# medhini/audio-video-textures

Hardware: AMD Instinct MI355X
Metric: clip-windows/sec encoded + N×N transition build, N=4096; HBM GB/s achieved (higher is better)
Workload: dtype f16x3

## Files before the change

audio-video-textures_amd/_lib.py:

```python
import ctypes as C
import os

_HERE = os.path.dirname(os.path.abspath(__file__))
LIB_PATH = os.environ.get("AVT_HIP_LIB") or os.path.join(_HERE, "libavt_hip.so")
HEADER_PATH = os.path.join(os.path.dirname(_HERE), "include", "avt.h")

_i32p, _i64p, _f32p, _vp = (C.POINTER(C.c_int32), C.POINTER(C.c_int64), C.POINTER(C.c_float), C.c_void_p)

SIGNATURES = {
    "avt_abi_version": [],
    "avt_device_check": [C.c_char_p, C.c_size_t],
    "avt_clip_sample_table": [C.c_int, _vp, _vp],
    "avt_clip_pack_plan": [_vp, C.c_int, C.c_int, C.c_int, _vp, _vp],
    "avt_clip_pack_u8": [_vp, C.c_int, C.c_int, C.c_int, _vp, _vp, C.c_int, C.c_int, C.c_float, C.c_float,
                         C.c_int, _vp, _vp, C.c_int, _vp],
    "avt_l2norm_rows": [_vp, C.c_int, _vp, C.c_int, C.c_int64, C.c_float, _vp, _vp, _vp, _vp],
    "avt_sim_gemm_nt": [_vp, _vp, _vp, _vp, C.c_int64, C.c_int64, C.c_int, C.c_float, C.c_int, _vp, C.c_int64, _vp],
    "avt_gemm_nt_x3_f32out": [_vp, _vp, C.c_int, _vp, _vp, _vp, C.c_int64, C.c_int, C.c_int, C.c_int, C.c_float, _vp, C.c_int, _vp],
    "avt_row_transition": [_vp, C.c_int64, C.c_int64, C.c_int64, _vp, C.c_int64, _vp, C.c_int64, C.c_float,
                           C.c_float, C.c_int, _vp, _vp, _vp, _vp, _vp, _vp],
    "avt_row_topk": [_vp, C.c_int64, C.c_int64, C.c_int64, _vp, C.c_int, _vp, _vp, _vp],
    "avt_softmax_ce_fwd": [_vp, C.c_int64, C.c_int64, _vp, _vp, _vp, _vp],
    "avt_softmax_ce_bwd": [_vp, _vp, C.c_int64, C.c_int64, C.c_float, _vp, _vp],
    "avt_clip_pack_u8_ndhwc4": [_vp, C.c_int, C.c_int, C.c_int, _vp, _vp, C.c_int, C.c_int, C.c_float, C.c_float,
                                C.c_int, _vp, _vp, _vp],
    "avt_maxpool_hw3s2_ndhwc_bf16": [_vp, _vp] + [C.c_int] * 7 + [_vp],
    "avt_mean_positions_bf16": [_vp] + [C.c_int] * 4 + [_vp, C.c_int, _vp],
    "avt_maxpool_hw2s2_ndhwc_bf16": [_vp, _vp] + [C.c_int] * 6 + [_vp],
    "avt_stem_conv_supported": [C.c_int] * 3,
    "avt_stem_conv_bf16": [_vp, _vp, _vp, _vp] + [C.c_int] * 9 + [_vp],
    "avt_stem_conv_pool_bf16": [_vp, _vp, _vp, _vp] + [C.c_int] * 10 + [_vp],
    "avt_bottleneck_fused_supported": [C.c_int] * 2,
    "avt_bottleneck_fused_bf16": [_vp] * 8 + [C.c_int] * 6 + [_vp],
    "avt_bottleneck_first_supported": [C.c_int] * 3,
    "avt_bottleneck_first_bf16": [_vp] * 9 + [C.c_int] * 7 + [_vp],
    "avt_pairwise_l2_f32": [_vp, C.c_int, C.c_int64, _vp, _vp],
    "avt_diag_filter_f32": [_vp, C.c_int, _vp, C.c_int, _vp, _vp],
    "avt_q_learning_supported": [C.c_int],
    "avt_q_learning_f32": [_vp, C.c_int, C.c_float, C.c_float, C.c_int, _vp, _vp, _vp],
    "avt_conv33_c64_supported": [C.c_int] * 3,
    "avt_conv33_c64_bf16": [_vp] * 4 + [C.c_int] * 6 + [_vp],
    "avt_pw_chain_supported": [C.c_int] * 5,
    "avt_pw_chain_bf16": [_vp, C.c_int, C.c_int, _vp, _vp, _vp, C.c_int, _vp, C.c_int, C.c_int, _vp, C.c_int, C.c_int,
                          _vp, _vp, _vp, C.c_int, C.c_int, C.c_int64, _vp],
    "avt_logmel_f64": [_vp, C.c_int, C.c_int64, _vp, C.c_int, C.c_int, C.c_int, _vp, C.c_int, C.c_double, _vp, _vp],
    "avt_logmel_examples_f32": [_vp, C.c_int64, C.c_int, C.c_int, C.c_int, _vp, _vp],
    "avt_infonce_fwd": [_vp, _vp, C.c_int64, C.c_int, C.c_int, C.c_float, C.c_float, _vp, _vp, _vp, _vp],
    "avt_infonce_bwd": [_vp] * 6 + [C.c_int64, C.c_int, C.c_int, C.c_float, _vp, _vp, _vp],
    "avt_conv3d_ktab": [C.c_int] * 7 + [_vp, C.c_int],
    "avt_conv3d_igemm_bf16": [_vp] * 6 + [C.c_int] * 22 + [_vp],
    "avt_conv3d_igemm_rows_bf16": [_vp] * 6 + [C.c_int] * 25 + [_vp],
    "avt_bn_train_fwd": [_vp, _vp, _vp, C.c_int64, C.c_int, _vp, _vp, C.c_float, C.c_float, C.c_int, C.c_int, _vp, C.c_int64, _vp, _vp, _vp,
                         _vp, _vp, _vp, C.c_int64, _vp],
    "avt_bn_train_bwd": [_vp, _vp, _vp, C.c_int64, C.c_int, _vp, _vp, _vp, _vp, C.c_int, C.c_int, _vp, _vp, C.c_int64, _vp, _vp, _vp, _vp,
                         C.c_int64, _vp],
    "avt_bn_train_ws_bytes": [C.c_int64, C.c_int, C.c_int],
    "avt_bn_train_ws_bytes_pre": [C.c_int, C.c_int, C.c_int],
    "avt_bn_train_fwd_pre": [_vp, _vp, _vp, C.c_int64, C.c_int, _vp, _vp, C.c_float, C.c_float, C.c_int, C.c_int, _vp, C.c_int64, _vp, _vp,
                             _vp, _vp, _vp, _vp, C.c_int64, C.c_int, _vp],
    "avt_conv3d_igemm_x3_f32_stat_rows": [C.c_int, C.c_int, C.c_int64, C.c_int],
    "avt_conv3d_igemm_x3_f32_bwdstats_rows": [C.c_int, C.c_int, C.c_int64, C.c_int],
    "avt_conv3d_igemm_x3_f32_bwdstats": [_vp] * 7 + [C.c_int] * 16 + [_vp] * 6 + [C.c_int, _vp, C.c_int, C.c_int, _vp],
    "avt_bn_train_bwd_pre": [_vp, _vp, C.c_int64, C.c_int, _vp, _vp, _vp, C.c_int, _vp, C.c_int64, C.c_int, _vp, _vp, _vp, _vp],
    "avt_pw_x3_f32_stat_rows": [C.c_int, C.c_int, C.c_int64, C.c_int],
    "avt_pw_x3_f32_bwdstats_rows": [C.c_int, C.c_int, C.c_int64, C.c_int],
    "avt_pw_x3_f32_bwdstats": [_vp, C.c_int, C.c_int, _vp, _vp, _vp, C.c_int, _vp, C.c_int, C.c_int, C.c_int64, C.c_int] + [_vp] * 6 +
                              [C.c_int, _vp, C.c_int, _vp],
    "avt_pw_x3_f32_stats": [_vp, C.c_int, C.c_int, _vp, _vp, _vp, _vp, C.c_int, C.c_int, C.c_int64, C.c_int, _vp, C.c_int, _vp],
    "avt_conv3d_igemm_x3_f32_stats": [_vp, _vp, _vp, _vp, _vp, _vp] + [C.c_int] * 18 + [_vp, C.c_int, C.c_int, _vp],
    "avt_conv3d_igemm_x3_f32": [_vp, _vp, _vp, _vp, _vp, _vp, _vp] + [C.c_int] * 19 + [_vp],
    "avt_conv3d_igemm_x3_f32_ex": [_vp] * 6 + [C.c_int] * 21 + [_vp],
    "avt_conv3d_wgrad_x3_f32": [_vp, _vp, _vp] + [C.c_int] * 17 + [_vp],
    "avt_wgrad_x3_set_xl": [C.c_int],
    "avt_conv_x3_set_small_tile": [C.c_int],
    "avt_conv3d_wgrad_x3_sub_f32": [_vp, _vp, _vp] + [C.c_int] * 22 + [_vp],
    "avt_interp_pack_pair_u8": [_vp, _vp, C.c_int, C.c_int, _f32p, _vp, _vp, _vp, C.c_int, _vp],
    "avt_avgpool2_x3": [_vp, _vp, C.c_int, C.c_int, C.c_int, C.c_int, C.c_int, _vp, _vp, C.c_int, C.c_int, _vp],
    "avt_upsample2_bilinear_x3": [_vp, _vp, C.c_int, C.c_int, C.c_int, C.c_int, C.c_int, _vp, _vp, C.c_int, C.c_int, _vp],
    "avt_interp_mid_input": [_vp, _vp, _vp, C.c_int, C.c_int, C.c_int, _vp, _vp, _vp, C.c_int, _vp],
    "avt_interp_final_u8": [_vp, _vp, _vp, _vp, C.c_int, C.c_int, C.c_int, _f32p, _vp, C.c_int, _vp],
    "avt_negative_sample_mt19937": [_vp, _vp, C.c_int, C.c_int, C.c_int, _vp, _vp],
    "avt_clip_pack_gather_u8": [_vp, C.c_int, C.c_int, C.c_int, _vp, C.c_int, C.c_int, C.c_int, C.c_float, C.c_float,
                                C.c_int, _vp, _vp, C.c_int, _vp],
    "avt_frames_resize_aa_norm_u8": [_vp, C.c_int, C.c_int, C.c_int, C.c_int, _f32p, _f32p, _vp, _vp],
    "avt_clip_gather_frames_f32": [_vp, C.c_int, C.c_int, _vp, C.c_int, C.c_int, _vp, _vp],
    "avt_stem_conv_x3": [_vp] * 8 + [C.c_int] * 11 + [_vp, C.c_int, _vp],
    "avt_lateral_x3_supported": [C.c_int] * 3,
    "avt_lateral_x3": [_vp, _vp, C.c_int, C.c_int, _vp, _vp, _vp, _vp, _vp, _vp] + [C.c_int] * 10 + [_vp],
    "avt_stem_conv_x3_merged": [_vp] * 8 + [C.c_int] * 10 + [_vp, _vp, C.c_int, C.c_int, _vp],
    "avt_clip_planes_f32": [_vp] + [C.c_int] * 4 + [C.c_int64] * 5 + [_vp, _vp, C.c_int, _vp],
    "avt_stem_conv_x3_f32": [_vp] * 6 + [C.c_int] * 11 + [_vp],
    "avt_weight_planes_f32": [_vp, C.c_int, C.c_int, _vp, _vp, _vp, C.c_int, _vp],
    "avt_weight_planes_t_f32": [_vp, C.c_int, C.c_int, C.c_int, _i32p, C.c_int, _vp, _vp, _vp],
    "avt_weight_planes_gather_f32": [_vp, _vp, C.c_int, C.c_int, _vp, _vp, _vp, C.c_int, _vp],
    "avt_weight_planes_job_bytes": [],
    "avt_weight_planes_multi": [_vp, _vp, C.c_int, _vp],
    "avt_sgd_job_bytes": [],
    "avt_sgd_multi": [_vp, _vp, C.c_int, _vp, _vp],
    "avt_sgd_upload": [_vp, _vp, C.c_int64, _vp],
    "avt_pack_job_bytes": [],
    "avt_grad_pack_multi": [_vp, _vp, C.c_int, _vp, _vp],
    "avt_maxpool_train_fwd": [_vp, _vp, _vp] + [C.c_int] * 4 + [C.c_int64, _vp],
    "avt_maxpool_train_bwd": [_vp, _vp, _vp] + [C.c_int] * 4 + [C.c_int64, _vp],
    "avt_maxpool3d_train_fwd": [_vp, _vp, _vp] + [C.c_int] * 5 + [C.c_int64, _vp],
    "avt_maxpool3d_train_bwd": [_vp, _vp, _vp] + [C.c_int] * 5 + [C.c_int64, _vp],
    "avt_stem_wgrad_x3_supported": [C.c_int] * 4,
    "avt_stem_wgrad_x3": [_vp] * 4 + [C.c_int] * 7 + [_vp],
    "avt_pw_x3_supported": [C.c_int] * 2,
    "avt_pw_x3": [_vp, _vp, C.c_int, C.c_int, _vp, _vp, _vp, _vp, _vp, _vp, C.c_int, _vp, _vp, C.c_int, C.c_int, C.c_int64,
                  C.c_int, C.c_int, _vp],
    "avt_pw_x3_f32_supported": [C.c_int] * 2,
    "avt_pw_x3_f32": [_vp, C.c_int, C.c_int, _vp, _vp, _vp, _vp, C.c_int, _vp, C.c_int, C.c_int, C.c_int64, C.c_int, _vp],
    "avt_pw_chain_x3_supported": [C.c_int] * 3,
    "avt_pw_chain_x3": [_vp, _vp, C.c_int, C.c_int, _vp, _vp, _vp, _vp, _vp, _vp, C.c_int, _vp, _vp, C.c_int, C.c_int, C.c_int,
                        _vp, _vp, _vp, _vp, _vp, _vp, C.c_int, C.c_int, C.c_int64, C.c_int, _vp],
    "avt_conv3d_igemm_x3": [_vp] * 10 + [C.c_int] * 26 + [_vp, _vp],
    "avt_conv3d_igemm_x3_wblk": [_vp] * 10 + [C.c_int] * 26 + [_vp, _vp],
    "avt_clip_pack_u8_ndhwc4_x3": [_vp, C.c_int, C.c_int, C.c_int, _vp, _vp, C.c_int, C.c_int, C.c_float, C.c_float,
                                   C.c_int, _vp, _vp, _vp, _vp, C.c_int, _vp],
    "avt_maxpool_hw3s2_ndhwc_x3": [_vp] * 4 + [C.c_int] * 8 + [_vp, _vp],
    "avt_maxpool_hw2s2_ndhwc_x3": [_vp] * 4 + [C.c_int] * 7 + [_vp],
    "avt_maxpool3d_k3s2_ndhwc_x3": [_vp] * 4 + [C.c_int] * 8 + [_vp],
    "avt_mean_positions_x3": [_vp, _vp] + [C.c_int] * 4 + [_vp, C.c_int, C.c_int, _vp],
    "avt_conv3d_igemm_x3_xl_picked": [C.c_int] * 3,
    "avt_conv33_x3_supported": [C.c_int] * 2,
    "avt_conv33_x3": [_vp] * 6 + [C.c_int] * 8 + [_vp],
    "avt_bneck_x3_supported": [C.c_int] * 3,
    "avt_bneck_x3": [_vp] * 6 + [C.c_int] * 8 + [_vp],
    "avt_res2_x3_supported": [C.c_int] * 3,
    "avt_res2_x3_wfrag_bytes": [],
    "avt_res2_x3": [_vp] * 6 + [C.c_int] * 7 + [_vp],
    "avt_conv3d_igemm_wfrag_supported": [C.c_int] * 5,
    "avt_conv3d_igemm_wfrag_bf16": [_vp] * 6 + [C.c_int] * 25 + [_vp, C.c_int, _vp],
}


class AvtError(RuntimeError):
    pass


_lib = None


def lib():
    global _lib
    if _lib is None:
        if not os.path.exists(LIB_PATH):
            raise AvtError(
                "HIP extension not built: %s is missing. Run `make -C %s` (needs hipcc); "
                "there is no CPU fallback for the hot path." % (LIB_PATH, os.path.join(_HERE, "csrc")))
        handle = C.CDLL(LIB_PATH)
        for name, argtypes in SIGNATURES.items():
            fn = getattr(handle, name)
            fn.argtypes = argtypes
            fn.restype = C.c_int64 if name in _RETURNS_I64 else C.c_int
        handle.avt_last_error.argtypes = []
        handle.avt_last_error.restype = C.c_char_p
        if handle.avt_abi_version() != ABI_VERSION:
            raise AvtError("libavt_hip.so ABI version %d, expected %d: rebuild with `make -C %s`"
                           % (handle.avt_abi_version(), ABI_VERSION, os.path.join(_HERE, "csrc")))
        if os.environ.get("AVT_SMALL_TILE", "") == "0":
            handle.avt_conv_x3_set_small_tile(0)
        if os.environ.get("AVT_WGRAD_ROUNDS", "") == "0":
            handle.avt_wgrad_x3_set_xl(7)
        _lib = handle
    return _lib


ABI_VERSION = 8
_RETURNS_I64 = {"avt_bn_train_ws_bytes", "avt_bn_train_ws_bytes_pre"}


def check(status, what):
    if status != 0:
        msg = lib().avt_last_error()
        raise AvtError("%s failed (%d): %s" % (what, status, msg.decode() if msg else "?"))
```

audio-video-textures_amd/csrc/conv_x3.hip:

```cpp
#include <stdlib.h>

#include <type_traits>

#include "avt_common.h"
#include "conv_args.h"
#include "launch.h"
#include "mfma.h"
#include "split_planes.h"

#ifdef AVT_CONV_STAMP
#define AVT_STAMP_FN avt_debug_stamps_x3
namespace {
#include "../../tools/diag/conv_stamp.h"
}
#ifndef AVT_DBG_CONST
#define AVT_DBG_CONST 0
#endif
#define DBG_SKIP(bit) (((AVT_DBG_CONST) & (bit)) != 0)
#ifdef AVT_STAMP_EPI
#define KSTAMP(i) STAMP(0)
#define EPI_STAMP(i) STAMP(i)
#else
#define KSTAMP(i) STAMP(i)
#define EPI_STAMP(i)
// ... 94 lines not shown
    }
    const int koff = ks * 32 + lh * 16;
#pragma unroll
    for (int j = 0; j < MT; ++j) {
      const int o = (wm * WTM + j * 32 + lr) * LSTR + koff;
      f.ah[j] = *reinterpret_cast<const i32x4*>(lds + o);
      f.al[j] = *reinterpret_cast<const i32x4*>(lds + A_LO + o);
    }
#pragma unroll
    for (int i = 0; i < NT; ++i) {
      const int o = (wn * WN + i * 32 + lr) * LSTR + koff;
      f.wh[i] = *reinterpret_cast<const i32x4*>(lds + B_HI + o);
      f.wl[i] = *reinterpret_cast<const i32x4*>(lds + B_LO + o);
    }
  };
  constexpr int NPIECE = 2 * (AU + BU), NGROUP = 4 * NT * MT, PPG = 2 * ((NPIECE + NGROUP - 1) / NGROUP);
  auto fmul = [&](const Frags& f, int g0, auto more_, auto&& piece) {
    constexpr bool more = decltype(more_)::value;
#pragma unroll
    for (int i = 0; i < NT; ++i)
#pragma unroll
      for (int j = 0; j < MT; ++j) {
        if (!DBG_SKIP(2)) {
          acc[i][j] = mfma32<F16>(f.wl[i], f.ah[j], acc[i][j]);
          acc[i][j] = mfma32<F16>(f.wh[i], f.al[j], acc[i][j]);
          acc[i][j] = mfma32<F16>(f.wh[i], f.ah[j], acc[i][j]);
        }
        if (more && !DBG_SKIP(4)) {
#pragma unroll
          for (int e = 0; e < PPG; ++e) {
            const int pc = (g0 + i * MT + j) * PPG + e;
            if (pc < NPIECE) piece(pc);
          }
        }
        __builtin_amdgcn_sched_barrier(0);
      }
  };
  auto compute = [&](auto more, auto&& prep, auto&& piece) {
    Frags f0, f1;
    fload(f0, 0);
    fload(f1, 1);
    if constexpr (decltype(more)::value) prep();
    __builtin_amdgcn_sched_barrier(0);
    fmul(f0, 0, more, piece);
    fload(f0, 2);
    __builtin_amdgcn_sched_barrier(0);
    fmul(f1, NT * MT, more, piece);
    fload(f1, 3);
    __builtin_amdgcn_sched_barrier(0);
    fmul(f0, 2 * NT * MT, more, piece);
    fmul(f1, 3 * NT * MT, more, piece);
  };

  const __amdgpu_buffer_rsrc_t rih = avt::buffer_rsrc(a.in, a.in_bytes);
  const __amdgpu_buffer_rsrc_t ril = avt::buffer_rsrc(a.in_lo, a.in_bytes);
  const __amdgpu_buffer_rsrc_t rwh = avt::buffer_rsrc(a.wt, a.wt_bytes);
  const __amdgpu_buffer_rsrc_t rwl = avt::buffer_rsrc(a.wt_lo, a.wt_bytes);
  int2* ltab = reinterpret_cast<int2*>(lds + STAGE);
  const bool tab_lds = a.nk <= kMaxTabSteps;
  if (tab_lds)
    for (int i = tid; i < a.nk * 8; i += 256) ltab[i] = a.ktab[i];
  i32x4 rah[AU], ral[AU], rbh[BU], rbl[BU];
  unsigned aoffs[AU], boffs[BU];
  auto gprep = [&](auto tl_, int kt) {
    int2 e;
    if constexpr (decltype(tl_)::value) e = ltab[kt * 8 + c16];
    else e = a.ktab[kt * 8 + c16];
    const unsigned ebits = (unsigned)e.y;
#pragma unroll
    for (int u = 0; u < AU; ++u) {
      const unsigned sel = ((rowmask[u] & ebits) == ebits) ? 0xFFFFFFFFu : 0u;
      aoffs[u] = (((unsigned)(rowoff[u] + e.x) * (IO32 ? 4u : 2u)) & sel) | (kOob & ~sel);
    }
    const unsigned ksel = ~(unsigned)(e.y >> 31);
    const unsigned kc2 = (unsigned)((kt * 8 + c16) * 16);
#pragma unroll
    for (int u = 0; u < BU; ++u) {
      const unsigned sel = ksel & wsel[u];
      boffs[u] = (((unsigned)wrow[u] * 2u + kc2) & sel) | (kOob & ~sel);
    }
  };
  auto gpiece = [&](int p) {
    if (p < 2 * AU) {
      const int u = p >> 1;
      if constexpr (IO32) {
        const unsigned o2 = aoffs[u] == kOob ? kOob : aoffs[u] + 16u;
        if (p & 1) ral[u] = __builtin_amdgcn_raw_buffer_load_b128(rih, (int)o2, 0, 0);
        else rah[u] = __builtin_amdgcn_raw_buffer_load_b128(rih, (int)aoffs[u], 0, 0);
      } else {
        if (p & 1) ral[u] = __builtin_amdgcn_raw_buffer_load_b128(ril, (int)aoffs[u], 0, 0);
        else rah[u] = __builtin_amdgcn_raw_buffer_load_b128(rih, (int)aoffs[u], 0, 0);
      }
    } else {
      const int u = (p - 2 * AU) >> 1;
      if (p & 1) rbl[u] = __builtin_amdgcn_raw_buffer_load_b128(rwl, (int)boffs[u], 0, 0);
      else rbh[u] = __builtin_amdgcn_raw_buffer_load_b128(rwh, (int)boffs[u], 0, 0);
    }
  };
  auto gload = [&](int kt) {
    gprep(std::false_type{}, kt);
#pragma unroll
    for (int p = 0; p < NPIECE; ++p) gpiece(p);
  };
  auto lstore = [&]() {
#pragma unroll
    for (int u = 0; u < AU; ++u) {
      const int o = (r0 + 32 * u) * LSTR + c16 * 16;
      if constexpr (IO32) {
        const float* fa = reinterpret_cast<const float*>(&rah[u]);
        const float* fb = reinterpret_cast<const float*>(&ral[u]);
        uint4 h, l;
        const float f8[8] = {fa[0], fa[1], fa[2], fa[3], fb[0], fb[1], fb[2], fb[3]};
        avt::split8<F16>(f8, h, l);
        *reinterpret_cast<uint4*>(lds + o) = h;
        *reinterpret_cast<uint4*>(lds + A_LO + o) = l;
      } else {
        *reinterpret_cast<i32x4*>(lds + o) = rah[u];
        *reinterpret_cast<i32x4*>(lds + A_LO + o) = ral[u];
      }
    }
#pragma unroll
    for (int u = 0; u < BU; ++u) {
      const int o = (r0 + 32 * u) * LSTR + c16 * 16;
      *reinterpret_cast<i32x4*>(lds + B_HI + o) = rbh[u];
      *reinterpret_cast<i32x4*>(lds + B_LO + o) = rbl[u];
    }
  };
  float* cfl = reinterpret_cast<float*>(lds + a.cf_ofs);
  for (int i = tid; i < 2 * BN; i += 256) {
    const int n = n0 + (i < BN ? i : i - BN);
    float v = i < BN ? 0.0f : 1.0f;
    if (n < a.Cout) {
      if (i < BN) { if (a.bias) v = a.bias[n]; } else if (a.wscale) v = a.wscale[n];
    }
    cfl[i] = v;
  }
  __syncthreads();
  STAMP_BEGIN();
  gload(0);
  lstore();
  __syncthreads();
  STAMP(0);
  auto kloop = [&](auto tl) {
    for (int kt = 0; kt + 1 < a.nk; ++kt) {
      STAMP(1);
      compute(std::true_type{}, [&]() { gprep(tl, kt + 1); }, gpiece);
      STAMP(2);
      __syncthreads();
      STAMP(3);
      if (!DBG_SKIP(1)) lstore();
      STAMP(4);
      __syncthreads();
      STAMP(5);
    }
  };
  if (tab_lds) kloop(std::true_type{});
  else kloop(std::false_type{});
  STAMP(1);
  compute(std::false_type{}, []() {}, gpiece);
  STAMP(2);
  __syncthreads();
  STAMP(3);

  const bool has_res = !IO32 && a.res != nullptr;
  uint4 rrh[EU], rrl[EU];
  if (has_res) {
#pragma unroll
    for (int u = 0; u < EU; ++u) {
      const int c = tid + 256 * u;
      const int m = m0 + c / CPR, n = n0 + (c % CPR) * 8;
      const bool ok = m < m_end && n < a.Cout;
      rrh[u] = ok ? *reinterpret_cast<const uint4*>(a.res + (int64_t)m * a.ldr + n) : make_uint4(0u, 0u, 0u, 0u);
      rrl[u] = ok ? *reinterpret_cast<const uint4*>(a.res_lo + (int64_t)m * a.ldr + n) : make_uint4(0u, 0u, 0u, 0u);
    }
  }
  if constexpr (IO32) {
    if (a.res) {
#pragma unroll
      for (int u = 0; u < EU; ++u) {
        const int c = tid + 256 * u;
        const int m = m0 + c / CPR, n = n0 + (c % CPR) * 8;
        const bool ok = m < m_end && n < a.Cout;
        const float* rf = reinterpret_cast<const float*>(a.res) + (int64_t)m * a.ldr + n;
        rrh[u] = ok ? *reinterpret_cast<const uint4*>(rf) : make_uint4(0u, 0u, 0u, 0u);
        rrl[u] = ok ? *reinterpret_cast<const uint4*>(rf + 4) : make_uint4(0u, 0u, 0u, 0u);
      }
    }
  }
  float4 bxa[BST ? EU : 1], bxb[BST ? EU : 1];
  unsigned bbits[BST ? EU : 1];
  BstCoef bk;
  if constexpr (BST) {
    {
      const int n = n0 + (tid % CPR) * 8;
      bst_load(a, tm / a.stat_tpg, n < a.Cout ? n : 0, bk);
#pragma unroll
      for (int u = 0; u < EU; ++u) {
        const int c = tid + 256 * u;
        const int m = m0 + c / CPR;
        const bool ok = m < m_end && n < a.Cout;
        const int64_t o = ok ? (int64_t)m * a.ldo + n : 0;
        bxa[u] = *reinterpret_cast<const float4*>(a.bst_x + o);
        bxb[u] = *reinterpret_cast<const float4*>(a.bst_x + o + 4);
        bbits[u] = a.bst_mask ? *reinterpret_cast<const uint16_t*>(a.bst_mask + (o >> 2)) : 0u;
        bbits[u] = (bbits[u] & 0xFu) | ((bbits[u] >> 4) & 0xF0u);
      }
    }
  }
#pragma unroll
  for (int i = 0; i < NT; ++i)
#pragma unroll
    for (int g = 0; g < 4; ++g) {
      const int nl = wn * WN + i * 32 + 8 * g + 4 * lh;
      const float4 bv = *reinterpret_cast<const float4*>(cfl + nl);
      const float4 sv = *reinterpret_cast<const float4*>(cfl + BN + nl);
#pragma unroll
      for (int j = 0; j < MT; ++j) {
        float4 v;
        v.x = acc[i][j][4 * g + 0] * sv.x + bv.x;
        v.y = acc[i][j][4 * g + 1] * sv.y + bv.y;
        v.z = acc[i][j][4 * g + 2] * sv.z + bv.z;
        v.w = acc[i][j][4 * g + 3] * sv.w + bv.w;
        const int ml = wm * WTM + j * 32 + lr;
        *reinterpret_cast<float4*>(lds + ml * ESTR + nl * 4) = v;
      }
    }
  __syncthreads();
  float st_s[IO32 ? 8 : 1], st_q[IO32 ? 8 : 1];
  if constexpr (IO32) {
#pragma unroll
    for (int e = 0; e < 8; ++e) st_s[e] = st_q[e] = 0.0f;
  }
#pragma unroll
  for (int u = 0; u < EU; ++u) {
    const int c = tid + 256 * u;
    const int row = c / CPR, cc = c % CPR;
    const int m = m0 + row, n = n0 + cc * 8;
    if (m < m_end && n < a.Cout) {
      const float4 v0 = *reinterpret_cast<const float4*>(lds + row * ESTR + cc * 32);
      const float4 v1 = *reinterpret_cast<const float4*>(lds + row * ESTR + cc * 32 + 16);
      float x[8] = {v0.x, v0.y, v0.z, v0.w, v1.x, v1.y, v1.z, v1.w};
      if (has_res) {
        const uint32_t* ph = reinterpret_cast<const uint32_t*>(&rrh[u]);
        const uint32_t* pl = reinterpret_cast<const uint32_t*>(&rrl[u]);
#pragma unroll
        for (int e = 0; e < 4; ++e) {
          const avt::f32x2 r = avt::join2<F16>(ph[e], pl[e]);
          x[2 * e] += r.x;
          x[2 * e + 1] += r.y;
        }
      }
      if (a.relu == 1) {
#pragma unroll
        for (int e = 0; e < 8; ++e) x[e] = avt::relu_keep_nan(x[e]);
      } else if (a.relu == 2) {
#pragma unroll
        for (int e = 0; e < 8; ++e) x[e] = fmaxf(x[e], 0.1f * x[e]);
      }
      const int64_t o = (int64_t)out_row(a, m) * a.ldo + n;
      if constexpr (IO32) {
        if (a.res) {
          const float4 r0_ = __builtin_bit_cast(float4, rrh[u]), r1_ = __builtin_bit_cast(float4, rrl[u]);
          x[0] += r0_.x; x[1] += r0_.y; x[2] += r0_.z; x[3] += r0_.w;
          x[4] += r1_.x; x[5] += r1_.y; x[6] += r1_.z; x[7] += r1_.w;
        }
        if constexpr (BST) {
          const float xv[8] = {bxa[u].x, bxa[u].y, bxa[u].z, bxa[u].w, bxb[u].x, bxb[u].y, bxb[u].z, bxb[u].w};
          bst_apply(a, bk, xv, bbits[u], x, st_s, st_q);
        } else if (a.stat_part) {
#pragma unroll
          for (int e = 0; e < 8; ++e) {
            st_s[e] += x[e];
            st_q[e] += x[e] * x[e];
          }
        }
        float* of = reinterpret_cast<float*>(a.out) + o;
        avt::stg4(of, avt::f32x4{x[0], x[1], x[2], x[3]});
        avt::stg4(of + 4, avt::f32x4{x[4], x[5], x[6], x[7]});
      } else {
        uint4 oh, ol;
        avt::split8<F16>(x, oh, ol);
        *reinterpret_cast<uint4*>(a.out + o) = oh;
        *reinterpret_cast<uint4*>(a.out_lo + o) = ol;
      }
    }
  }
  if constexpr (IO32) {
    if (a.stat_part) {
      __syncthreads();
      float* red = reinterpret_cast<float*>(lds);
      const int tr = tid / CPR, cc = tid % CPR;
#pragma unroll
      for (int e = 0; e < 8; ++e) {
        red[(tr * 2 + 0) * BN + cc * 8 + e] = st_s[e];
        red[(tr * 2 + 1) * BN + cc * 8 + e] = st_q[e];
      }
      __syncthreads();
      stat_fold_store<BN, 256>(a, red, 256 / CPR, tm, n0, tid);
    }
  }
  STAMP_END();
}

template <bool F16, bool IO32 = false, bool OUT32 = IO32>
__global__ __launch_bounds__(512, 2) void conv_x3_xl_kernel(ConvArgs a) {
  constexpr int BM = 256, BN = 256, NTHR = 512, KB = 32;
  constexpr int MT = 4, NT = 2;
  constexpr int AU = BM / 128, BU = BN / 128;
  constexpr int PL = BM * 64;
  constexpr int STG = 4 * PL;
  constexpr int ESTR = BN * 4 + 16;
  extern __shared__ __attribute__((aligned(16))) char lds[];

  const int swz = avt::xcd_contiguous(blockIdx.x, a.nblk);
  const int tm = swz / a.tiles_n, tn = swz % a.tiles_n;
  const int n0 = tn * BN;
  int m0, m_end;
  if constexpr (IO32) tile_rows(a, tm, BM, m0, m_end);
  else { m0 = tm * BM; m_end = a.M; }
  const int tid = threadIdx.x;
  const int lane = tid & 63, wid = tid >> 6;
  const int wm = wid >> 2, wn = wid & 3;
  const int lr = lane & 31, lh = lane >> 5;
  const int r0 = tid >> 2, c4 = (tid & 3) ^ ((r0 >> 2) & 3);

  int rowoff[AU];
  unsigned rowmask[AU];
#pragma unroll
  for (int u = 0; u < AU; ++u) {
    const int m = m0 + r0 + 128 * u;
    rowoff[u] = 0;
    rowmask[u] = 0u;
    if (m < m_end && a.pointwise) {
      rowoff[u] = m * a.ldi;
      rowmask[u] = 0x010101u;
    } else if (m < m_end) {
      const int t1 = (int)fastdiv((uint32_t)m, a.dWo), wo = m - t1 * a.Wo;
      const int t2 = (int)fastdiv((uint32_t)t1, a.dHo), ho = t1 - t2 * a.Ho;
      const int b = (int)fastdiv((uint32_t)t2, a.dTo), to = t2 - b * a.To;
      const int ti0 = to * a.st - a.pt, hi0 = ho * a.sh - a.ph, wi0 = wo * a.sw - a.pw;
      rowoff[u] = (((b * a.T + ti0) * a.H + hi0) * a.W + wi0) * a.ldi;
      unsigned mask = 0u;
      for (int dt = 0; dt < a.KT; ++dt) mask |= ((unsigned)(ti0 + dt) < (unsigned)a.T ? 1u : 0u) << dt;
      for (int dh = 0; dh < a.KH; ++dh) mask |= ((unsigned)(hi0 + dh) < (unsigned)a.H ? 1u : 0u) << (8 + dh);
      for (int dw = 0; dw < a.KW; ++dw) mask |= ((unsigned)(wi0 + dw) < (unsigned)a.W ? 1u : 0u) << (16 + dw);
      rowmask[u] = mask;
    }
  }
  int wrow[BU];
  unsigned wsel[BU];
#pragma unroll
  for (int u = 0; u < BU; ++u) {
    const int n = n0 + r0 + 128 * u;
    wrow[u] = n < a.Cout ? n * a.K : 0;
    wsel[u] = n < a.Cout ? 0xFFFFFFFFu : 0u;
  }

  f32x16 acc[NT][MT];
#pragma unroll
  for (int i = 0; i < NT; ++i)
#pragma unroll
    for (int j = 0; j < MT; ++j)
#pragma unroll
      for (int r = 0; r < 16; ++r) acc[i][j][r] = 0.0f;
  const __amdgpu_buffer_rsrc_t rih = avt::buffer_rsrc(a.in, a.in_bytes);
  const __amdgpu_buffer_rsrc_t ril = avt::buffer_rsrc(a.in_lo, a.in_bytes);
  const __amdgpu_buffer_rsrc_t rwh = avt::buffer_rsrc(a.wt, a.wt_bytes);
  const __amdgpu_buffer_rsrc_t rwl = avt::buffer_rsrc(a.wt_lo, a.wt_bytes);
  int2* ltab = reinterpret_cast<int2*>(lds + 2 * STG);
  for (int i = tid; i < a.nk * 8; i += NTHR) ltab[i] = a.ktab[i];
  const int nk32 = (a.K + KB - 1) / KB;

  unsigned aoffs[AU], boffs[BU];
  auto gtab = [&](int kt) -> int2 { return ltab[kt * 4 + c4]; };
  auto gcalc = [&](int kt, int2 e) {
    const unsigned ebits = (unsigned)e.y;
#pragma unroll
    for (int u = 0; u < AU; ++u) {
      const unsigned sel = ((rowmask[u] & ebits) == ebits) ? 0xFFFFFFFFu : 0u;
      aoffs[u] = (((unsigned)(rowoff[u] + e.x) * (IO32 ? 4u : 2u)) & sel) | (kOob & ~sel);
    }
    const unsigned ksel = ~(unsigned)(e.y >> 31);
    const unsigned kc2 = (unsigned)((kt * 4 + c4) * 16);
#pragma unroll
    for (int u = 0; u < BU; ++u) {
      const unsigned sel = ksel & wsel[u];
      boffs[u] = (((unsigned)wrow[u] * 2u + kc2) & sel) | (kOob & ~sel);
      if (a.wblk) boffs[u] = (((unsigned)(kt * a.Cout + n0 + r0 + 128 * u) * 64u + (unsigned)c4 * 16u) & sel) | (kOob & ~sel);
    }
  };
  auto gprep = [&](int kt) { gcalc(kt, gtab(kt)); };
  constexpr int NPIECE = 2 * (AU + BU);
  typedef __attribute__((address_space(3))) void* lds_ptr;
  const int wrow0 = wid * 16 * 64;
  auto gpiece = [&](int p, char* st) {
    if (p < 2 * AU) {
      const int u = p >> 1;
      __builtin_amdgcn_raw_ptr_buffer_load_lds((p & 1) ? ril : rih, (lds_ptr)(st + (p & 1) * PL + wrow0 + u * 128 * 64), 16,
                                               (int)aoffs[u], 0, 0, 0);
    } else {
      const int u = (p - 2 * AU) >> 1;
      __builtin_amdgcn_raw_ptr_buffer_load_lds((p & 1) ? rwl : rwh, (lds_ptr)(st + (2 + (p & 1)) * PL + wrow0 + u * 128 * 64), 16,
                                               (int)boffs[u], 0, 0, 0);
    }
  };
  i32x4 ra[IO32 ? AU : 1][2];
  auto aload = [&]() {
    if constexpr (IO32) {
#pragma unroll
      for (int u = 0; u < AU; ++u) {
        const unsigned o2 = aoffs[u] == kOob ? kOob : aoffs[u] + 16u;
        ra[u][0] = __builtin_amdgcn_raw_buffer_load_b128(rih, (int)aoffs[u], 0, 0);
        ra[u][1] = __builtin_amdgcn_raw_buffer_load_b128(rih, (int)o2, 0, 0);
      }
    }
  };
  auto astore = [&](char* st) {
    if constexpr (IO32) {
#pragma unroll
      for (int u = 0; u < AU; ++u) {
        const float* fa = reinterpret_cast<const float*>(&ra[u][0]);
        const float* fb = reinterpret_cast<const float*>(&ra[u][1]);
        uint4 h, l;
        const float f8[8] = {fa[0], fa[1], fa[2], fa[3], fb[0], fb[1], fb[2], fb[3]};
        avt::split8<F16>(f8, h, l);
        const int o = (r0 + 128 * u) * 64 + (tid & 3) * 16;
        *reinterpret_cast<uint4*>(st + o) = h;
        *reinterpret_cast<uint4*>(st + PL + o) = l;
      }
    }
  };
  const int fsw = (lr >> 2) & 3;
  struct Frags {
    i32x4 ah[MT], al[MT], wh[NT], wl[NT];
  };
  auto fload = [&](Frags& f, const char* st, int ks) {
    const int slot = ((ks * 2 + lh) ^ fsw) * 16;
    auto rd_w = [&](int i) {
      const int o = (wn * 64 + i * 32 + lr) * 64 + slot;
      f.wh[i] = *reinterpret_cast<const i32x4*>(st + 2 * PL + o);
      f.wl[i] = *reinterpret_cast<const i32x4*>(st + 3 * PL + o);
    };
    rd_w(0);
#pragma unroll
    for (int j = 0; j < MT; ++j) {
      const int o = (wm * 128 + j * 32 + lr) * 64 + slot;
      f.ah[j] = *reinterpret_cast<const i32x4*>(st + o);
      f.al[j] = *reinterpret_cast<const i32x4*>(st + PL + o);
    }
#pragma unroll
    for (int i = 1; i < NT; ++i) rd_w(i);
  };
  auto fmul = [&](const Frags& f, int g0, bool more, char* nst) {
#pragma unroll
    for (int i = 0; i < NT; ++i)
#pragma unroll
      for (int j = 0; j < MT; ++j) {
        acc[i][j] = mfma32<F16>(f.wl[i], f.ah[j], acc[i][j]);
        acc[i][j] = mfma32<F16>(f.wh[i], f.al[j], acc[i][j]);
        acc[i][j] = mfma32<F16>(f.wh[i], f.ah[j], acc[i][j]);
        const int pc = g0 + i * MT + j + (IO32 ? 2 * AU : 0);
        if (more && pc < NPIECE) gpiece(pc, nst);
        __builtin_amdgcn_sched_barrier(0);
      }
  };

  float* cfl = reinterpret_cast<float*>(lds + a.cf_ofs);
  {
    const int n = n0 + (tid & 255);
    float v = tid < 256 ? 0.0f : 1.0f;
    if (n < a.Cout) {
      if (tid < 256) { if (a.bias) v = a.bias[n]; } else if (a.wscale) v = a.wscale[n];
    }
    cfl[tid] = v;
  }
  __syncthreads();
  STAMP_BEGIN();
  gprep(0);
  if constexpr (IO32) {
    aload();
#pragma unroll
    for (int p = 2 * AU; p < NPIECE; ++p) gpiece(p, lds);
    asm volatile("s_waitcnt vmcnt(0)" ::: "memory");
    astore(lds);
  } else {
#pragma unroll
    for (int p = 0; p < NPIECE; ++p) gpiece(p, lds);
    asm volatile("s_waitcnt vmcnt(0)" ::: "memory");
  }
  __syncthreads();
  STAMP(0);
  if constexpr (IO32) {
    for (int kt = 0; kt < nk32; ++kt) {
      const bool more = kt + 1 < nk32;
      char* cur = lds + (kt & 1) * STG;
      char* nst = lds + ((kt + 1) & 1) * STG;
      int2 e = make_int2(0, 0);
      if (more) e = gtab(kt + 1);
      Frags f;
      fload(f, cur, 0);
      if (more) {
        gcalc(kt + 1, e);
        aload();
      }
      __builtin_amdgcn_sched_barrier(0);
      fmul(f, 0, more, nst);
      fload(f, cur, 1);
      __builtin_amdgcn_sched_barrier(0);
      fmul(f, NPIECE, false, nst);
      asm volatile("s_waitcnt vmcnt(0)" ::: "memory");
      if (more) astore(nst);
      __syncthreads();
    }
  } else {
    Frags f0, f1;
    fload(f0, lds, 0);
    if (nk32 > 1) gprep(1);
    fload(f1, lds, 1);
    __builtin_amdgcn_sched_barrier(0);
    fmul(f0, 0, nk32 > 1, lds + STG);
    asm volatile("s_waitcnt vmcnt(0) lgkmcnt(0)" ::: "memory");
    __syncthreads();
    for (int kt = 1; kt < nk32; ++kt) {
      const bool more = kt + 1 < nk32;
      char* cur = lds + (kt & 1) * STG;
      char* nst = lds + ((kt + 1) & 1) * STG;
      int2 e = make_int2(0, 0);
      if (more) e = gtab(kt + 1);
      fload(f0, cur, 0);
      if (more) gcalc(kt + 1, e);
      __builtin_amdgcn_sched_barrier(0);
      fmul(f1, 0, more, nst);
      KSTAMP(1);
      fload(f1, cur, 1);
      __builtin_amdgcn_sched_barrier(0);
      fmul(f0, NPIECE, false, nst);
      KSTAMP(2);
      asm volatile("s_waitcnt vmcnt(0) lgkmcnt(0)" ::: "memory");
      KSTAMP(3);
      __syncthreads();
      KSTAMP(4);
    }
    fmul(f1, NPIECE, false, lds);
  }

  constexpr int SR = 64;
  constexpr int CPR = BN / 8;
  constexpr int EU = (SR * CPR) / NTHR;
  constexpr int EBUF = SR * ESTR;
  static_assert(2 * EBUF <= 2 * STG + kMaxTabSteps * 64, "two staging buffers fit the operand stages + the table area");
  const bool has_res = !OUT32 && a.res != nullptr;
  auto stage_slab = [&](auto half, int pass) {
    constexpr int H = decltype(half)::value;
    char* eb = lds + (pass & 1) * EBUF;
#pragma unroll
    for (int i = 0; i < NT; ++i)
#pragma unroll
      for (int g = 0; g < 4; ++g) {
        const int nl = wn * 64 + i * 32 + 8 * g + 4 * lh;
        const float4 bv = *reinterpret_cast<const float4*>(cfl + nl);
        const float4 sv = *reinterpret_cast<const float4*>(cfl + 256 + nl);
#pragma unroll
        for (int jj = 0; jj < 2; ++jj) {
          const int j = 2 * H + jj;
          float4 v;
          v.x = acc[i][j][4 * g + 0] * sv.x + bv.x;
          v.y = acc[i][j][4 * g + 1] * sv.y + bv.y;
          v.z = acc[i][j][4 * g + 2] * sv.z + bv.z;
          v.w = acc[i][j][4 * g + 3] * sv.w + bv.w;
          const int rl = jj * 32 + lr;
          *reinterpret_cast<float4*>(eb + rl * ESTR + nl * 4) = v;
        }
      }
  };
  KSTAMP(5);
  if (wm == 0) stage_slab(std::integral_constant<int, 0>{}, 0);
  __syncthreads();
  EPI_STAMP(1);
  float st_s[IO32 ? 8 : 1], st_q[IO32 ? 8 : 1];
  if constexpr (IO32) {
#pragma unroll
    for (int e = 0; e < 8; ++e) st_s[e] = st_q[e] = 0.0f;
  }
#pragma unroll 1
  for (int pass = 0; pass < 4; ++pass) {
    const char* eb = lds + (pass & 1) * EBUF;
    uint4 rrh[EU], rrl[EU];
    if (has_res) {
#pragma unroll
      for (int u = 0; u < EU; ++u) {
        const int c = tid + NTHR * u;
        const int m = m0 + pass * SR + c / CPR, n = n0 + (c % CPR) * 8;
        const bool ok = m < m_end && n < a.Cout;
        rrh[u] = ok ? *reinterpret_cast<const uint4*>(a.res + (int64_t)m * a.ldr + n) : make_uint4(0u, 0u, 0u, 0u);
        rrl[u] = ok ? *reinterpret_cast<const uint4*>(a.res_lo + (int64_t)m * a.ldr + n) : make_uint4(0u, 0u, 0u, 0u);
      }
    }
    if constexpr (IO32) {
      if (a.res) {
#pragma unroll
        for (int u = 0; u < EU; ++u) {
          const int c = tid + NTHR * u;
          const int m = m0 + pass * SR + c / CPR, n = n0 + (c % CPR) * 8;
          const bool ok = m < m_end && n < a.Cout;
          const float* rf = reinterpret_cast<const float*>(a.res) + (int64_t)m * a.ldr + n;
          rrh[u] = ok ? *reinterpret_cast<const uint4*>(rf) : make_uint4(0u, 0u, 0u, 0u);
          rrl[u] = ok ? *reinterpret_cast<const uint4*>(rf + 4) : make_uint4(0u, 0u, 0u, 0u);
        }
      }
    }
    if (pass + 1 < 4 && wm == ((pass + 1) >> 1)) {
      if ((pass + 1) & 1) stage_slab(std::integral_constant<int, 1>{}, pass + 1);
      else stage_slab(std::integral_constant<int, 0>{}, pass + 1);
    }
    EPI_STAMP(2);
#pragma unroll
    for (int u = 0; u < EU; ++u) {
      const int c = tid + NTHR * u;
      const int row = c / CPR, cc = c % CPR;
      const int m = m0 + pass * SR + row, n = n0 + cc * 8;
      if (m < m_end && n < a.Cout) {
        const float4 v0 = *reinterpret_cast<const float4*>(eb + row * ESTR + cc * 32);
        const float4 v1 = *reinterpret_cast<const float4*>(eb + row * ESTR + cc * 32 + 16);
        float x[8] = {v0.x, v0.y, v0.z, v0.w, v1.x, v1.y, v1.z, v1.w};
        if (has_res) {
          const uint32_t* ph = reinterpret_cast<const uint32_t*>(&rrh[u]);
          const uint32_t* pl = reinterpret_cast<const uint32_t*>(&rrl[u]);
#pragma unroll
          for (int e = 0; e < 4; ++e) {
            const avt::f32x2 r = avt::join2<F16>(ph[e], pl[e]);
            x[2 * e] += r.x;
            x[2 * e + 1] += r.y;
          }
        }
        if (a.relu == 1) {
#pragma unroll
          for (int e = 0; e < 8; ++e) x[e] = avt::relu_keep_nan(x[e]);
        } else if (a.relu == 2) {
#pragma unroll
          for (int e = 0; e < 8; ++e) x[e] = fmaxf(x[e], 0.1f * x[e]);
        }
        const int64_t o = (int64_t)out_row(a, m) * a.ldo + n;
        if constexpr (OUT32) {
          if (a.odiv != 0.0f) {
#pragma unroll
            for (int e = 0; e < 8; ++e) x[e] = __fdiv_rn(x[e], a.odiv);
          }
          if (IO32 && a.res) {
            const float4 q0 = __builtin_bit_cast(float4, rrh[u]), q1 = __builtin_bit_cast(float4, rrl[u]);
            x[0] += q0.x; x[1] += q0.y; x[2] += q0.z; x[3] += q0.w;
            x[4] += q1.x; x[5] += q1.y; x[6] += q1.z; x[7] += q1.w;
          }
          if constexpr (IO32) {
            if (a.stat_part) {
#pragma unroll
              for (int e = 0; e < 8; ++e) {
                st_s[e] += x[e];
                st_q[e] += x[e] * x[e];
              }
            }
          }
          float* of = reinterpret_cast<float*>(a.out) + o;
          avt::stg4(of, avt::f32x4{x[0], x[1], x[2], x[3]});
          avt::stg4(of + 4, avt::f32x4{x[4], x[5], x[6], x[7]});
        } else {
          uint4 oh, ol;
          avt::split8<F16>(x, oh, ol);
          *reinterpret_cast<uint4*>(a.out + o) = oh;
          *reinterpret_cast<uint4*>(a.out_lo + o) = ol;
        }
      }
    }
    EPI_STAMP(3);
    __syncthreads();
    EPI_STAMP(4);
  }
  if constexpr (IO32) {
    if (a.stat_part) {
      float* red = reinterpret_cast<float*>(lds);
      const int tr = tid / CPR, cc = tid % CPR;
#pragma unroll
      for (int e = 0; e < 8; ++e) {
        red[(tr * 2 + 0) * BN + cc * 8 + e] = st_s[e];
        red[(tr * 2 + 1) * BN + cc * 8 + e] = st_q[e];
      }
      __syncthreads();
      stat_fold_store<BN, NTHR>(a, red, NTHR / CPR, tm, n0, tid);
    }
  }
  STAMP_END();
}

template <bool F16, bool IO32 = false, bool OUT32 = IO32>
int launch_x3_xl(ConvArgs& a, hipStream_t st) {
  if (a.stat_part) a.stat_tpg = (a.stat_mg + 255) / 256;
  const int tiles_m = a.stat_part ? a.stat_groups * a.stat_tpg : (a.M + 255) / 256;
  a.tiles_n = (a.Cout + 255) / 256;
  a.nblk = tiles_m * a.tiles_n;
  constexpr int lds_bytes = 2 * 4 * 256 * 64 + kMaxTabSteps * 64 + 2 * 256 * 4;
  a.cf_ofs = lds_bytes - 2 * 256 * 4;
  return avt::launch<conv_x3_xl_kernel<F16, IO32, OUT32>>("avt_conv3d_igemm_x3", dim3((unsigned)a.nblk), dim3(512), lds_bytes, lds_bytes,
                                                          st, a);
}

template <int BM, int BN, int WTM, bool F16, bool IO32 = false, bool BST = false>
int launch_x3(ConvArgs& a, hipStream_t st) {
  if (a.stat_part) a.stat_tpg = (a.stat_mg + BM - 1) / BM;
  const int tiles_m = a.stat_part ? a.stat_groups * a.stat_tpg : (a.M + BM - 1) / BM;
  a.tiles_n = (a.Cout + BN - 1) / BN;
  a.nblk = tiles_m * a.tiles_n;
  constexpr int epi_bytes = BM * (BN * 4 + 16);
  constexpr int opnd_max = 2 * (BM + BN) * LSTR + kMaxTabSteps * 64;
  constexpr int lds_max = (opnd_max > epi_bytes ? opnd_max : epi_bytes) + 2 * BN * 4;
  const int tab_bytes = (a.nk <= kMaxTabSteps ? a.nk : 0) * 64;
  int lds_bytes = 2 * (BM + BN) * LSTR + tab_bytes;
  if (lds_bytes < epi_bytes) lds_bytes = epi_bytes;
  a.cf_ofs = lds_bytes;
  lds_bytes += 2 * BN * 4;
  return avt::launch<conv_x3_kernel<BM, BN, WTM, F16, IO32, BST>>("avt_conv3d_igemm_x3", dim3((unsigned)a.nblk), dim3(256), lds_max,
                                                                  lds_bytes, st, a);
}

template <bool F16, bool IO32 = false, bool BST = false>
int launch_x3_by_cout(ConvArgs& a, hipStream_t st, bool small = false) {
  if (a.Cout <= 32) return launch_x3<128, 32, 32, F16, IO32, BST>(a, st);
  if (a.Cout <= 64) return launch_x3<128, 64, 64, F16, IO32, BST>(a, st);
  if constexpr (IO32) {
    if (small) return launch_x3<64, 128, 32, F16, IO32, BST>(a, st);
  }
  return launch_x3<128, 128, 64, F16, IO32, BST>(a, st);
}

struct X3Planes {
  const void *in_hi, *in_lo, *wt_hi, *wt_lo;
  const float* bias;
  const void *res_hi, *res_lo;
  void *out_hi, *out_lo;
};

}

extern "C" int avt_conv3d_igemm_x3_xl_picked(int cout, int k, int m) {
  return (cout % 256 == 0 && k >= 256 && k <= kMaxTabSteps * 64 && m >= 256 * 64) ? 1 : 0;
}

static int igemm_x3_one(const X3Planes& p, const int32_t* ktab, const ConvGeom& g, int plane_dtype, const float* wscale, void* stream,
                        int wblk, int xl) {
  AVT_REQUIRE(plane_dtype == AVT_X3_BF16 || plane_dtype == AVT_X3_F16, "avt_conv3d_igemm_x3: plane_dtype must be 0 (bf16) or 1 (fp16)");
  AVT_REQUIRE(!wscale || avt::aligned16(wscale), "avt_conv3d_igemm_x3: wscale must be 16-byte aligned");
  AVT_REQUIRE(p.in_lo && p.wt_lo && p.out_lo && (!p.res_hi == !p.res_lo), "avt_conv3d_igemm_x3: every tensor needs both planes");
  AVT_REQUIRE(avt::aligned16(p.in_lo) && avt::aligned16(p.wt_lo) && avt::aligned16(p.out_lo) && (!p.res_lo || avt::aligned16(p.res_lo)),
              "avt_conv3d_igemm_x3: pointers must be 16-byte aligned");
  ConvArgs a;
  const int rc = conv_args_fill(a, "avt_conv3d_igemm_x3", p.in_hi, p.wt_hi, p.bias, p.res_hi, p.out_hi, ktab, g);
  if (rc != AVT_OK) return rc;
  a.in_lo = static_cast<const uint16_t*>(p.in_lo);
  a.wt_lo = static_cast<const uint16_t*>(p.wt_lo);
  a.res_lo = static_cast<const uint16_t*>(p.res_lo);
  a.out_lo = static_cast<uint16_t*>(p.out_lo);
  a.wscale = wscale;
  a.wfrag = nullptr;
  a.nup = 0;
  a.wblk = wblk;
  hipStream_t s = static_cast<hipStream_t>(stream);
  AVT_REQUIRE(!wblk || (xl && a.K % 32 == 0),
              "avt_conv3d_igemm_x3_wblk: K-blocked weights are the 256 x 256 tile's (avt_conv3d_igemm_x3_xl_picked, K %% 32 == 0)");
  if (xl) return plane_dtype == AVT_X3_F16 ? launch_x3_xl<true>(a, s) : launch_x3_xl<false>(a, s);
  return plane_dtype == AVT_X3_F16 ? launch_x3_by_cout<true>(a, s) : launch_x3_by_cout<false>(a, s);
}

static int igemm_x3_impl(const X3Planes& p, const int32_t* ktab, const ConvGeom& g, int plane_dtype, const float* wscale, void* stream,
                         int wblk) {
  constexpr int64_t kMaxPlane = (1ll << 31) - 64;
  const bool sane = g.batch > 0 && g.t > 0 && g.h > 0 && g.w > 0 && g.ldi > 0 && g.ldo > 0 && g.cin > 0 && g.cout > 0 && g.kt >= 1 &&
                    g.kh >= 1 && g.kw >= 1 && g.st >= 1 && g.sh >= 1 && g.sw >= 1 && g.ph >= 0 && g.pw >= 0 && g.ho >= 0 && g.wo >= 0 &&
                    g.out_row_stride >= 1 && g.out_h >= 0 && g.out_w >= 0;
  const int64_t frame = sane ? (int64_t)g.h * g.w * g.ldi : 0, frames = sane ? (int64_t)g.batch * g.t : 0;
  if (!sane || frame * frames < kMaxPlane || g.kt != 1 || g.st != 1 || g.pt != 0 || (g.to != 0 && g.to != g.t)) {
    const int64_t k_all = (int64_t)g.kt * g.kh * g.kw * g.cin;
    int xl = 0;
    if (sane && k_all < (1ll << 31)) {
      const int64_t fho = g.ho > 0 ? g.ho : (g.h + 2 * g.ph - g.kh) / g.sh + 1, fwo = g.wo > 0 ? g.wo : (g.w + 2 * g.pw - g.kw) / g.sw + 1;
      const int64_t fto = g.to > 0 ? g.to : (g.t + 2 * g.pt - g.kt) / g.st + 1;
      const int64_t m = (int64_t)g.batch * fto * fho * fwo;
      xl = (m > 0 && m < (1ll << 31)) ? avt_conv3d_igemm_x3_xl_picked(g.cout, (int)k_all, (int)m) : 0;
    }
    return igemm_x3_one(p, ktab, g, plane_dtype, wscale, stream, wblk, xl);
  }
  AVT_REQUIRE(frame < kMaxPlane, "avt_conv3d_igemm_x3: one frame's input plane (%d x %d x %d elements) is too large for 32-bit offsets", g.h,
              g.w, g.ldi);
  AVT_REQUIRE(p.in_hi && p.in_lo && p.out_hi && p.out_lo && (!p.res_hi == !p.res_lo), "avt_conv3d_igemm_x3: every tensor needs both planes");
  const int fho = g.ho > 0 ? g.ho : (g.h + 2 * g.ph - g.kh) / g.sh + 1, fwo = g.wo > 0 ? g.wo : (g.w + 2 * g.pw - g.kw) / g.sw + 1;
  AVT_REQUIRE(fho > 0 && fwo > 0, "avt_conv3d_igemm_x3: bad output extent");
  const bool remap = g.out_row_stride > 1 || (g.out_h > 0 && g.out_w > 0);
  const int64_t m_all = frames * fho * fwo;
  const int64_t orows = remap ? (int64_t)g.out_h * g.out_w : (int64_t)fho * fwo;
  AVT_REQUIRE(m_all < (1ll << 31) && frames * orows < (1ll << 31) && (int64_t)g.kh * g.kw * g.cin < (1ll << 31),
              "avt_conv3d_igemm_x3: tensor too large for 32-bit rows");
  const int xl = avt_conv3d_igemm_x3_xl_picked(g.cout, g.kh * g.kw * g.cin, (int)m_all);
  const int64_t fmax = kMaxPlane / frame;
  const int64_t nrange = (frames + fmax - 1) / fmax;
  const int64_t per = (frames + nrange - 1) / nrange;
  for (int64_t f0 = 0; f0 < frames; f0 += per) {
    ConvGeom gr = g;
    gr.batch = (int)((frames - f0 < per) ? frames - f0 : per);
    gr.t = 1;
    gr.to = g.to ? 1 : 0;
    const int64_t io = f0 * frame, oo = f0 * orows * g.ldo, ro = f0 * fho * fwo * g.ldr;
    auto adv = [](const void* q, int64_t e) { return q ? static_cast<const void*>(static_cast<const uint16_t*>(q) + e) : nullptr; };
    X3Planes pr = p;
    pr.in_hi = adv(p.in_hi, io), pr.in_lo = adv(p.in_lo, io);
    pr.res_hi = adv(p.res_hi, ro), pr.res_lo = adv(p.res_lo, ro);
    pr.out_hi = const_cast<void*>(adv(p.out_hi, oo)), pr.out_lo = const_cast<void*>(adv(p.out_lo, oo));
    const int rc = igemm_x3_one(pr, ktab, gr, plane_dtype, wscale, stream, wblk, xl);
    if (rc != AVT_OK) return rc;
  }
  return AVT_OK;
}

extern "C" int avt_conv3d_igemm_x3(const void* in_hi, const void* in_lo, const void* wt_hi, const void* wt_lo,
                                   const float* bias, const void* res_hi, const void* res_lo, void* out_hi, void* out_lo,
                                   const int32_t* ktab, int batch, int t, int h, int w, int cin, int cout, int kt, int kh,
                                   int kw, int st, int sh, int sw, int pt, int ph, int pw, int to, int ho, int wo, int ldi,
                                   int ldo, int ldr, int relu, int out_row_stride, int out_h, int out_w, int plane_dtype,
                                   const float* wscale, void* stream) {
  const ConvGeom g = {.batch = batch, .t = t, .h = h, .w = w, .cin = cin, .cout = cout, .kt = kt, .kh = kh, .kw = kw,
                      .st = st, .sh = sh, .sw = sw, .pt = pt, .ph = ph, .pw = pw, .to = to, .ho = ho, .wo = wo,
                      .ldi = ldi, .ldo = ldo, .ldr = ldr, .relu = relu, .out_row_stride = out_row_stride, .out_h = out_h, .out_w = out_w};
  const X3Planes p = {.in_hi = in_hi, .in_lo = in_lo, .wt_hi = wt_hi, .wt_lo = wt_lo, .bias = bias,
                      .res_hi = res_hi, .res_lo = res_lo, .out_hi = out_hi, .out_lo = out_lo};
  return igemm_x3_impl(p, ktab, g, plane_dtype, wscale, stream, 0);
}

extern "C" int avt_conv3d_igemm_x3_wblk(const void* in_hi, const void* in_lo, const void* wt_hi, const void* wt_lo,
                                        const float* bias, const void* res_hi, const void* res_lo, void* out_hi, void* out_lo,
                                        const int32_t* ktab, int batch, int t, int h, int w, int cin, int cout, int kt, int kh,
                                        int kw, int st, int sh, int sw, int pt, int ph, int pw, int to, int ho, int wo, int ldi,
                                        int ldo, int ldr, int relu, int out_row_stride, int out_h, int out_w, int plane_dtype,
                                        const float* wscale, void* stream) {
  const ConvGeom g = {.batch = batch, .t = t, .h = h, .w = w, .cin = cin, .cout = cout, .kt = kt, .kh = kh, .kw = kw,
                      .st = st, .sh = sh, .sw = sw, .pt = pt, .ph = ph, .pw = pw, .to = to, .ho = ho, .wo = wo,
                      .ldi = ldi, .ldo = ldo, .ldr = ldr, .relu = relu, .out_row_stride = out_row_stride, .out_h = out_h, .out_w = out_w};
  const X3Planes p = {.in_hi = in_hi, .in_lo = in_lo, .wt_hi = wt_hi, .wt_lo = wt_lo, .bias = bias,
                      .res_hi = res_hi, .res_lo = res_lo, .out_hi = out_hi, .out_lo = out_lo};
  return igemm_x3_impl(p, ktab, g, plane_dtype, wscale, stream, 1);
}

extern "C" int avt_gemm_nt_x3_f32out(const void* a_hi, const void* a_lo, int lda, const void* b_hi, const void* b_lo, float* out, int64_t ldo,
                                     int m, int n, int k, float divisor, const int32_t* ktab, int plane_dtype, void* stream) {
  AVT_REQUIRE(plane_dtype == AVT_X3_BF16 || plane_dtype == AVT_X3_F16, "avt_gemm_nt_x3_f32out: plane_dtype must be 0 (bf16) or 1 (fp16)");
  AVT_REQUIRE(a_lo && b_lo && avt::aligned16(a_lo) && avt::aligned16(b_lo) && divisor != 0.0f, "avt_gemm_nt_x3_f32out: both planes, divisor != 0");
  AVT_REQUIRE(m > 0 && n % 256 == 0 && k % 32 == 0 && k >= 256 && k <= kMaxTabSteps * 64 && ldo >= n && ldo % 4 == 0 && ldo < (1ll << 31),
              "avt_gemm_nt_x3_f32out: n %% 256 == 0, 256 <= k <= %d in multiples of 32 (got m %d n %d k %d)", kMaxTabSteps * 64, m, n, k);
  const ConvGeom g = {.batch = 1, .t = 1, .h = 1, .w = m, .cin = k, .cout = n, .kt = 1, .kh = 1, .kw = 1, .st = 1, .sh = 1, .sw = 1,
                      .pt = 0, .ph = 0, .pw = 0, .to = 0, .ho = 0, .wo = 0, .ldi = lda, .ldo = 8 * (int)((ldo + 7) / 8), .ldr = 0,
                      .relu = 0, .out_row_stride = 1, .out_h = 0, .out_w = 0};
  ConvArgs a;
  const int rc = conv_args_fill(a, "avt_gemm_nt_x3_f32out", a_hi, b_hi, nullptr, nullptr, out, ktab, g);
  if (rc != AVT_OK) return rc;
  a.ldo = (int)ldo;
  a.in_lo = static_cast<const uint16_t*>(a_lo);
  a.wt_lo = static_cast<const uint16_t*>(b_lo);
  a.res_lo = nullptr;
  a.out_lo = nullptr;
  a.wscale = nullptr;
  a.wfrag = nullptr;
  a.nup = 0;
  a.wblk = 0;
  a.odiv = divisor;
  hipStream_t s = static_cast<hipStream_t>(stream);
  return plane_dtype == AVT_X3_F16 ? launch_x3_xl<true, false, true>(a, s) : launch_x3_xl<false, false, true>(a, s);
}

static int g_io32_small = 1;
static int io32_tile_rows(int cout, int k, int64_t m) {
  if (k % 32 == 0 && m < (1ll << 31) && avt_conv3d_igemm_x3_xl_picked(cout, k, (int)m) && m >= 256 * 256) return 256;
  if (g_io32_small && cout > 64 && ((m + 127) / 128) * ((cout + 127) / 128) < 512) return 64;
  return 128;
}

extern "C" int avt_conv_x3_set_small_tile(int on) {
  const int was = g_io32_small;
  g_io32_small = on ? 1 : 0;
  return was;
}

static int igemm_x3_f32_impl(const float* in, const void* wt_hi, const void* wt_lo, const float* wscale, const float* add, float* out,
                             const int32_t* ktab, const ConvGeom& g, int plane_dtype, void* stream, double* stat_part = nullptr,
                             int stat_groups = 0, int stat_c = 0, const ConvArgs* bst = nullptr) {
  const int cout = g.cout;
  AVT_REQUIRE(plane_dtype == AVT_X3_BF16 || plane_dtype == AVT_X3_F16, "avt_conv3d_igemm_x3_f32: plane_dtype must be 0 (bf16) or 1 (fp16)");
  AVT_REQUIRE(wt_lo && avt::aligned16(wt_lo) && (!wscale || avt::aligned16(wscale)), "avt_conv3d_igemm_x3_f32: weight planes / wscale NULL or unaligned");
  AVT_REQUIRE((int64_t)g.batch * g.t * g.h * g.w * g.ldi < (1ll << 30) - 64, "avt_conv3d_igemm_x3_f32: input too large for 32-bit byte offsets");
  ConvArgs a;
  const int rc = conv_args_fill(a, "avt_conv3d_igemm_x3_f32", in, wt_hi, nullptr, add, out, ktab, g);
  if (rc != AVT_OK) return rc;
  a.in_bytes *= 2u;
  a.in_lo = nullptr;
  a.wt_lo = static_cast<const uint16_t*>(wt_lo);
  a.res_lo = nullptr;
  a.out_lo = nullptr;
  a.wscale = wscale;
  a.wfrag = nullptr;
  a.nup = 0;
  a.wblk = 0;
  if (stat_part) {
    AVT_REQUIRE(stat_groups >= 1 && a.M % stat_groups == 0 && stat_c >= 8 && cout % stat_c == 0 && a.oH == 0 && (!add || bst) &&
                    avt::aligned16(stat_part),
                "avt_conv3d_igemm_x3_f32_stats: %d rows in %d groups, %d channels of %d columns, no row remap, no add operand", a.M,
                stat_groups, stat_c, cout);
    {
      const int bn_launch = (!bst && a.oH == 0 && io32_tile_rows(cout, a.K, a.M) == 256) ? 256 : (cout <= 32 ? 32 : (cout <= 64 ? 64 : 128));
      AVT_REQUIRE(stat_c == cout || cout <= bn_launch,
                  "avt_conv3d_igemm_x3_f32_stats: %d pixel copies of %d channels span more than one %d-column tile", cout / stat_c, stat_c,
                  bn_launch);
    }
    if (bst) {
      AVT_REQUIRE(bst->bst_x && bst->bst_mean && bst->bst_invstd && bst->bst_gamma && g.ldo == cout && avt::aligned16(bst->bst_x) &&
                      (!bst->bst_relu || bst->bst_mask || bst->bst_beta),
                  "avt_conv3d_igemm_x3_f32_bwdstats: BatchNorm input / statistics / scale missing, or the output rows are not contiguous");
      a.bst_x = bst->bst_x; a.bst_mean = bst->bst_mean; a.bst_invstd = bst->bst_invstd; a.bst_gamma = bst->bst_gamma;
      a.bst_beta = bst->bst_beta; a.bst_mask = bst->bst_mask; a.bst_relu = bst->bst_relu;
    }
    a.stat_part = stat_part;
    a.stat_groups = stat_groups;
    a.stat_mg = a.M / stat_groups;
    a.stat_c = stat_c;
    AVT_REQUIRE((int64_t)stat_groups * ((a.stat_mg + 127) / 128) < (1ll << 24), "avt_conv3d_igemm_x3_f32_stats: too many tiles");
  }
  hipStream_t s = static_cast<hipStream_t>(stream);
  if (bst) {
    AVT_REQUIRE(plane_dtype == AVT_X3_BF16 && io32_tile_rows(cout, a.K, a.M) != 256,
                "avt_conv3d_igemm_x3_f32_bwdstats: bf16 planes, layers of the 128- / 64-row tiles (avt_conv3d_igemm_x3_f32_bwdstats_rows)");
    return launch_x3_by_cout<false, true, true>(a, s, io32_tile_rows(cout, a.K, a.M) == 64);
  }
  const bool small = io32_tile_rows(cout, a.K, a.M) == 64;
  if (a.oH == 0 && io32_tile_rows(cout, a.K, a.M) == 256)
    return plane_dtype == AVT_X3_F16 ? launch_x3_xl<true, true>(a, s) : launch_x3_xl<false, true>(a, s);
  return plane_dtype == AVT_X3_F16 ? launch_x3_by_cout<true, true>(a, s, small) : launch_x3_by_cout<false, true>(a, s, small);
}

extern "C" int avt_conv3d_igemm_x3_f32(const float* in, const void* wt_hi, const void* wt_lo, const float* wscale, const float* add,
                                       float* out, const int32_t* ktab, int batch, int t, int h, int w, int cin, int cout, int kt, int kh,
                                       int kw, int st, int sh, int sw, int pt, int ph, int pw, int ldi, int ldo, int lda, int plane_dtype,
                                       void* stream) {
  const ConvGeom g = {.batch = batch, .t = t, .h = h, .w = w, .cin = cin, .cout = cout, .kt = kt, .kh = kh, .kw = kw,
                      .st = st, .sh = sh, .sw = sw, .pt = pt, .ph = ph, .pw = pw, .ldi = ldi, .ldo = ldo, .ldr = add ? lda : 0,
                      .out_row_stride = 1};
  return igemm_x3_f32_impl(in, wt_hi, wt_lo, wscale, add, out, ktab, g, plane_dtype, stream);
}

extern "C" int avt_conv3d_igemm_x3_f32_stat_rows(int cout, int k, int64_t m, int groups) {
  if (groups < 1 || m <= 0 || m % groups) return -1;
  const int bm = io32_tile_rows(cout, k, m);
  return (int)((m / groups + bm - 1) / bm);
}

extern "C" int avt_conv3d_igemm_x3_f32_stats(const float* in, const void* wt_hi, const void* wt_lo, const float* wscale, float* out,
                                             const int32_t* ktab, int batch, int t, int h, int w, int cin, int cout, int kt, int kh, int kw,
                                             int st, int sh, int sw, int pt, int ph, int pw, int ldi, int ldo, int plane_dtype,
                                             void* stat_part, int groups, int stat_c, void* stream) {
  AVT_REQUIRE(stat_part, "avt_conv3d_igemm_x3_f32_stats: NULL stat_part");
  const ConvGeom g = {.batch = batch, .t = t, .h = h, .w = w, .cin = cin, .cout = cout, .kt = kt, .kh = kh, .kw = kw,
                      .st = st, .sh = sh, .sw = sw, .pt = pt, .ph = ph, .pw = pw, .ldi = ldi, .ldo = ldo, .ldr = 0,
                      .out_row_stride = 1};
  return igemm_x3_f32_impl(in, wt_hi, wt_lo, wscale, nullptr, out, ktab, g, plane_dtype, stream, static_cast<double*>(stat_part), groups,
                           stat_c);
}

extern "C" int avt_conv3d_igemm_x3_f32_bwdstats_rows(int cout, int k, int64_t m, int groups) {
  if (groups < 1 || m <= 0 || m % groups) return -1;
  const int bm = io32_tile_rows(cout, k, m);
  if (bm == 256) return -1;
  return (int)((m / groups + bm - 1) / bm);
}

extern "C" int avt_conv3d_igemm_x3_f32_bwdstats(const float* in, const void* wt_hi, const void* wt_lo, const float* wscale, const float* add,
                                                float* out, const int32_t* ktab, int batch, int t, int h, int w, int cin, int cout, int kt,
                                                int kh, int kw, int pt, int ph, int pw, int ldi, int ldo, int lda, int plane_dtype,
                                                const float* bn_x, const float* bn_mean, const float* bn_invstd, const float* bn_gamma,
                                                const float* bn_beta, const void* bn_mask, int relu, void* stat_part, int groups, int stat_c,
                                                void* stream) {
  AVT_REQUIRE(stat_part, "avt_conv3d_igemm_x3_f32_bwdstats: NULL stat_part");
  ConvArgs b = {};
  b.bst_x = bn_x; b.bst_mean = bn_mean; b.bst_invstd = bn_invstd; b.bst_gamma = bn_gamma; b.bst_beta = bn_beta;
  b.bst_mask = static_cast<const uint8_t*>(bn_mask); b.bst_relu = relu;
  const ConvGeom g = {.batch = batch, .t = t, .h = h, .w = w, .cin = cin, .cout = cout, .kt = kt, .kh = kh, .kw = kw,
                      .st = 1, .sh = 1, .sw = 1, .pt = pt, .ph = ph, .pw = pw, .ldi = ldi, .ldo = ldo, .ldr = add ? lda : 0,
                      .out_row_stride = 1};
  return igemm_x3_f32_impl(in, wt_hi, wt_lo, wscale, add, out, ktab, g, plane_dtype, stream, static_cast<double*>(stat_part), groups,
                           stat_c, &b);
}

extern "C" int avt_conv3d_igemm_x3_f32_ex(const float* in, const void* wt_hi, const void* wt_lo, const float* wscale, float* out,
                                          const int32_t* ktab, int batch, int t, int h, int w, int cin, int cout, int kt, int kh, int kw,
                                          int pt, int ph, int pw, int to, int ho, int wo, int ldi, int ldo, int out_row_stride, int out_h,
                                          int out_w, int plane_dtype, void* stream) {
  const ConvGeom g = {.batch = batch, .t = t, .h = h, .w = w, .cin = cin, .cout = cout, .kt = kt, .kh = kh, .kw = kw,
                      .st = 1, .sh = 1, .sw = 1, .pt = pt, .ph = ph, .pw = pw, .to = to, .ho = ho, .wo = wo, .ldi = ldi, .ldo = ldo, .ldr = 0,
                      .out_row_stride = out_row_stride, .out_h = out_h, .out_w = out_w};
  return igemm_x3_f32_impl(in, wt_hi, wt_lo, wscale, nullptr, out, ktab, g, plane_dtype, stream);
}
```

audio-video-textures_amd/fused_slowfast.py:

```python
import torch
import torch.nn as nn

from . import ops
from ._lib import AvtError


_FUSE_BLOCK = 1
_C33 = 1
_CHAIN = 1
_CHAIN_MAXN = 512
_FUSE_KCAT = 1
_XB = 1
_FUSE_SCAT = 1
_FUSE_TCHUNK = 0
_FUSE_SCAT_X3 = 1
_SCAT_X3_SKIP = set()
_FUSE_BLOCK_X3 = 1
_FUSE_TCHUNK_X3 = 0
_CHAIN_X3 = 1
_WBLK_X3 = 1
_STEM_FM_X3 = 1
_C33_X3 = 1
_RES2_X3 = 1
_PW_X3 = 1
_STEM_LDS = 1
_STEM_POOL = 1
_PW_X3_SKIP = {(512, 128), (320, 128)}
_LATERAL_X3 = {(32, 64)}
_STEM_MERGE = 1
_KW1_CAP = 32

PROFILER = None


def _observed(name, launch, flops, nbytes):
    if PROFILER is None:
        launch()
    else:
        PROFILER(name() if callable(name) else name, launch, flops, nbytes)


def _rows(dims):
    return dims[0] * dims[1] * dims[2] * dims[3]


class Act:

    __slots__ = ("buf", "dims", "c0", "C", "lo")

    def __init__(self, buf, dims, c0=0, C=None, lo=None):
        self.buf, self.dims, self.c0, self.lo = buf, dims, c0, lo
        self.C = buf.shape[1] - c0 if C is None else C

    @property
    def ptr(self):
        return self.buf.data_ptr() + 2 * self.c0

    @property
    def ptrs(self):
        return (self.buf.data_ptr() + 2 * self.c0, self.lo.data_ptr() + 2 * self.c0)

    @property
    def ld(self):
        return self.buf.shape[1]

    @property
    def rows(self):
        return _rows(self.dims)

    def float(self, plane_dtype=None):
        if self.lo is None:
            return self.buf[:, self.c0 : self.c0 + self.C].float()
        dt = torch.float16 if plane_dtype == ops.X3_F16 else torch.bfloat16
        sl = slice(self.c0, self.c0 + self.C)
        return self.buf.view(dt)[:, sl].float() + self.lo.view(dt)[:, sl].float()


def new_act(m, c, dims, device, x3=False):
    buf = torch.empty((m, c), dtype=torch.bfloat16, device=device)
    return Act(buf, dims, lo=torch.empty_like(buf) if x3 else None)


def split_planes(w, plane_dtype):
    w = w.detach().float()
    dt = torch.float16 if plane_dtype == ops.X3_F16 else torch.bfloat16
    hi = w.to(dt)
    lo = (w - hi.float()).to(dt)
    return hi.view(torch.bfloat16).contiguous(), lo.view(torch.bfloat16).contiguous()


def fold_bn(conv, bn):
    w = conv.weight.detach().float()
    if bn is not None:
        scale = bn.weight.detach().float() / torch.sqrt(bn.running_var.detach().float() + bn.eps)
        bias = bn.bias.detach().float() - bn.running_mean.detach().float() * scale
        w = w * scale.view(-1, 1, 1, 1, 1)
    else:
        bias = conv.bias.detach().float() if conv.bias is not None else torch.zeros(w.shape[0])
    return w, bias


def group_weights_w(w, g):
    cout, cin, kt, kh, kw = w.shape
    r = kw // 2
    rg = -(-r // g)
    kwg = 1 + 2 * rg
    wg = torch.zeros((g, cout, g, cin, kt, kh, kwg))
    for po in range(g):
        for dg in range(kwg):
            for pi in range(g):
                dw = g * (dg - rg) + pi - po + r
                if 0 <= dw < kw:
                    wg[po, :, pi, :, :, :, dg] = w[:, :, :, :, dw]
    return wg.reshape(g * cout, g * cin, kt, kh, kwg), rg


def pack_wfrag(wt, cin, taps):
    wt = wt.detach().float().cpu()
    cout, k = wt.shape
    nu = -(-k // 32)
    nup = -(-nu // 4) * 4 + 4
    tiles = -(-cout // 256) * 8
    wp = torch.zeros((tiles * 32, k + 1))
    wp[:cout, :k] = wt
    i = torch.arange(nup).view(-1, 1, 1, 1)
    cc, tap = (i // taps, i % taps) if taps > 1 else (i, torch.zeros_like(i))
    ks = torch.arange(2).view(1, -1, 1, 1)
    lane = torch.arange(64).view(1, 1, -1, 1)
    e = torch.arange(8).view(1, 1, 1, -1)
    cch = cc * 32 + ks * 16 + (lane >> 5) * 8 + e
    kidx = torch.where((cch < cin) & (i < nu), tap * cin + cch, torch.full_like(cch, k)).expand(nup, 2, 64, 8)
    rows = (torch.arange(tiles).view(-1, 1, 1, 1, 1) * 32 + (lane & 31).view(1, 1, 1, 64, 1)).expand(tiles, nup, 2, 64, 8)
    return wp[rows, kidx.unsqueeze(0).expand(tiles, nup, 2, 64, 8)].to(torch.bfloat16).contiguous()


class FusedConv:
    def __init__(self, conv, bn, relu, device, packed=None, folded=None, x3=None):
        self.crop = (0, 0, 0)
        self.x3 = x3
        self._folded = None
        self._grouped = {}
        if packed is None:
            if folded is None:
                w, bias = fold_bn(conv, bn)
                self.stride, self.pad = tuple(conv.stride), tuple(conv.padding)
            else:
                w, bias, self.stride, self.pad = folded
            self.kernel = tuple(w.shape[2:])
            self.cin, cout = w.shape[1], w.shape[0]
            wt = w.permute(0, 2, 3, 4, 1).reshape(cout, -1)
            self._folded = (w, bias)
        else:
            wt, bias, self.cin, self.kernel, self.stride, self.pad, self.crop = packed
            cout = wt.shape[0]
        self.cout, self.relu = cout, relu
        if relu == 2 and x3 is None:
            raise AvtError("FusedConv: LeakyReLU (relu=2) exists in the split-plane kernel only")
        if self.cin % 8:
            raise AvtError("FusedConv: input channels must be a multiple of 8 (got %d)" % self.cin)
        if cout % 8:
            raise AvtError("FusedConv: output channels must be a multiple of 8 (got %d)" % cout)
        self.wfrag = self.wt_lo = self.wscale = self.wblk = self.pw = self.lat = None
        taps = self.kernel[0] * self.kernel[1] * self.kernel[2]
        if x3 is not None:
            wf = wt.detach().float()
            if x3 == ops.X3_F16:
                mx = wf.abs().amax(dim=1).clamp_min(1e-30)
                e = torch.floor(torch.log2(mx))
                sc = torch.pow(2.0, 9.0 - e)
                wf = wf * sc.view(-1, 1)
                self.wscale = (1.0 / sc).float().contiguous().to(device)
            hi, lo = split_planes(wf, x3)
            self.wt, self.wt_lo = hi.to(device), lo.to(device)
            k_all = hi.shape[1]
            if _WBLK_X3 and cout % 256 == 0 and k_all % 32 == 0 and ops.conv3d_igemm_x3_xl_picked(cout, k_all, 1 << 20):
                blk = lambda p: p.view(cout, k_all // 32, 32).permute(1, 0, 2).contiguous().to(device)
                self.wblk = (blk(hi), blk(lo))
            if (_PW_X3 and relu != 2 and self.kernel == (1, 1, 1) and self.stride == (1, 1, 1) and self.pad == (0, 0, 0) and
                    not any(self.crop) and cout % 32 == 0 and ops.pw_x3_supported(self.cin, cout) and
                    (self.cin, cout) not in _PW_X3_SKIP):
                self.pw = (pack_pw_planes(hi).to(device), pack_pw_planes(lo).to(device))
            if ((_LATERAL_X3 == "all" or (self.cin, cout) in _LATERAL_X3) and relu != 2 and self.kernel[0] > 1 and self.kernel[1:] == (1, 1) and self.stride[1:] == (1, 1) and
                    self.pad[1:] == (0, 0) and not any(self.crop) and ops.lateral_x3_supported(self.cin, cout, self.kernel[0])):
                n_pad = -(-cout // 32) * 32
                padr = lambda p: torch.cat([p.cpu(), torch.zeros((n_pad - cout, p.shape[1]), dtype=p.dtype)], 0) if n_pad > cout else p
                padv = lambda v, fill: None if v is None else torch.cat([v.cpu().float(), torch.full((n_pad - cout,), fill)]).contiguous().to(device)
                self.lat = (pack_pw_planes(padr(hi)).to(device), pack_pw_planes(padr(lo)).to(device), padv(bias, 0.0), padv(self.wscale, 1.0))
        else:
            self.wt = wt.to(torch.bfloat16).contiguous().to(device)
            if _XB and ops.conv3d_wfrag_supported(self.cin, cout, self.kernel):
                self.wfrag = pack_wfrag(self.wt.float().cpu(), self.cin, taps).to(device)
        self.bias = bias.float().contiguous().to(device)
        self.dev = device
        self._tabs = {}
        self.alg_flops_per_row = 2.0 * self.wt.shape[1] * cout

    def out_dims(self, dims):
        b, t, h, w = dims
        o = [(n + 2 * p - k) // s + 1 - c for n, p, k, s, c in zip((t, h, w), self.pad, self.kernel, self.stride, self.crop)]
        return (b, o[0], o[1], o[2])

    def kernel_symbol(self, m_out):
        if self.x3 is not None:
            if self.pw is not None or self.lat is not None:
                return "pw_x3_kernel<%s>" % ("f16" if self.x3 == ops.X3_F16 else "bf16")
            if ops.conv3d_igemm_x3_xl_picked(self.cout, self.wt.shape[1], m_out):
                return "conv_x3_xl_kernel<%s>" % ("f16" if self.x3 == ops.X3_F16 else "bf16")
            tile = "128,32,32" if self.cout <= 32 else ("128,64,64" if self.cout <= 64 else "128,128,64")
            return "conv_x3_kernel<%s,%s>" % (tile, "f16" if self.x3 == ops.X3_F16 else "bf16")
        if self.wfrag is not None:
            return "conv_xb_kernel"
        taps = self.kernel[0] * self.kernel[1] * self.kernel[2]
        nk = -(-self.wt.shape[1] // 64)
        if self.cout >= 256 and nk >= 16 and (self.cin % 32 == 0 or taps == 1):
            return "conv_xl_kernel<256,256,2>"
        return "conv_igemm_kernel<%s>" % ("256,32,64" if self.cout <= 32 else ("256,64,64" if self.cout <= 64 else "128,128,64"))

    def group_factor(self, x, out, res):
        if self._folded is None or self.stride[2] != 1 or self.pad[2] != self.kernel[2] // 2:
            return 1
        if self.lat is not None and res is None:
            return 1
        if x.ld != x.C or x.c0 or (out is not None and (out.ld != out.C or out.c0)) or \
                (res is not None and (res.ld != res.C or res.c0)):
            return 1
        small = min(self.cin, self.cout)
        g = 4 if small <= 16 else (2 if small <= 32 else 1)
        if self.kernel[2] == 1 and self.kernel[0] > 1 and _KW1_CAP:
            while g > 1 and g * self.cout > _KW1_CAP:
                g //= 2
        while g > 1 and x.dims[3] % g:
            g //= 2
        return g

    def __call__(self, x, out=None, res=None, relu=None, out_rows=None):
        if x.C != self.cin:
            raise AvtError("FusedConv: input has %d channels, conv expects %d" % (x.C, self.cin))
        g = 1 if out_rows is not None else self.group_factor(x, out, res)
        if g > 1:
            sub = self._grouped.get(g)
            if sub is None:
                w, bias = self._folded
                wg, rg = group_weights_w(w, g)
                sub = FusedConv(None, None, self.relu, self.dev,
                                folded=(wg, bias.repeat(g), self.stride, (self.pad[0], self.pad[1], rg)), x3=self.x3)
                sub._folded = None
                sub.alg_flops_per_row = g * self.alg_flops_per_row
                self._grouped[g] = sub
            b, t, h, w_ = x.dims
            od = self.out_dims(x.dims)
            if out is None:
                out = new_act(_rows(od), self.cout, od, self.dev, self.x3 is not None)
            view = lambda a, d, c: Act(a.buf.view(-1, g * c), (d[0], d[1], d[2], d[3] // g),
                                       lo=a.lo.view(-1, g * c) if a.lo is not None else None)
            sub(view(x, x.dims, self.cin), out=view(out, od, self.cout),
                res=view(res, od, self.cout) if res is not None else None, relu=relu)
            return out
        key = (x.dims[2], x.dims[3], x.ld)
        tab = self._tabs.get(key)
        if tab is None:
            tab = torch.from_numpy(ops.conv3d_ktab(self.cin, self.kernel, x.dims[2], x.dims[3], x.ld)).to(self.dev)
            self._tabs[key] = tab
        od = self.out_dims(x.dims)
        m_out = _rows(od)
        if out is None:
            out = new_act(m_out, self.cout, od, self.dev, self.x3 is not None)

        def launch_x3():
            blocked = self.wblk is not None and ops.conv3d_igemm_x3_xl_picked(self.cout, self.wt.shape[1], m_out)
            wh, wl = self.wblk if blocked else (self.wt, self.wt_lo)
            ops.conv3d_igemm_x3(x.ptrs, wh, wl, self.bias, res.ptrs if res is not None else None, out.ptrs, tab,
                                x.dims, self.cin, self.cout, self.kernel, self.stride, self.pad, x.ld, out.ld,
                                res.ld if res is not None else 0, self.relu if relu is None else relu, self.x3,
                                wscale=self.wscale, out_dims=od[1:] if any(self.crop) else (0, 0, 0), out_rows=out_rows,
                                wblk=blocked)

        def launch_pw():
            ops.pw_x3(x.ptrs, x.ld, self.cin, self.pw[0], self.pw[1], self.bias, self.wscale,
                      res.ptrs if res is not None else None, res.ld if res is not None else 0, out.ptrs, out.ld, self.cout,
                      x.rows, self.relu if relu is None else relu, self.x3)

        def launch_lat():
            b_, t_, h_, w_ = x.dims
            ops.lateral_x3(x.ptrs, x.ld, self.cin, self.lat[0], self.lat[1], self.lat[2], self.lat[3], out.ptrs, out.ld, self.cout, b_, t_,
                           h_ * w_, self.kernel[0], self.stride[0], self.pad[0], self.relu if relu is None else relu, self.x3)

        def launch():
            if self.x3 is not None:
                if self.lat is not None and out_rows is None and res is None:
                    return launch_lat()
                return launch_pw() if (self.pw is not None and out_rows is None) else launch_x3()
            ops.conv3d_igemm(x.ptr, self.wt, self.bias, res.ptr if res is not None else 0, out.ptr, tab, x.dims,
                             self.cin, self.cout, self.kernel, self.stride, self.pad, x.ld, out.ld,
                             res.ld if res is not None else 0, self.relu if relu is None else relu,
                             out_dims=od[1:] if any(self.crop) else (0, 0, 0), out_rows=out_rows, wfrag=self.wfrag)

        nb = 2.0 * (x.rows * self.cin + m_out * self.cout * (2 if res is not None else 1)) + self.wt.numel() * 2
        _observed(lambda: self.kernel_symbol(m_out), launch, m_out * self.alg_flops_per_row, nb * (2 if self.x3 is not None else 1))
        return out


def stem_lds_image(wt, kt, frame_major=False):
    cout = wt.shape[0]
    if frame_major:
        w = wt.reshape(cout // 32, 2, 4, 4, kt, 7, 4, 8)
        return w.permute(0, 4, 5, 1, 6, 2, 3, 7).contiguous().reshape(cout // 32, -1)
    w = wt.reshape(cout // 32, 4, 2, 4, kt, 7, 4, 8)
    return w.permute(0, 4, 5, 2, 6, 1, 3, 7).contiguous().reshape(cout // 32, -1)


def merged_stem_taps(conv, win_len, device):
    hit = conv._merged.get(win_len)
    if hit is not None or win_len in conv._merged:
        return hit
    wg, bias = conv.wg
    g, c, kt_g = wg.shape[0], wg.shape[1], wg.shape[2]
    fast_off, _ = ops.clip_sample_table(win_len)
    n_slots, pt = len(fast_off), conv.pad[0]
    n_grp = (n_slots + 2 * pt - kt_g) // g + 1
    groups = []
    for to in range(n_grp):
        by_src = {}
        for dt in range(kt_g):
            k = g * to - pt + dt
            if 0 <= k < n_slots:
                by_src.setdefault(int(fast_off[k]), []).append(dt)
        groups.append(sorted(by_src.items()))
    ktm = max(len(x) for x in groups)
    if ktm >= kt_g:
        conv._merged[win_len] = None
        return None
    kt0 = kt_g - g + 1
    wflat = wg.reshape(g * c, kt_g, -1)
    wm = torch.zeros((g * c, n_grp * ktm, wflat.shape[2]))
    src = torch.full((n_grp, ktm), -1, dtype=torch.int32)
    tiles = torch.zeros((n_grp * ktm,), dtype=torch.int32)
    for to, items in enumerate(groups):
        for j, (off, dts) in enumerate(items):
            wm[:, to * ktm + j] = sum(wflat[:, dt] for dt in dts)
            src[to, j] = off
            tiles[to * ktm + j] = sum(1 << n for n in range(2) if any(2 * n <= dt <= 2 * n + kt0 for dt in dts))
    m = FusedConv(None, None, True, device,
                  packed=(wm.reshape(g * c, -1), bias.repeat(g), 8, (n_grp * ktm, conv.kernel[1], 4), conv.stride, conv.pad, (0, 0, 1)),
                  x3=conv.x3)
    out = {"wt_hi": stem_lds_image(m.wt, n_grp * ktm, True), "wt_lo": stem_lds_image(m.wt_lo, n_grp * ktm, True), "bias": m.bias,
           "wscale": m.wscale, "src": src.to(device), "tiles": tiles.to(device), "ktm": ktm, "groups": n_grp}
    conv._merged[win_len] = out
    return out


def stem_conv(stem, device, tgroup=1, x3=None):
    w, bias = fold_bn(stem.conv, stem.bn)
    c, _, kt, kh, kw = w.shape
    if (kh, kw) != (7, 7) or tuple(stem.conv.stride) != (1, 2, 2) or tuple(stem.conv.padding) != (kt // 2, 3, 3):
        raise AvtError("stem_conv: expected a [kt,7,7] stride-[1,2,2] stem")
    wp = torch.zeros((c, kt, kh, 4, 2, 4))
    for dwp in range(4):
        for p in range(2):
            k = 2 * dwp + p - 1
            if 0 <= k < kw:
                wp[:, :, :, dwp, p, :3] = w[:, :, :, :, k].permute(0, 2, 3, 1)
    if tgroup > 1:
        g = tgroup
        wg = torch.zeros((g, c, kt + g - 1) + tuple(wp.shape[2:]))
        for j in range(g):
            wg[j, :, j : j + kt] = wp
        conv = FusedConv(None, None, True, device,
                         packed=(wg.reshape(g * c, -1), bias.repeat(g), 8, (kt + g - 1, kh, 4), (g, 2, 1),
                                 (kt // 2, 3, 2), (0, 0, 1)), x3=x3)
        conv.tgroup, conv.frame_channels = g, c
        conv.alg_flops_per_row = g * 2.0 * (kt * kh * kw * 3) * c
        conv.frames_per_tile = 2 if (_STEM_FM_X3 and x3 is not None and g == 4 and c == 8) else 0
        fm = conv.frames_per_tile > 0
        conv.wt_lds = stem_lds_image(conv.wt, kt + g - 1, fm) if conv.cout % 32 == 0 else None
        conv.wt_lds_lo = stem_lds_image(conv.wt_lo, kt + g - 1, fm) if conv.cout % 32 == 0 and x3 is not None else None
        conv.wg, conv._merged = (wg, bias) if fm else None, {}
        return conv
    conv = FusedConv(None, None, True, device,
                     packed=(wp.reshape(c, -1), bias, 8, (kt, kh, 4), (1, 2, 1), (kt // 2, 3, 2), (0, 0, 1)), x3=x3)
    conv.tgroup, conv.frame_channels, conv.frames_per_tile = 1, c, 0
    conv.wg, conv._merged = None, {}
    conv.alg_flops_per_row = 2.0 * (kt * kh * kw * 3) * c
    conv.wt_lds = stem_lds_image(conv.wt, kt) if conv.cout % 32 == 0 else None
    conv.wt_lds_lo = stem_lds_image(conv.wt_lo, kt) if conv.cout % 32 == 0 and x3 is not None else None
    return conv


def pack_pw_planes(plane):
    raw = plane.detach().cpu().view(torch.int16)
    n_out, k = raw.shape
    ks = -(-k // 32)
    wp = torch.zeros((n_out, ks * 32), dtype=torch.int16)
    wp[:, :k] = raw
    lane = torch.arange(64)
    n, q = lane & 15, lane >> 4
    e = torch.arange(8)
    shape = (n_out // 16, ks, 64, 8)
    nt = torch.arange(n_out // 16).view(-1, 1, 1, 1)
    row = (32 * (nt // 2) + 8 * (n >> 2).view(1, 1, -1, 1) + 4 * (nt % 2) + (n & 3).view(1, 1, -1, 1)).expand(shape)
    col = (torch.arange(ks).view(1, -1, 1, 1) * 32 + q.view(1, 1, -1, 1) * 8 + e.view(1, 1, 1, -1)).expand(shape)
    return wp[row, col].contiguous().view(torch.bfloat16)


def _bottleneck_fragments(wa, wb, wc, wsc=None, sc_kgroup=0):
    cm, c, cin = wa.shape[0], wc.shape[0], wa.shape[1]
    cmp_ = 16 if cm <= 16 else 32
    first = cin == 8
    nta = cmp_ // 16
    lane = torch.arange(64)
    n, q = lane & 15, lane >> 4
    e = torch.arange(8)
    L, E = n.numel(), e.numel()
    if first:
        wa_p = torch.zeros((cmp_, 8, 4))
        wa_p[:cm, :, :3] = wa[:, :, :, 0, 0]
        wa_f = wa_p[n.view(-1, 1).expand(L, E), e.view(1, -1).expand(L, E), q.view(-1, 1).expand(L, E)].view(1, 1, 1, L, E)
    else:
        wa_p = torch.zeros((cmp_, cin, 3))
        wa_p[:cm] = wa[:, :, :, 0, 0]
        ka = cin // 32
        k_idx = (torch.arange(ka).view(-1, 1, 1, 1) * 32 + q.view(1, 1, -1, 1) * 8 + e.view(1, 1, 1, -1)).expand(ka, nta, L, E)
        r_idx = (torch.arange(nta).view(1, -1, 1, 1) * 16 + n.view(1, 1, -1, 1)).expand(ka, nta, L, E)
        wa_f = torch.stack([wa_p[r_idx, k_idx, dt] for dt in range(3)])
    wb_p = torch.zeros((cmp_, cmp_, 10))
    wb_p[:cm, :cm, :9] = wb[:, :, 0].reshape(cm, cm, 9)
    nb = 5 if cmp_ == 16 else 9
    j = torch.arange(nb).view(-1, 1, 1, 1)
    if cmp_ == 16:
        tap = (2 * j + (q >> 1).view(1, 1, -1, 1)).expand(nb, nta, L, E)
        ch = (8 * (q & 1).view(1, 1, -1, 1) + e.view(1, 1, 1, -1)).expand(nb, nta, L, E)
    else:
        tap = j.expand(nb, nta, L, E)
        ch = (8 * q.view(1, 1, -1, 1) + e.view(1, 1, 1, -1)).expand(nb, nta, L, E)
    rb = (torch.arange(nta).view(1, -1, 1, 1) * 16 + n.view(1, 1, -1, 1)).expand(nb, nta, L, E)
    wb_f = wb_p[rb, ch, tap]
    wc_p = torch.zeros((c, 32))
    wc_p[:, :cm] = wc[:, :, 0, 0, 0]
    nt = torch.arange(c // 16).view(-1, 1, 1)
    chan = (32 * (nt // 2) + 8 * (n >> 2).view(1, -1, 1) + 4 * (nt % 2) + (n & 3).view(1, -1, 1)).expand(c // 16, L, E)
    kk = (q.view(1, -1, 1) * 8 + e.view(1, 1, -1)).expand(c // 16, L, E)
    wc_f = wc_p[chan, kk]
    if wsc is None:
        return wa_f, wb_f, wc_f, None
    ks = max(cin // 32, 1)
    ws_p = torch.zeros((c, ks * 32))
    ws_p[:, 8 * sc_kgroup : 8 * sc_kgroup + cin] = wsc[:, :, 0, 0, 0]
    chan4 = chan.view(c // 16, 1, L, E).expand(c // 16, ks, L, E)
    kk4 = (torch.arange(ks).view(1, -1, 1, 1) * 32 + kk.view(c // 16, 1, L, E)).expand(c // 16, ks, L, E)
    return wa_f, wb_f, wc_f, ws_p[chan4, kk4]


def pack_bottleneck(wa, ba, wb, bb, wc, bc, device, shortcut=None):
    wa, ba, wb, bb, wc, bc = [v.detach().float().cpu() for v in (wa, ba, wb, bb, wc, bc)]
    cmp_ = 16 if wa.shape[0] <= 16 else 32
    wsc = bsc = None
    if shortcut is not None:
        wsc, bsc = [v.detach().float().cpu() for v in shortcut]
    wa_f, wb_f, wc_f, ws_f = _bottleneck_fragments(wa, wb, wc, wsc)
    padw = lambda v: torch.cat([v.float(), torch.zeros(cmp_ - v.numel())])
    dev = lambda v, dt: v.to(dt).contiguous().to(device)
    out = (dev(wa_f, torch.bfloat16), dev(padw(ba), torch.float32), dev(wb_f, torch.bfloat16), dev(padw(bb), torch.float32),
           dev(wc_f, torch.bfloat16))
    if shortcut is None:
        return out + (dev(bc.float(), torch.float32),)
    return out + (dev((bc + bsc).float(), torch.float32), dev(ws_f, torch.bfloat16))


def pack_bottleneck_x3(wa, ba, wb, bb, wc, bc, x3, device, shortcut=None):
    wa, ba, wb, bb, wc, bc = [v.detach().float().cpu() for v in (wa, ba, wb, bb, wc, bc)]
    cm, c = wa.shape[0], wc.shape[0]
    cmp_ = 16 if cm <= 16 else 32
    wsc = bsc = None
    if shortcut is not None:
        wsc, bsc = [v.detach().float().cpu() for v in shortcut]

    def scale_of(*ws):
        if x3 != ops.X3_F16:
            return torch.ones(ws[0].shape[0])
        mx = torch.stack([w.reshape(w.shape[0], -1).abs().amax(dim=1) for w in ws]).amax(dim=0).clamp_min(1e-30)
        return torch.pow(2.0, 9.0 - torch.floor(torch.log2(mx)))

    sa, sb = scale_of(wa), scale_of(wb)
    sc = scale_of(wc, wsc) if wsc is not None else scale_of(wc)
    v5 = lambda s_: s_.view(-1, 1, 1, 1, 1)
    wa_f, wb_f, wc_f, ws_f = _bottleneck_fragments(wa * v5(sa), wb * v5(sb), wc * v5(sc),
                                                    None if wsc is None else wsc * v5(sc),
                                                    sc_kgroup=1 if wa.shape[1] == 8 else 0)
    frags = [wa_f.reshape(-1, 64, 8), wb_f.reshape(-1, 64, 8), wc_f.reshape(-1, 64, 8)]
    if ws_f is not None:
        frags.append(ws_f.reshape(-1, 64, 8))
    allf = torch.cat(frags, 0)
    hi, lo = split_planes(allf, x3)
    wfrag = torch.stack([hi, lo], 1).contiguous().to(device)
    padw = lambda v, fill: torch.cat([v.float(), torch.full((cmp_ - v.numel(),), fill)])
    coef = torch.cat([padw(1.0 / sa, 1.0), padw(ba, 0.0), padw(1.0 / sb, 1.0), padw(bb, 0.0), 1.0 / sc,
                      bc if bsc is None else bc + bsc]).float().contiguous().to(device)
    return wfrag, coef


def pack_c33(wb, device):
    wb = wb.detach().float().cpu()
    cm = wb.shape[0]
    lane = torch.arange(64)
    n, q = lane & 15, lane >> 4
    e = torch.arange(8)
    wb9 = wb[:, :, 0].reshape(cm, cm, 9)
    shape = (9, 2, cm // 16, 64, 8)
    tap = torch.arange(9).view(-1, 1, 1, 1, 1).expand(shape)
    kh = torch.arange(2).view(1, -1, 1, 1, 1)
    nt = torch.arange(cm // 16).view(1, 1, -1, 1, 1)
    row = (32 * (nt // 2) + 8 * (n >> 2).view(1, 1, 1, -1, 1) + 4 * (nt % 2) + (n & 3).view(1, 1, 1, -1, 1)).expand(shape)
    ch = (kh * 32 + q.view(1, 1, 1, -1, 1) * 8 + e.view(1, 1, 1, 1, -1)).expand(shape)
    return wb9[row, ch, tap].to(torch.bfloat16).contiguous().to(device)


def pack_c33_x3(wb, bias, x3, device):
    wb = wb.detach().float().cpu()
    co, ci = wb.shape[0], wb.shape[1]
    w9 = wb[:, :, 0].reshape(co, ci, 9)
    if x3 == ops.X3_F16:
        mx = w9.reshape(co, -1).abs().amax(dim=1).clamp_min(1e-30)
        sc = torch.pow(2.0, 9.0 - torch.floor(torch.log2(mx)))
    else:
        sc = torch.ones(co)
    w9 = w9 * sc.view(-1, 1, 1)
    lane = torch.arange(64)
    rho, kh = lane & 31, lane >> 5
    h = (rho >> 2) & 1
    r = (rho & 3) + 4 * (rho >> 3)
    shape = (9, 4, 2, 64, 8)
    n = torch.arange(2).view(1, 1, -1, 1, 1)
    ch = (32 * n + ((2 * (r >> 3) + h) * 8 + (r & 7)).view(1, 1, 1, -1, 1)).expand(shape)
    kk = (torch.arange(4).view(1, -1, 1, 1, 1) * 16 + (kh * 8).view(1, 1, 1, -1, 1) + torch.arange(8).view(1, 1, 1, 1, -1)).expand(shape)
    tap = torch.arange(9).view(-1, 1, 1, 1, 1).expand(shape)
    frags = w9[ch, kk, tap]
    hi, lo = split_planes(frags, x3)
    wfrag = torch.stack([hi, lo], 3).contiguous().to(device)
    coef = torch.cat([1.0 / sc, bias.detach().float().cpu()]).float().contiguous().to(device)
    return wfrag, coef


def pack_res2_x3(wa, ba, wb, bb, wc, bc, x3, device):
    wa, ba, wb, bb, wc, bc = [v.detach().float().cpu() for v in (wa, ba, wb, bb, wc, bc)]
    cm, c = wa.shape[0], wc.shape[0]
    assert (cm, c) == (64, 256) and wa.shape[1] == c and tuple(wb.shape) == (cm, cm, 1, 3, 3) and wc.shape[1] == cm

    def scale_of(w):
        if x3 != ops.X3_F16:
            return torch.ones(w.shape[0])
        mx = w.reshape(w.shape[0], -1).abs().amax(dim=1).clamp_min(1e-30)
        return torch.pow(2.0, 9.0 - torch.floor(torch.log2(mx)))

    sa, sb, sc = scale_of(wa), scale_of(wb), scale_of(wc)
    a2 = wa.reshape(cm, c) * sa.view(-1, 1)
    b9 = wb[:, :, 0].reshape(cm, cm, 9) * sb.view(-1, 1, 1)
    c2 = wc.reshape(c, cm) * sc.view(-1, 1)

    def frags(mat):
        hi, lo = split_planes(mat, x3)
        return pack_pw_planes(hi), pack_pw_planes(lo)

    pairs = []
    ah, al = frags(a2)
    for jc in range(4):
        for kk in range(2):
            for nt in range(4):
                pairs.append((ah[nt, 2 * jc + kk], al[nt, 2 * jc + kk]))
    for t in range(9):
        bh, bl = frags(b9[:, :, t].contiguous())
        for kk in range(2):
            for nt in range(4):
                pairs.append((bh[nt, kk], bl[nt, kk]))
    ch, cl = frags(c2)
    for jc in range(4):
        for nn in range(4):
            for kk in range(2):
                pairs.append((ch[4 * jc + nn, kk], cl[4 * jc + nn, kk]))
    wfrag = torch.stack([torch.stack([h, l]) for h, l in pairs]).contiguous().to(device)
# ... 490 lines not shown
```

audio-video-textures_amd/ops.py:

```python
import ctypes as C

import numpy as np
import torch

from . import _lib

SIM_BF16, SIM_BF16X3, SIM_F32 = 0, 1, 2
_PREC = {"bf16": SIM_BF16, "bf16x3": SIM_BF16X3, "f32": SIM_F32}
FAST_T, SLOW_T, SLOTS = 32, 8, 40


def _dev(t, name, dtype=None, contiguous=True):
    if not isinstance(t, torch.Tensor) or not t.is_cuda:
        raise _lib.AvtError("%s must be a device (HIP) tensor; the hot path has no CPU fallback" % name)
    if dtype is not None and t.dtype != dtype:
        raise _lib.AvtError("%s must be %s, got %s" % (name, dtype, t.dtype))
    if contiguous and not t.is_contiguous():
        raise _lib.AvtError("%s must be contiguous" % name)
    return t


def _p(t):
    return None if t is None else C.c_void_p(t.data_ptr())

# ... 80 lines not shown

    def chunk(self, parts):
        starts = self.start.chunk(parts) if self.start is not None else [None] * parts
        return [FrameClip(self.hi, self.lo, i.contiguous(), self.plane_dtype, s, self.win_len) for i, s in zip(self.idx.chunk(parts), starts)]

    def record_stream(self, st):
        for t_ in (self.hi, self.lo, self.idx, self.start):
            if t_ is not None:
                t_.record_stream(st)

    def dense(self):
        flat = self.idx.reshape(-1).long()
        shp = self.shape
        return SplitClip(self.hi.index_select(0, flat).view(shp), self.lo.index_select(0, flat).view(shp), self.plane_dtype)

    def float(self):
        return self.dense().float()


X3_BF16, X3_F16 = 0, 1
_X3 = {"bf16x3": X3_BF16, "f16x3": X3_F16}


def clip_pack(frames_u8, win_start, win_len, out_hw=224, mean=0.45, std=0.225, bgr=True,
              dtype=torch.bfloat16, plan=None, layout="ncthw", planes=None):
    _dev(frames_u8, "frames_u8", torch.uint8)
    assert frames_u8.dim() == 4 and frames_u8.shape[3] == 3
    n_frames, h, w, _ = frames_u8.shape
    win_start = np.ascontiguousarray(win_start, np.int32)
    n_win = win_start.shape[0]
    if plan is None:
        off, slot = clip_pack_plan(win_start, win_len, n_frames)
        plan = (torch.from_numpy(off).to(frames_u8.device), torch.from_numpy(slot).to(frames_u8.device))
    d_off, d_slot = plan
    if layout == "ndhwc4":
        if dtype != torch.bfloat16:
            raise _lib.AvtError("clip_pack: layout ndhwc4 is bf16 only")
        mk = lambda t_: torch.empty((n_win, t_, out_hw, out_hw, 4), dtype=dtype, device=frames_u8.device)
        if planes is not None:
            pd = _X3[planes]
            slow, fast = SplitClip(mk(SLOW_T), mk(SLOW_T), pd), SplitClip(mk(FAST_T), mk(FAST_T), pd)
            _lib.check(_lib.lib().avt_clip_pack_u8_ndhwc4_x3(_p(frames_u8), n_frames, h, w, _p(d_off), _p(d_slot), n_win,
                                                             int(out_hw), float(mean), float(std), 1 if bgr else 0,
                                                             _p(slow.hi), _p(slow.lo), _p(fast.hi), _p(fast.lo), pd,
                                                             _stream()), "avt_clip_pack_u8_ndhwc4_x3")
            return slow, fast
        slow, fast = mk(SLOW_T), mk(FAST_T)
        _lib.check(_lib.lib().avt_clip_pack_u8_ndhwc4(_p(frames_u8), n_frames, h, w, _p(d_off), _p(d_slot), n_win,
                                                      int(out_hw), float(mean), float(std), 1 if bgr else 0, _p(slow),
                                                      _p(fast), _stream()), "avt_clip_pack_u8_ndhwc4")
        return slow, fast
    if dtype not in (torch.bfloat16, torch.float32):
        raise _lib.AvtError("clip_pack: dtype must be bfloat16 or float32")
    slow = torch.empty((n_win, 3, SLOW_T, out_hw, out_hw), dtype=dtype, device=frames_u8.device)
    fast = torch.empty((n_win, 3, FAST_T, out_hw, out_hw), dtype=dtype, device=frames_u8.device)
    _lib.check(_lib.lib().avt_clip_pack_u8(_p(frames_u8), n_frames, h, w, _p(d_off), _p(d_slot), n_win, int(out_hw),
                                           float(mean), float(std), 1 if bgr else 0, _p(slow), _p(fast),
                                           1 if dtype == torch.bfloat16 else 0, _stream()), "avt_clip_pack_u8")
    return slow, fast


def clip_pack_frames(frames_u8, win_start, win_len, out_hw=224, mean=0.45, std=0.225, bgr=True, planes="f16x3"):
    _dev(frames_u8, "frames_u8", torch.uint8)
    assert frames_u8.dim() == 4 and frames_u8.shape[3] == 3
    n_frames, h, w, _ = frames_u8.shape
    win_start = np.ascontiguousarray(win_start, np.int64)
    if win_start.size and (win_start.min() < 0 or win_start.max() + win_len > n_frames):
        raise _lib.AvtError("clip_pack_frames: a window leaves the %d frames" % n_frames)
    pd = _X3[planes]
    dev = frames_u8.device
    f = np.arange(n_frames, dtype=np.int32)
    off = np.arange(n_frames + 1, dtype=np.int32)
    slot = (f // SLOW_T) * SLOTS + f % SLOW_T
    n_grp = -(-n_frames // SLOW_T)
    hi = torch.empty((n_grp * SLOW_T, out_hw, out_hw, 4), dtype=torch.bfloat16, device=dev)
    lo = torch.empty_like(hi)
    d_off, d_slot = torch.from_numpy(off).to(dev, non_blocking=True), torch.from_numpy(slot.astype(np.int32)).to(dev, non_blocking=True)
    _lib.check(_lib.lib().avt_clip_pack_u8_ndhwc4_x3(_p(frames_u8), n_frames, h, w, _p(d_off), _p(d_slot), n_grp, int(out_hw),
                                                     float(mean), float(std), 1 if bgr else 0, _p(hi), _p(lo), _p(hi), _p(lo), pd,
                                                     _stream()), "avt_clip_pack_u8_ndhwc4_x3")
    fast_off, slow_off = clip_sample_table(win_len)
    idx_f = torch.from_numpy((win_start[:, None] + fast_off[None, :]).astype(np.int32)).to(dev, non_blocking=True)
    idx_s = torch.from_numpy((win_start[:, None] + slow_off[None, :]).astype(np.int32)).to(dev, non_blocking=True)
    start = torch.from_numpy(win_start.astype(np.int32)).to(dev, non_blocking=True)
    hi, lo = hi[:n_frames], lo[:n_frames]
    return FrameClip(hi, lo, idx_s, pd, start, int(win_len)), FrameClip(hi, lo, idx_f, pd, start, int(win_len))


def clip_pack_gather(frames_u8, win_start_dev, win_len, out_hw=224, mean=0.45, std=0.225, bgr=True, dtype=torch.float32):
    _dev(frames_u8, "frames_u8", torch.uint8)
    _dev(win_start_dev, "win_start", torch.int32)
    n_frames, h, w, _ = frames_u8.shape
    n_win = int(win_start_dev.numel())
    if dtype not in (torch.bfloat16, torch.float32):
        raise _lib.AvtError("clip_pack_gather: dtype must be bfloat16 or float32")
    slow = torch.empty((n_win, 3, SLOW_T, out_hw, out_hw), dtype=dtype, device=frames_u8.device)
    fast = torch.empty((n_win, 3, FAST_T, out_hw, out_hw), dtype=dtype, device=frames_u8.device)
    _lib.check(_lib.lib().avt_clip_pack_gather_u8(_p(frames_u8), n_frames, h, w, _p(win_start_dev), n_win, int(win_len),
                                                  int(out_hw), float(mean), float(std), 1 if bgr else 0, _p(slow), _p(fast),
                                                  1 if dtype == torch.bfloat16 else 0, _stream()), "avt_clip_pack_gather_u8")
    return slow, fast


RESNET_MEAN, RESNET_STD = (0.4345, 0.4051, 0.3775), (0.2768, 0.2713, 0.2737)


def frames_resize_aa_norm(frames_u8, out_hw, mean=RESNET_MEAN, std=RESNET_STD):
    _dev(frames_u8, "frames_u8", torch.uint8)
    if frames_u8.dim() != 4 or frames_u8.shape[3] != 3:
        raise _lib.AvtError("frames_resize_aa_norm: frames_u8 must be [F, H, W, 3]")
    n_frames, h, w, _ = frames_u8.shape
    out = torch.empty((n_frames, 3, int(out_hw), int(out_hw)), dtype=torch.float32, device=frames_u8.device)
    m, s = (C.c_float * 3)(*[float(v) for v in mean]), (C.c_float * 3)(*[float(v) for v in std])
    _lib.check(_lib.lib().avt_frames_resize_aa_norm_u8(_p(frames_u8), n_frames, h, w, int(out_hw), m, s, _p(out), _stream()),
               "avt_frames_resize_aa_norm_u8")
    return out


def clip_gather_frames(table, win_start_dev, win_len):
    _dev(table, "table", torch.float32)
    _dev(win_start_dev, "win_start", torch.int32)
    if table.dim() != 4 or table.shape[1] != 3 or table.shape[2] != table.shape[3]:
        raise _lib.AvtError("clip_gather_frames: table must be [F, 3, hw, hw]")
    n_frames, hw, n_win = int(table.shape[0]), int(table.shape[2]), int(win_start_dev.numel())
    out = torch.empty((n_win, int(win_len), 3, hw, hw), dtype=torch.float32, device=table.device)
    _lib.check(_lib.lib().avt_clip_gather_frames_f32(_p(table), n_frames, hw, _p(win_start_dev), n_win, int(win_len), _p(out),
                                                     _stream()), "avt_clip_gather_frames_f32")
    return out


def negative_sample(mt_state, idx, n_len, n_negs):
    _dev(mt_state, "mt_state", torch.int32)
    _dev(idx, "idx", torch.int64)
    out = torch.empty((idx.numel(), int(n_negs)), dtype=torch.int32, device=idx.device)
    _lib.check(_lib.lib().avt_negative_sample_mt19937(_p(mt_state), _p(idx), int(idx.numel()), int(n_len), int(n_negs),
                                                      _p(out), _stream()), "avt_negative_sample_mt19937")
    return out


def l2norm_rows(x0, x1=None, eps=1e-12, want_f32=True, want_split=False):
    _dev(x0, "x0", torch.float32)
    n, d0 = x0.shape
    d1 = 0
    if x1 is not None:
        _dev(x1, "x1", torch.float32)
        assert x1.shape[0] == n
        d1 = x1.shape[1]
    d = d0 + d1
    y = torch.empty((n, d), dtype=torch.float32, device=x0.device) if want_f32 else None
    hi = torch.empty((n, d), dtype=torch.bfloat16, device=x0.device) if want_split else None
    lo = torch.empty((n, d), dtype=torch.bfloat16, device=x0.device) if want_split else None
    _lib.check(_lib.lib().avt_l2norm_rows(_p(x0), d0, _p(x1), d1, n, float(eps), _p(y), _p(hi), _p(lo), _stream()),
               "avt_l2norm_rows")
    return y, hi, lo


SIM_XL = True
_GEMM_TABS = {}


def _gemm_ktab(k, lda, device):
    key = (int(k), int(lda), str(device))
    tab = _GEMM_TABS.get(key)
    if tab is None:
        tab = torch.from_numpy(conv3d_ktab(int(k), (1, 1, 1), 1, 1, int(lda))).to(device)
        _GEMM_TABS[key] = tab
    return tab


def sim_gemm_nt(q, t, temp, precision="f32", q_lo=None, t_lo=None, out=None, nq_total=None):
    prec = _PREC[precision]
    nq_all = max(int(q.shape[0]), int(t.shape[0])) if nq_total is None else int(nq_total)
    if (SIM_XL and prec == SIM_BF16X3 and q_lo is not None and t_lo is not None and q.dim() == 2 and t.shape[0] % 256 == 0 and
            q.shape[1] % 32 == 0 and 256 <= q.shape[1] <= 8192 and (SIM_XL == "always" or -(-nq_all // 256) * (t.shape[0] // 256) >= 192) and
            (out is None or out.stride(0) % 4 == 0)):
        for name, v in (("q", q), ("q_lo", q_lo), ("t", t), ("t_lo", t_lo)):
            _dev(v, name, torch.bfloat16)
        nq, d = q.shape
        nt = t.shape[0]
        if out is None:
            out = torch.empty((nq, nt), dtype=torch.float32, device=q.device)
        else:
            _dev(out, "out", torch.float32, contiguous=False)
        _lib.check(_lib.lib().avt_gemm_nt_x3_f32out(_p(q), _p(q_lo), d, _p(t), _p(t_lo), _p(out), out.stride(0), nq, nt, d, float(temp),
                                                    _p(_gemm_ktab(d, d, q.device)), X3_BF16, _stream()), "avt_gemm_nt_x3_f32out")
        return out
    want = torch.float32 if prec == SIM_F32 else torch.bfloat16
    _dev(q, "q", want)
    _dev(t, "t", want)
    nq, d = q.shape
    nt = t.shape[0]
    assert t.shape[1] == d
    if prec == SIM_BF16X3:
        _dev(q_lo, "q_lo", torch.bfloat16)
        _dev(t_lo, "t_lo", torch.bfloat16)
    if out is None:
        out = torch.empty((nq, nt), dtype=torch.float32, device=q.device)
    else:
        _dev(out, "out", torch.float32)
    _lib.check(_lib.lib().avt_sim_gemm_nt(_p(q), _p(q_lo), _p(t), _p(t_lo), nq, nt, d, float(temp), prec, _p(out),
                                          out.stride(0), _stream()), "avt_sim_gemm_nt")
    return out


def row_transition(sim, q_ids=None, sim_a=None, alpha=0.5, threshold=0.0, cap=64):
    _dev(sim, "sim", torch.float32)
    nq, nt = sim.shape
    n_seg = 0
    if q_ids is not None:
        _dev(q_ids, "q_ids", torch.int64)
        n_seg = nt
    if sim_a is not None:
        _dev(sim_a, "sim_a", torch.float32)
        assert sim_a.shape == sim.shape
    dev = sim.device
    idx = torch.full((nq, cap), -1, dtype=torch.int32, device=dev)
    seg = torch.full((nq, cap), -1, dtype=torch.int32, device=dev)
    p = torch.zeros((nq, cap), dtype=torch.float32, device=dev)
    cnt = torch.zeros((nq,), dtype=torch.int32, device=dev)
    stats = torch.zeros((nq, 4), dtype=torch.float32, device=dev)
    _lib.check(_lib.lib().avt_row_transition(_p(sim), nq, nt, sim.stride(0), _p(q_ids), n_seg, _p(sim_a),
                                             sim_a.stride(0) if sim_a is not None else 0, float(alpha),
                                             float(threshold), int(cap), _p(idx), _p(seg), _p(p), _p(cnt), _p(stats),
                                             _stream()), "avt_row_transition")
    return dict(idx=idx, seg=seg, p=p, cnt=cnt, stats=stats)


def row_topk(sim, k, self_col=None):
    _dev(sim, "sim", torch.float32)
    nq, nt = sim.shape
    if self_col is not None:
        _dev(self_col, "self_col", torch.int64)
    idx = torch.empty((nq, k), dtype=torch.int32, device=sim.device)
    val = torch.empty((nq, k), dtype=torch.float32, device=sim.device)
    _lib.check(_lib.lib().avt_row_topk(_p(sim), nq, nt, sim.stride(0), _p(self_col), int(k), _p(idx), _p(val),
                                       _stream()), "avt_row_topk")
    return idx, val


def softmax_ce_fwd(logits, label=None):
    _dev(logits, "logits", torch.float32)
    b, c = logits.shape
    if label is not None:
        _dev(label, "label", torch.int64)
    loss = torch.empty((b,), dtype=torch.float32, device=logits.device)
    prob = torch.empty((b, c), dtype=torch.float32, device=logits.device)
    _lib.check(_lib.lib().avt_softmax_ce_fwd(_p(logits), b, c, _p(label), _p(loss), _p(prob), _stream()),
               "avt_softmax_ce_fwd")
    return loss, prob


def softmax_ce_bwd(prob, label=None, scale=1.0):
    _dev(prob, "prob", torch.float32)
    b, c = prob.shape
    d = torch.empty_like(prob)
    _lib.check(_lib.lib().avt_softmax_ce_bwd(_p(prob), _p(label), b, c, float(scale), _p(d), _stream()),
               "avt_softmax_ce_bwd")
    return d


def conv3d_ktab(cin, kernel, h, w, ldi):
    kt, kh, kw = kernel
    n_entries = 8 * ((kt * kh * kw * cin + 63) // 64) + 2
    tab = np.empty((n_entries, 2), np.int32)
    _lib.check(_lib.lib().avt_conv3d_ktab(int(cin), kt, kh, kw, int(h), int(w), int(ldi), tab.ctypes.data, n_entries),
               "avt_conv3d_ktab")
    return tab


def conv3d_wfrag_supported(cin, cout, kernel):
    return bool(_lib.lib().avt_conv3d_igemm_wfrag_supported(int(cin), int(cout), *[int(k) for k in kernel]))


def conv3d_igemm(x_ptr, wt, bias, res_ptr, out_ptr, ktab, dims, cin, cout, kernel, stride, pad, ldi, ldo, ldr, relu,
                 out_dims=(0, 0, 0), out_rows=None, wfrag=None):
    b, t, h, w = dims
    if wfrag is not None:
        _dev(wfrag, "wfrag", torch.bfloat16)
        orr = out_rows if out_rows is not None else (1, 0, 0)
        _lib.check(_lib.lib().avt_conv3d_igemm_wfrag_bf16(C.c_void_p(x_ptr), _p(wt), _p(bias),
                                                          C.c_void_p(res_ptr) if res_ptr else None, C.c_void_p(out_ptr),
                                                          _p(ktab), b, t, h, w, int(cin), int(cout), *kernel, *stride, *pad,
                                                          *out_dims, int(ldi), int(ldo), int(ldr), 1 if relu else 0,
                                                          int(orr[0]), int(orr[1]), int(orr[2]), _p(wfrag),
                                                          int(wfrag.shape[1]), _stream()),
                   "avt_conv3d_igemm_wfrag_bf16")
        return
    if out_rows is not None:
        _lib.check(_lib.lib().avt_conv3d_igemm_rows_bf16(C.c_void_p(x_ptr), _p(wt), _p(bias),
                                                         C.c_void_p(res_ptr) if res_ptr else None, C.c_void_p(out_ptr),
                                                         _p(ktab), b, t, h, w, int(cin), int(cout), *kernel, *stride, *pad,
                                                         *out_dims, int(ldi), int(ldo), int(ldr), 1 if relu else 0,
                                                         int(out_rows[0]), int(out_rows[1]), int(out_rows[2]), _stream()),
                   "avt_conv3d_igemm_rows_bf16")
        return
    _lib.check(_lib.lib().avt_conv3d_igemm_bf16(C.c_void_p(x_ptr), _p(wt), _p(bias),
                                                C.c_void_p(res_ptr) if res_ptr else None, C.c_void_p(out_ptr), _p(ktab),
                                                b, t, h, w, int(cin), int(cout), *kernel, *stride, *pad, *out_dims,
                                                int(ldi), int(ldo), int(ldr), 1 if relu else 0, _stream()),
               "avt_conv3d_igemm_bf16")


def conv3d_igemm_x3(x_ptrs, wt_hi, wt_lo, bias, res_ptrs, out_ptrs, ktab, dims, cin, cout, kernel, stride, pad, ldi, ldo,
                    ldr, relu, plane_dtype, wscale=None, out_dims=(0, 0, 0), out_rows=None, wblk=False):
    b, t, h, w = dims
    _dev(wt_hi, "wt_hi", torch.bfloat16)
    _dev(wt_lo, "wt_lo", torch.bfloat16)
    orr = out_rows if out_rows is not None else (1, 0, 0)
    rh, rl = res_ptrs if res_ptrs is not None else (0, 0)
    fn = _lib.lib().avt_conv3d_igemm_x3_wblk if wblk else _lib.lib().avt_conv3d_igemm_x3
    _lib.check(fn(C.c_void_p(x_ptrs[0]), C.c_void_p(x_ptrs[1]), _p(wt_hi), _p(wt_lo), _p(bias),
                                              C.c_void_p(rh) if rh else None, C.c_void_p(rl) if rl else None,
                                              C.c_void_p(out_ptrs[0]), C.c_void_p(out_ptrs[1]), _p(ktab), b, t, h, w,
                                              int(cin), int(cout), *kernel, *stride, *pad, *out_dims, int(ldi), int(ldo),
                                              int(ldr), int(relu), int(orr[0]), int(orr[1]), int(orr[2]),
                                              int(plane_dtype), _p(wscale), _stream()), "avt_conv3d_igemm_x3_wblk" if wblk else "avt_conv3d_igemm_x3")


def conv3d_igemm_x3_f32(x, wt_hi, wt_lo, wscale, out, ktab, dims, cin, cout, kernel, stride, pad, ldi, ldo, plane_dtype, add=None):
    b, t, h, w = dims
    _dev(x, "x", torch.float32)
    _dev(out, "out", torch.float32)
    _dev(wt_hi, "wt_hi", torch.bfloat16)
    _dev(wt_lo, "wt_lo", torch.bfloat16)
    if add is not None:
        _dev(add, "add", torch.float32)
    _lib.check(_lib.lib().avt_conv3d_igemm_x3_f32(_p(x), _p(wt_hi), _p(wt_lo), _p(wscale), _p(add), _p(out), _p(ktab), int(b), int(t),
                                                  int(h), int(w), int(cin), int(cout), *[int(k) for k in kernel],
                                                  *[int(v) for v in stride], *[int(v) for v in pad], int(ldi), int(ldo),
                                                  int(cout), int(plane_dtype), _stream()), "avt_conv3d_igemm_x3_f32")


def conv3d_igemm_x3_f32_stats(x, wt_hi, wt_lo, wscale, out, ktab, dims, cin, cout, kernel, stride, pad, ldi, ldo, plane_dtype, groups, stat_c):
    b, t, h, w = dims
    _dev(x, "x", torch.float32)
    _dev(out, "out", torch.float32)
    _dev(wt_hi, "wt_hi", torch.bfloat16)
    _dev(wt_lo, "wt_lo", torch.bfloat16)
    k = int(kernel[0]) * int(kernel[1]) * int(kernel[2]) * int(cin)
    m = out.numel() // int(cout)
    rows = _lib.lib().avt_conv3d_igemm_x3_f32_stat_rows(int(cout), k, int(m), int(groups))
    if rows <= 0:
        raise _lib.AvtError("conv3d_igemm_x3_f32_stats: %d rows do not split into %d groups" % (m, groups))
    pre_rows = rows * max(1, int(stat_c) // 1024)
    ws = torch.empty(_lib.lib().avt_bn_train_ws_bytes_pre(int(stat_c), int(groups), pre_rows), dtype=torch.uint8, device=x.device)
    _lib.check(_lib.lib().avt_conv3d_igemm_x3_f32_stats(_p(x), _p(wt_hi), _p(wt_lo), _p(wscale), _p(out), _p(ktab), int(b), int(t), int(h),
                                                        int(w), int(cin), int(cout), *[int(v) for v in kernel], *[int(v) for v in stride],
                                                        *[int(v) for v in pad], int(ldi), int(ldo), int(plane_dtype), _p(ws), int(groups),
                                                        int(stat_c), _stream()), "avt_conv3d_igemm_x3_f32_stats")
    return ws, pre_rows


def pw_x3_f32_supported(k, n):
    return bool(_lib.lib().avt_pw_x3_f32_supported(int(k), int(n)))


def pw_x3_f32(x, k, wt_hi, wt_lo, wscale, out, n, plane_dtype, add=None):
    _dev(x, "x", torch.float32)
    _dev(out, "out", torch.float32)
    _dev(wt_hi, "wt_hi", torch.bfloat16)
    _dev(wt_lo, "wt_lo", torch.bfloat16)
    if add is not None:
        _dev(add, "add", torch.float32)
    m = x.numel() // k
    _lib.check(_lib.lib().avt_pw_x3_f32(_p(x), int(k), int(k), _p(wt_hi), _p(wt_lo), _p(wscale), _p(add), int(n), _p(out), int(n), int(n),
                                        int(m), int(plane_dtype), _stream()), "avt_pw_x3_f32")


def conv3d_igemm_x3_f32_bwdstats(dy, wt_hi, wt_lo, out, ktab, dims, cin, cout, kernel, pad, plane_dtype, bn, groups, stat_c, add=None):
    b, t, h, w = dims
    _dev(dy, "dy", torch.float32)
    _dev(out, "out", torch.float32)
    k = int(kernel[0]) * int(kernel[1]) * int(kernel[2]) * int(cin)
    m = out.numel() // int(cout)
    rows = _lib.lib().avt_conv3d_igemm_x3_f32_bwdstats_rows(int(cout), k, int(m), int(groups))
    if rows <= 0:
        return None
    bx, mean, invstd, gamma, beta, mask, relu = bn
    pre_rows = rows * max(1, int(stat_c) // 1024)
    ws = torch.empty(_lib.lib().avt_bn_train_ws_bytes_pre(int(stat_c), int(groups), pre_rows), dtype=torch.uint8, device=dy.device)
    _lib.check(_lib.lib().avt_conv3d_igemm_x3_f32_bwdstats(
        _p(dy), _p(wt_hi), _p(wt_lo), None, _p(add), _p(out), _p(ktab), int(b), int(t), int(h), int(w), int(cin), int(cout),
        *[int(v) for v in kernel], *[int(v) for v in pad], int(cin), int(cout), int(cout), int(plane_dtype), _p(bx), _p(mean), _p(invstd),
        _p(gamma), _p(beta), _p(mask), int(relu), _p(ws), int(groups), int(stat_c), _stream()), "avt_conv3d_igemm_x3_f32_bwdstats")
    return ws, pre_rows


def pw_x3_f32_bwdstats(dy, k, wt_hi, wt_lo, out, n, plane_dtype, bn, groups, add=None):
    _dev(dy, "dy", torch.float32)
    _dev(out, "out", torch.float32)
    m = dy.numel() // k
    rows = _lib.lib().avt_pw_x3_f32_bwdstats_rows(int(k), int(n), int(m), int(groups))
    if rows <= 0 or plane_dtype != X3_BF16:
        return None
    bx, mean, invstd, gamma, beta, mask, relu = bn
    pre_rows = rows * max(1, int(n) // 1024)
    ws = torch.empty(_lib.lib().avt_bn_train_ws_bytes_pre(int(n), int(groups), pre_rows), dtype=torch.uint8, device=dy.device)
    _lib.check(_lib.lib().avt_pw_x3_f32_bwdstats(_p(dy), int(k), int(k), _p(wt_hi), _p(wt_lo), _p(add), int(n), _p(out), int(n), int(n), int(m),
                                                 int(plane_dtype), _p(bx), _p(mean), _p(invstd), _p(gamma), _p(beta), _p(mask),
                                                 1 if relu else 0, _p(ws), int(groups), _stream()), "avt_pw_x3_f32_bwdstats")
    return ws, pre_rows


def pw_x3_f32_stats(x, k, wt_hi, wt_lo, wscale, out, n, plane_dtype, groups):
    _dev(x, "x", torch.float32)
    _dev(out, "out", torch.float32)
    _dev(wt_hi, "wt_hi", torch.bfloat16)
    _dev(wt_lo, "wt_lo", torch.bfloat16)
    m = x.numel() // k
    rows = _lib.lib().avt_pw_x3_f32_stat_rows(int(k), int(n), int(m), int(groups))
    if rows <= 0 or n & (n - 1):
        return None
    pre_rows = rows * max(1, int(n) // 1024)
    ws = torch.empty(_lib.lib().avt_bn_train_ws_bytes_pre(int(n), int(groups), pre_rows), dtype=torch.uint8, device=x.device)
    _lib.check(_lib.lib().avt_pw_x3_f32_stats(_p(x), int(k), int(k), _p(wt_hi), _p(wt_lo), _p(wscale), _p(out), int(n), int(n), int(m),
                                              int(plane_dtype), _p(ws), int(groups), _stream()), "avt_pw_x3_f32_stats")
    return ws, pre_rows


def conv3d_igemm_x3_f32_ex(x, wt_hi, wt_lo, wscale, out, ktab, dims, cin, cout, kernel, pad, out_dims, ldi, ldo, plane_dtype,
                           out_rows=(1, 0, 0)):
    b, t, h, w = dims
    _dev(x, "x", torch.float32)
    _dev(wt_hi, "wt_hi", torch.bfloat16)
    _dev(wt_lo, "wt_lo", torch.bfloat16)
    _lib.check(_lib.lib().avt_conv3d_igemm_x3_f32_ex(_p(x), _p(wt_hi), _p(wt_lo), _p(wscale), C.c_void_p(out.data_ptr()), _p(ktab), int(b),
                                                     int(t), int(h), int(w), int(cin), int(cout), *[int(k) for k in kernel],
                                                     *[int(v) for v in pad], *[int(v) for v in out_dims], int(ldi), int(ldo),
                                                     int(out_rows[0]), int(out_rows[1]), int(out_rows[2]), int(plane_dtype), _stream()),
               "avt_conv3d_igemm_x3_f32_ex")


def weight_planes_f32(w2d, plane_dtype):
    _dev(w2d, "w", torch.float32)
    cout, k = w2d.shape
    hi = torch.empty((cout, k), dtype=torch.bfloat16, device=w2d.device)
    lo = torch.empty_like(hi)
    ws = torch.empty(cout, dtype=torch.float32, device=w2d.device) if plane_dtype == X3_F16 else None
    _lib.check(_lib.lib().avt_weight_planes_f32(_p(w2d), int(cout), int(k), _p(hi), _p(lo), _p(ws), int(plane_dtype), _stream()),
               "avt_weight_planes_f32")
    return hi, lo, ws


def weight_planes_gather_f32(w, idx_map, plane_dtype):
    _dev(w, "w", torch.float32, contiguous=False)
    _dev(idx_map, "idx_map", torch.int32)
    rows, k = idx_map.shape
    hi = torch.empty((rows, k), dtype=torch.bfloat16, device=w.device)
    lo = torch.empty_like(hi)
    ws = torch.empty(rows, dtype=torch.float32, device=w.device) if plane_dtype == X3_F16 else None
    _lib.check(_lib.lib().avt_weight_planes_gather_f32(C.c_void_p(w.data_ptr()), _p(idx_map), int(rows), int(k), _p(hi), _p(lo), _p(ws),
                                                       int(plane_dtype), _stream()), "avt_weight_planes_gather_f32")
    return hi, lo, ws


def conv_x3_set_small_tile(on):
    return int(_lib.lib().avt_conv_x3_set_small_tile(int(bool(on))))


def weight_planes_job_bytes():
    return int(_lib.lib().avt_weight_planes_job_bytes())


def weight_planes_multi(jobs, blk2job, nblocks):
    assert jobs.is_cuda and blk2job.is_cuda and blk2job.dtype == torch.int32 and blk2job.numel() == nblocks
    _lib.check(_lib.lib().avt_weight_planes_multi(_p(jobs), _p(blk2job), int(nblocks), _stream()), "avt_weight_planes_multi")


def sgd_job_bytes():
    return int(_lib.lib().avt_sgd_job_bytes())


def sgd_multi(jobs, blk2job, nblocks, hyper):
    assert jobs.is_cuda and blk2job.is_cuda and blk2job.dtype == torch.int32 and blk2job.numel() == nblocks
    assert hyper.is_cuda and hyper.dtype == torch.float32 and hyper.is_contiguous() and hyper.shape[-1] == 4
    _lib.check(_lib.lib().avt_sgd_multi(_p(jobs), _p(blk2job), int(nblocks), _p(hyper), _stream()), "avt_sgd_multi")


def sgd_upload(dst, src_pinned, nbytes):
    assert dst.is_cuda and dst.is_contiguous() and not src_pinned.is_cuda and src_pinned.is_pinned() and src_pinned.is_contiguous()
    assert 0 < nbytes <= min(dst.numel() * dst.element_size(), src_pinned.numel() * src_pinned.element_size())
    _lib.check(_lib.lib().avt_sgd_upload(_p(dst), _p(src_pinned), int(nbytes), _stream()), "avt_sgd_upload")


def pack_job_bytes():
    return int(_lib.lib().avt_pack_job_bytes())


def grad_pack_multi(jobs, blk2job, nblocks, scale):
    assert jobs.is_cuda and blk2job.is_cuda and blk2job.dtype == torch.int32 and blk2job.numel() == nblocks
    assert scale.is_cuda and scale.dtype == torch.float32 and scale.numel() == 1
    _lib.check(_lib.lib().avt_grad_pack_multi(_p(jobs), _p(blk2job), int(nblocks), _p(scale), _stream()), "avt_grad_pack_multi")


def weight_planes_t_f32(w3d, sel):
    _dev(w3d, "w", torch.float32)
    cout, taps, cin = w3d.shape
    hi = torch.empty((cin, len(sel) * cout), dtype=torch.bfloat16, device=w3d.device)
    lo = torch.empty_like(hi)
    arr = (C.c_int32 * len(sel))(*[int(v) for v in sel])
    _lib.check(_lib.lib().avt_weight_planes_t_f32(_p(w3d), int(cout), int(taps), int(cin), arr, len(sel), _p(hi), _p(lo), _stream()),
               "avt_weight_planes_t_f32")
    return hi, lo


def conv3d_wgrad_x3_f32(dy, x, dw, dims, cin, cout, kernel, stride, pad, ldx, ldy):
    b, t, h, w = dims
    _dev(dy, "dy", torch.float32)
    _dev(x, "x", torch.float32)
    _dev(dw, "dw", torch.float32)
    _lib.check(_lib.lib().avt_conv3d_wgrad_x3_f32(_p(dy), _p(x), _p(dw), int(b), int(t), int(h), int(w), int(cin), int(cout),
                                                  *[int(k) for k in kernel], *[int(v) for v in stride], *[int(v) for v in pad],
                                                  int(ldx), int(ldy), _stream()), "avt_conv3d_wgrad_x3_f32")


def conv3d_wgrad_x3_sub_f32(dy, x, dw, dims, cin, cout, kernel, stride, pad, out_dims, ldx, ldy, ldw, zero_dw):
    b, t, h, w = dims
    _dev(dy, "dy", torch.float32)
    _dev(x, "x", torch.float32)
    _lib.check(_lib.lib().avt_conv3d_wgrad_x3_sub_f32(_p(dy), _p(x), C.c_void_p(dw.data_ptr()), int(b), int(t), int(h), int(w),
                                                      int(cin), int(cout), *[int(k) for k in kernel], *[int(v) for v in stride],
                                                      *[int(v) for v in pad], *[int(v) for v in out_dims], int(ldx), int(ldy),
                                                      int(ldw), int(bool(zero_dw)), _stream()), "avt_conv3d_wgrad_x3_sub_f32")


def stem_conv_x3(x_ptrs, wt_hi, wt_lo, bias, wscale, out_ptrs, batch, t, h, pw, cout, kt, st, pt, plane_dtype, relu=True,
                 frames_per_tile=0, frame_idx=None, table_frames=0):
    _dev(wt_hi, "wt_hi", torch.bfloat16)
    _dev(wt_lo, "wt_lo", torch.bfloat16)
    if frame_idx is not None:
        _dev(frame_idx, "frame_idx", torch.int32)
        if frame_idx.numel() != batch * t:
            raise _lib.AvtError("stem_conv_x3: frame_idx has %d entries, expected batch * t = %d" % (frame_idx.numel(), batch * t))
    _lib.check(_lib.lib().avt_stem_conv_x3(C.c_void_p(x_ptrs[0]), C.c_void_p(x_ptrs[1]), _p(wt_hi), _p(wt_lo), _p(bias),
                                           _p(wscale), C.c_void_p(out_ptrs[0]), C.c_void_p(out_ptrs[1]), int(batch), int(t),
                                           int(h), int(pw), int(cout), int(kt), int(st), int(pt), int(bool(relu)),
                                           int(plane_dtype), int(frames_per_tile), _p(frame_idx), int(table_frames), _stream()),
               "avt_stem_conv_x3")


def lateral_x3_supported(cin, cout, kt):
    return bool(_lib.lib().avt_lateral_x3_supported(int(cin), int(cout), int(kt)))


def lateral_x3(x_ptrs, ldx, cin, w_hi, w_lo, bias, wscale, y_ptrs, ldy, cout, batch, t, hw, kt, st, pt, relu, plane_dtype):
    _dev(w_hi, "w_hi", torch.bfloat16)
    _dev(w_lo, "w_lo", torch.bfloat16)
    _lib.check(_lib.lib().avt_lateral_x3(C.c_void_p(x_ptrs[0]), C.c_void_p(x_ptrs[1]), int(ldx), int(cin), _p(w_hi), _p(w_lo), _p(bias),
                                         _p(wscale), C.c_void_p(y_ptrs[0]), C.c_void_p(y_ptrs[1]), int(ldy), int(cout), int(batch),
                                         int(t), int(hw), int(kt), int(st), int(pt), int(relu), int(plane_dtype), _stream()),
               "avt_lateral_x3")


def stem_conv_x3_merged(x_ptrs, wt_hi, wt_lo, bias, wscale, out_ptrs, batch, t, h, pw, cout, kt, st, pt, plane_dtype, tap_frames,
                        tap_tiles, ktm, table_frames, relu=True):
    _dev(wt_hi, "wt_hi", torch.bfloat16)
    _dev(wt_lo, "wt_lo", torch.bfloat16)
    _dev(tap_frames, "tap_frames", torch.int32)
    _dev(tap_tiles, "tap_tiles", torch.int32)
    _lib.check(_lib.lib().avt_stem_conv_x3_merged(C.c_void_p(x_ptrs[0]), C.c_void_p(x_ptrs[1]), _p(wt_hi), _p(wt_lo), _p(bias),
                                                  _p(wscale), C.c_void_p(out_ptrs[0]), C.c_void_p(out_ptrs[1]), int(batch), int(t),
                                                  int(h), int(pw), int(cout), int(kt), int(st), int(pt), int(bool(relu)),
                                                  int(plane_dtype), _p(tap_frames), _p(tap_tiles), int(ktm), int(table_frames),
                                                  _stream()), "avt_stem_conv_x3_merged")


def clip_planes_f32(x, plane_dtype):
    _dev(x, "x", torch.float32, contiguous=False)
    if x.dim() != 5 or x.shape[1] != 3:
        raise _lib.AvtError("clip_planes_f32: expected [B, 3, T, H, W], got %s" % (tuple(x.shape),))
    b, _, t, h, w = x.shape
    hi = torch.empty((b, t, h, w, 4), dtype=torch.bfloat16, device=x.device)
    lo = torch.empty_like(hi)
    sb, sc, st, sh, sw = x.stride()
    _lib.check(_lib.lib().avt_clip_planes_f32(_p(x), b, t, h, w, sb, sc, st, sh, sw, _p(hi), _p(lo), int(plane_dtype), _stream()),
               "avt_clip_planes_f32")
    return hi, lo


def stem_conv_x3_f32(x_hi, x_lo, wt_hi, wt_lo, wscale, out, batch, t, h, pw, cout, kt, st, pt, tgroup, plane_dtype, frames_per_tile=0):
    _dev(wt_hi, "wt_hi", torch.bfloat16)
    _dev(wt_lo, "wt_lo", torch.bfloat16)
    _dev(out, "out", torch.float32, contiguous=False)
    _lib.check(_lib.lib().avt_stem_conv_x3_f32(_p(x_hi), _p(x_lo), _p(wt_hi), _p(wt_lo), _p(wscale), _p(out), int(batch), int(t),
                                               int(h), int(pw), int(cout), int(kt), int(st), int(pt), int(tgroup),
                                               int(plane_dtype), int(frames_per_tile), _stream()), "avt_stem_conv_x3_f32")


def stem_wgrad_x3_supported(h, pw, cout, kt):
    return bool(_lib.lib().avt_stem_wgrad_x3_supported(int(h), int(pw), int(cout), int(kt)))


def stem_wgrad_x3(x_hi, x_lo, dy, batch, t, h, pw, cout, kt, pt):
    _dev(dy, "dy", torch.float32, contiguous=False)
    dw = torch.zeros((cout, kt, 7, 4, 8), dtype=torch.float32, device=dy.device)
    _lib.check(_lib.lib().avt_stem_wgrad_x3(_p(x_hi), _p(x_lo), _p(dy), _p(dw), int(batch), int(t), int(h), int(pw), int(cout),
                                            int(kt), int(pt), _stream()), "avt_stem_wgrad_x3")
    return dw


def pw_x3_supported(k, n):
    return bool(_lib.lib().avt_pw_x3_supported(int(k), int(n)))


def pw_x3(x_ptrs, ldx, k, w_hi, w_lo, bias, wscale, res_ptrs, ldr, y_ptrs, ldy, n, m, relu, plane_dtype):
    _dev(w_hi, "w_hi", torch.bfloat16)
    _dev(w_lo, "w_lo", torch.bfloat16)
    rh, rl = res_ptrs if res_ptrs is not None else (0, 0)
    _lib.check(_lib.lib().avt_pw_x3(C.c_void_p(x_ptrs[0]), C.c_void_p(x_ptrs[1]), int(ldx), int(k), _p(w_hi), _p(w_lo),
                                    _p(bias), _p(wscale), C.c_void_p(rh) if rh else None, C.c_void_p(rl) if rl else None,
                                    int(ldr), C.c_void_p(y_ptrs[0]), C.c_void_p(y_ptrs[1]), int(ldy), int(n), int(m),
                                    1 if relu else 0, int(plane_dtype), _stream()), "avt_pw_x3")


def pw_chain_x3_supported(k1, n1, n2):
    return bool(_lib.lib().avt_pw_chain_x3_supported(int(k1), int(n1), int(n2)))


def pw_chain_x3(x_ptrs, ldx, k1, w1, bias1, wscale1, res_ptrs, ldr, y_ptrs, ldy, n1, relu1, w2, bias2, wscale2, z_ptrs, ldz, n2, m,
                plane_dtype):
    rh, rl = res_ptrs if res_ptrs is not None else (0, 0)
    _lib.check(_lib.lib().avt_pw_chain_x3(C.c_void_p(x_ptrs[0]), C.c_void_p(x_ptrs[1]), int(ldx), int(k1), _p(w1[0]), _p(w1[1]),
                                          _p(bias1), _p(wscale1), C.c_void_p(rh) if rh else None, C.c_void_p(rl) if rl else None,
                                          int(ldr), C.c_void_p(y_ptrs[0]), C.c_void_p(y_ptrs[1]), int(ldy), int(n1),
                                          1 if relu1 else 0, _p(w2[0]), _p(w2[1]), _p(bias2), _p(wscale2), C.c_void_p(z_ptrs[0]),
                                          C.c_void_p(z_ptrs[1]), int(ldz), int(n2), int(m), int(plane_dtype), _stream()),
               "avt_pw_chain_x3")


def maxpool_hw3s2_x3(x_ptrs, out_ptrs, bt, h, w, c, ldi, ldo, plane_dtype, tgroup=1, frame_idx=None):
    if frame_idx is not None:
        _dev(frame_idx, "frame_idx", torch.int32)
        if frame_idx.numel() != bt:
            raise _lib.AvtError("maxpool_hw3s2_x3: frame_idx has %d entries, expected %d" % (frame_idx.numel(), bt))
    _lib.check(_lib.lib().avt_maxpool_hw3s2_ndhwc_x3(C.c_void_p(x_ptrs[0]), C.c_void_p(x_ptrs[1]), C.c_void_p(out_ptrs[0]),
                                                     C.c_void_p(out_ptrs[1]), int(bt), int(h), int(w), int(c), int(ldi),
                                                     int(ldo), int(tgroup), int(plane_dtype), _p(frame_idx), _stream()),
               "avt_maxpool_hw3s2_ndhwc_x3")


def maxpool_hw2s2_x3(x_ptrs, out_ptrs, bt, h, w, c, ldi, ldo, plane_dtype):
    _lib.check(_lib.lib().avt_maxpool_hw2s2_ndhwc_x3(C.c_void_p(x_ptrs[0]), C.c_void_p(x_ptrs[1]), C.c_void_p(out_ptrs[0]),
                                                     C.c_void_p(out_ptrs[1]), int(bt), int(h), int(w), int(c), int(ldi),
                                                     int(ldo), int(plane_dtype), _stream()), "avt_maxpool_hw2s2_ndhwc_x3")


def maxpool3d_k3s2_x3(x_ptrs, out_ptrs, batch, t, h, w, c, ldi, ldo, plane_dtype):
    _lib.check(_lib.lib().avt_maxpool3d_k3s2_ndhwc_x3(C.c_void_p(x_ptrs[0]), C.c_void_p(x_ptrs[1]), C.c_void_p(out_ptrs[0]),
                                                      C.c_void_p(out_ptrs[1]), int(batch), int(t), int(h), int(w), int(c),
                                                      int(ldi), int(ldo), int(plane_dtype), _stream()), "avt_maxpool3d_k3s2_ndhwc_x3")


def mean_positions_x3(x_ptrs, batch, p, c, ldi, out, col0, plane_dtype):
    _dev(out, "out", torch.float32)
    _lib.check(_lib.lib().avt_mean_positions_x3(C.c_void_p(x_ptrs[0]), C.c_void_p(x_ptrs[1]), int(batch), int(p), int(c),
                                                int(ldi), C.c_void_p(out.data_ptr() + 4 * int(col0)), int(out.shape[1]),
                                                int(plane_dtype), _stream()), "avt_mean_positions_x3")


def maxpool_hw3s2(x_ptr, out_ptr, bt, h, w, c, ldi, ldo, tgroup=1):
    _lib.check(_lib.lib().avt_maxpool_hw3s2_ndhwc_bf16(C.c_void_p(x_ptr), C.c_void_p(out_ptr), int(bt), int(h), int(w),
                                                       int(c), int(ldi), int(ldo), int(tgroup), _stream()),
               "avt_maxpool_hw3s2_ndhwc_bf16")


def stem_conv_supported(h, pw, cout):
    return bool(_lib.lib().avt_stem_conv_supported(int(h), int(pw), int(cout)))


def stem_conv(x_ptr, wt, bias, out_ptr, batch, t, h, pw, cout, kt, st, pt, relu=True):
    _dev(wt, "wt", torch.bfloat16)
    _dev(bias, "bias", torch.float32)
    _lib.check(_lib.lib().avt_stem_conv_bf16(C.c_void_p(x_ptr), _p(wt), _p(bias), C.c_void_p(out_ptr), int(batch), int(t),
                                             int(h), int(pw), int(cout), int(kt), int(st), int(pt), int(bool(relu)),
                                             _stream()), "avt_stem_conv_bf16")


def stem_conv_pool(x_ptr, wt, bias, out_ptr, batch, t, h, pw, cout, kt, st, pt, tgroup, ldo):
    _dev(wt, "wt", torch.bfloat16)
    _dev(bias, "bias", torch.float32)
    _lib.check(_lib.lib().avt_stem_conv_pool_bf16(C.c_void_p(x_ptr), _p(wt), _p(bias), C.c_void_p(out_ptr), int(batch),
                                                  int(t), int(h), int(pw), int(cout), int(kt), int(st), int(pt),
                                                  int(tgroup), int(ldo), _stream()), "avt_stem_conv_pool_bf16")


def bottleneck_fused_supported(c, w):
    return bool(_lib.lib().avt_bottleneck_fused_supported(int(c), int(w)))


def bottleneck_fused(x_ptr, out_ptr, packed, batch, t, h, w, c, tchunk=8):
    wa, ba, wb, bb, wc, bc = packed
    _lib.check(_lib.lib().avt_bottleneck_fused_bf16(C.c_void_p(x_ptr), C.c_void_p(out_ptr), _p(wa), _p(ba), _p(wb), _p(bb),
                                                    _p(wc), _p(bc), int(batch), int(t), int(h), int(w), int(c),
                                                    int(tchunk), _stream()), "avt_bottleneck_fused_bf16")


def conv3d_igemm_x3_xl_picked(cout, k, m):
    return bool(_lib.lib().avt_conv3d_igemm_x3_xl_picked(int(cout), int(k), int(m)))


def conv33_x3_supported(cin, cout):
    return bool(_lib.lib().avt_conv33_x3_supported(int(cin), int(cout)))


def conv33_x3(x_ptrs, packed, out_ptrs, batch, t, h, w, ldi, ldo, plane_dtype, relu=True):
    wfrag, coef = packed
    _dev(wfrag, "wfrag", torch.bfloat16)
    _dev(coef, "coef", torch.float32)
    _lib.check(_lib.lib().avt_conv33_x3(C.c_void_p(x_ptrs[0]), C.c_void_p(x_ptrs[1]), _p(wfrag), _p(coef), C.c_void_p(out_ptrs[0]),
                                        C.c_void_p(out_ptrs[1]), int(batch), int(t), int(h), int(w), int(ldi), int(ldo),
                                        int(bool(relu)), int(plane_dtype), _stream()), "avt_conv33_x3")


def res2_x3_supported(c, cm, w):
    return bool(_lib.lib().avt_res2_x3_supported(int(c), int(cm), int(w)))


def res2_x3(x_ptrs, ldi, out_ptrs, ldo, packed, batch, t, h, w, plane_dtype):
    wfrag, coef = packed
    _dev(wfrag, "wfrag", torch.bfloat16)
    _dev(coef, "coef", torch.float32)
    if wfrag.numel() * 2 != _lib.lib().avt_res2_x3_wfrag_bytes():
        raise _lib.AvtError("res2_x3: wfrag holds %d bytes, the kernel streams %d" % (wfrag.numel() * 2, _lib.lib().avt_res2_x3_wfrag_bytes()))
    clip_bytes = int(t) * int(h) * int(w) * max(int(ldi), int(ldo)) * 2
    ranges = -(-int(batch) * clip_bytes // ((1 << 32) - 65)) if clip_bytes > 0 else 1
    per = -(-int(batch) // max(ranges, 1))
    for b0 in range(0, int(batch), max(per, 1)):
        nb = min(per, int(batch) - b0)
        xo, oo = b0 * t * h * w * int(ldi) * 2, b0 * t * h * w * int(ldo) * 2
        _lib.check(_lib.lib().avt_res2_x3(C.c_void_p(x_ptrs[0] + xo), C.c_void_p(x_ptrs[1] + xo), C.c_void_p(out_ptrs[0] + oo),
                                          C.c_void_p(out_ptrs[1] + oo), _p(wfrag), _p(coef), nb, int(t), int(h), int(w), int(ldi), int(ldo),
                                          int(plane_dtype), _stream()), "avt_res2_x3")


def bneck_x3_supported(cin, c, w):
    return bool(_lib.lib().avt_bneck_x3_supported(int(cin), int(c), int(w)))


def bneck_x3(x_ptrs, out_ptrs, packed, batch, t, h, w, cin, c, plane_dtype, tchunk=16):
    wfrag, coef = packed
    _dev(wfrag, "wfrag", torch.bfloat16)
    _dev(coef, "coef", torch.float32)
    _lib.check(_lib.lib().avt_bneck_x3(C.c_void_p(x_ptrs[0]), C.c_void_p(x_ptrs[1]), C.c_void_p(out_ptrs[0]),
                                       C.c_void_p(out_ptrs[1]), _p(wfrag), _p(coef), int(batch), int(t), int(h), int(w),
                                       int(cin), int(c), int(tchunk), int(plane_dtype), _stream()), "avt_bneck_x3")


def mean_positions(x_ptr, batch, p, c, ldi, out, col0=0):
    _dev(out, "out", torch.float32)
    _lib.check(_lib.lib().avt_mean_positions_bf16(C.c_void_p(x_ptr), int(batch), int(p), int(c), int(ldi),
                                                  C.c_void_p(out.data_ptr() + 4 * int(col0)), int(out.shape[1]), _stream()),
               "avt_mean_positions_bf16")


def bottleneck_first_supported(cin, c, w):
    return bool(_lib.lib().avt_bottleneck_first_supported(int(cin), int(c), int(w)))


def bottleneck_first(x_ptr, out_ptr, packed, batch, t, h, w, cin, c, tchunk=8):
    wa, ba, wb, bb, wc, bc, wsc = packed
    _lib.check(_lib.lib().avt_bottleneck_first_bf16(C.c_void_p(x_ptr), C.c_void_p(out_ptr), _p(wa), _p(ba), _p(wb), _p(bb),
                                                    _p(wc), _p(wsc), _p(bc), int(batch), int(t), int(h), int(w), int(cin),
                                                    int(c), int(tchunk), _stream()), "avt_bottleneck_first_bf16")


def conv33_c64_supported(cin, cout, w):
    return bool(_lib.lib().avt_conv33_c64_supported(int(cin), int(cout), int(w)))


def conv33_c64(x_ptr, wb, bias, out_ptr, batch, t, h, w, ldo, relu=True):
    _dev(wb, "wb", torch.bfloat16)
    _dev(bias, "bias", torch.float32)
    _lib.check(_lib.lib().avt_conv33_c64_bf16(C.c_void_p(x_ptr), _p(wb), _p(bias), C.c_void_p(out_ptr), int(batch), int(t),
                                              int(h), int(w), int(ldo), int(bool(relu)), _stream()), "avt_conv33_c64_bf16")


def pw_chain_supported(k1, n1, n2, has_res, k2x=0):
    return bool(_lib.lib().avt_pw_chain_supported(int(k1), int(n1), int(n2), int(bool(has_res)), int(k2x)))


def pw_chain(x1_ptr, ldx, k1, w1, b1, res_ptr, ldr, y_ptr, ldy, n1, w2, b2, z_ptr, ldz, n2, m, x2_ptr=0, ldx2=0, k2x=0):
    _dev(w1, "w1", torch.bfloat16)
    _dev(w2, "w2", torch.bfloat16)
    _dev(b1, "b1", torch.float32)
    _dev(b2, "b2", torch.float32)
    _lib.check(_lib.lib().avt_pw_chain_bf16(C.c_void_p(x1_ptr), int(ldx), int(k1), _p(w1), _p(b1),
                                            C.c_void_p(res_ptr) if res_ptr else None, int(ldr), C.c_void_p(y_ptr), int(ldy),
                                            int(n1), C.c_void_p(x2_ptr) if x2_ptr else None, int(ldx2), int(k2x), _p(w2),
                                            _p(b2), C.c_void_p(z_ptr), int(ldz), int(n2), int(m), _stream()),
               "avt_pw_chain_bf16")


def maxpool_hw2s2(x_ptr, out_ptr, bt, h, w, c, ldi, ldo):
    _lib.check(_lib.lib().avt_maxpool_hw2s2_ndhwc_bf16(C.c_void_p(x_ptr), C.c_void_p(out_ptr), int(bt), int(h), int(w),
                                                       int(c), int(ldi), int(ldo), _stream()),
               "avt_maxpool_hw2s2_ndhwc_bf16")


def pairwise_l2(x):
    _dev(x, "x", torch.float32)
    n, d = x.shape
    out = torch.empty((n, n), dtype=torch.float32, device=x.device)
    _lib.check(_lib.lib().avt_pairwise_l2_f32(_p(x), int(n), int(d), _p(out), _stream()), "avt_pairwise_l2_f32")
    return out


def diag_filter(d1, w):
    _dev(d1, "d1", torch.float32)
    _dev(w, "w", torch.float32)
    n, fs = d1.shape[0], int(w.numel())
    out = torch.empty((n - fs + 1, n - fs + 1), dtype=torch.float32, device=d1.device)
    _lib.check(_lib.lib().avt_diag_filter_f32(_p(d1), int(n), _p(w), fs, _p(out), _stream()), "avt_diag_filter_f32")
    return out


def q_learning_supported(n):
    return bool(_lib.lib().avt_q_learning_supported(int(n)))


def q_learning(d3, alpha, tol=10e-3, max_iter=1000):
    _dev(d3, "d3", torch.float32)
    n = d3.shape[0]
    assert d3.shape[1] == n
    out = torch.empty_like(d3)
    iters = torch.zeros(1, dtype=torch.int32, device=d3.device)
    _lib.check(_lib.lib().avt_q_learning_f32(_p(d3), int(n), float(alpha), float(tol), int(max_iter), _p(out), _p(iters),
                                             _stream()), "avt_q_learning_f32")
    return out, iters


def logmel(wave, window, melmat, hop, fft_len, log_offset):
    if wave.dtype not in (torch.float32, torch.float64):
        raise _lib.AvtError("logmel: waveform must be float32 or float64, got %s" % wave.dtype)
    _dev(wave, "wave", wave.dtype)
    _dev(window, "window", torch.float64)
    _dev(melmat, "melmat", torch.float64)
    win, n_mel = int(window.numel()), int(melmat.shape[1])
    if melmat.shape[0] != fft_len // 2 + 1:
        raise _lib.AvtError("logmel: melmat has %d rows, fft_len/2+1 = %d" % (melmat.shape[0], fft_len // 2 + 1))
    n = int(wave.numel())
    n_frames = 1 + (n - win) // hop if n >= win else 0
    out = torch.empty((n_frames, n_mel), dtype=torch.float64, device=wave.device)
    _lib.check(_lib.lib().avt_logmel_f64(_p(wave), int(wave.dtype == torch.float64), n, _p(window), win, int(hop),
                                         int(fft_len), _p(melmat), n_mel, float(log_offset), _p(out), _stream()),
               "avt_logmel_f64")
    return out


def logmel_examples(lm, ex_len, ex_hop):
    _dev(lm, "logmel", torch.float64)
    n_frames, n_mel = int(lm.shape[0]), int(lm.shape[1])
    n_ex = 1 + (n_frames - ex_len) // ex_hop if n_frames >= ex_len else 0
    out = torch.empty((n_ex, ex_len, n_mel), dtype=torch.float32, device=lm.device)
    _lib.check(_lib.lib().avt_logmel_examples_f32(_p(lm), n_frames, n_mel, int(ex_len), int(ex_hop), _p(out),
                                                  _stream()), "avt_logmel_examples_f32")
    return out


def infonce_fwd(q, t, temp, eps=1e-12):
    _dev(q, "q", torch.float32)
    _dev(t, "t", torch.float32)
    b, n, d = t.shape
    logits = torch.empty((b, n), dtype=torch.float32, device=q.device)
    inv_q = torch.empty((b,), dtype=torch.float32, device=q.device)
    inv_t = torch.empty((b, n), dtype=torch.float32, device=q.device)
    _lib.check(_lib.lib().avt_infonce_fwd(_p(q), _p(t), b, n, d, float(temp), float(eps), _p(logits), _p(inv_q), _p(inv_t),
                                          _stream()), "avt_infonce_fwd")
    return logits, inv_q, inv_t


def infonce_bwd(q, t, logits, dlogits, inv_q, inv_t, temp):
    b, n, d = t.shape
    dq = torch.empty_like(q)
    dt = torch.empty_like(t)
    _lib.check(_lib.lib().avt_infonce_bwd(_p(q), _p(t), _p(logits), _p(_dev(dlogits.contiguous(), "dlogits", torch.float32)),
                                          _p(inv_q), _p(inv_t), b, n, d, float(temp), _p(dq), _p(dt), _stream()),
               "avt_infonce_bwd")
    return dq, dt


def _mean3(mean):
    return (C.c_float * 3)(*[float(m) for m in mean])


def interp_pack_pair(frame0, frame1, mean, img, x_ptrs, plane_dtype):
    _dev(frame0, "frame0", torch.uint8)
    _dev(frame1, "frame1", torch.uint8)
    _dev(img, "img", torch.float32)
    h, w = frame0.shape[0], frame0.shape[1]
    _lib.check(_lib.lib().avt_interp_pack_pair_u8(_p(frame0), _p(frame1), int(h), int(w), _mean3(mean), _p(img), C.c_void_p(x_ptrs[0]),
                                                  C.c_void_p(x_ptrs[1]), int(plane_dtype), _stream()), "avt_interp_pack_pair_u8")


def avgpool2_x3(x_ptrs, dims, c, ldi, y_ptrs, ldo, plane_dtype):
    b, h, w = dims
    _lib.check(_lib.lib().avt_avgpool2_x3(C.c_void_p(x_ptrs[0]), C.c_void_p(x_ptrs[1]), int(b), int(h), int(w), int(c), int(ldi),
                                          C.c_void_p(y_ptrs[0]), C.c_void_p(y_ptrs[1]), int(ldo), int(plane_dtype), _stream()),
               "avt_avgpool2_x3")


def upsample2_bilinear_x3(x_ptrs, dims, c, ldi, y_ptrs, ldo, plane_dtype):
    b, h, w = dims
    _lib.check(_lib.lib().avt_upsample2_bilinear_x3(C.c_void_p(x_ptrs[0]), C.c_void_p(x_ptrs[1]), int(b), int(h), int(w), int(c),
                                                    int(ldi), C.c_void_p(y_ptrs[0]), C.c_void_p(y_ptrs[1]), int(ldo), int(plane_dtype),
                                                    _stream()), "avt_upsample2_bilinear_x3")


def interp_mid_input(img, flow_ptrs, h, w, sf, x_ptrs, ft, plane_dtype):
    _dev(img, "img", torch.float32)
    _dev(ft, "ft", torch.float32)
    _lib.check(_lib.lib().avt_interp_mid_input(_p(img), C.c_void_p(flow_ptrs[0]), C.c_void_p(flow_ptrs[1]), int(h), int(w), int(sf),
                                               C.c_void_p(x_ptrs[0]), C.c_void_p(x_ptrs[1]), _p(ft), int(plane_dtype), _stream()),
               "avt_interp_mid_input")


def interp_final(img, ft, o_ptrs, h, w, sf, mean, out, plane_dtype):
    _dev(img, "img", torch.float32)
    _dev(ft, "ft", torch.float32)
    _dev(out, "out", torch.uint8)
    _lib.check(_lib.lib().avt_interp_final_u8(_p(img), _p(ft), C.c_void_p(o_ptrs[0]), C.c_void_p(o_ptrs[1]), int(h), int(w), int(sf),
                                              _mean3(mean), _p(out), int(plane_dtype), _stream()), "avt_interp_final_u8")
```

include/avt.h:

```cpp
#ifndef AVT_H
#define AVT_H

#include <stddef.h>
#include <stdint.h>

#ifdef __cplusplus
extern "C" {
#endif

#define AVT_ABI_VERSION 8

typedef enum {
  AVT_OK = 0,
  AVT_ERR_ARG = -1,
  AVT_ERR_UNSUPPORTED = -2,
  AVT_ERR_LAUNCH = -3,
  AVT_ERR_DEVICE = -4
} avt_status;

#define AVT_SIM_BF16    0
#define AVT_SIM_BF16X3  1
#define AVT_SIM_F32     2

#define AVT_DT_F32   0
#define AVT_DT_BF16  1

#define AVT_FAST_T 32
#define AVT_SLOW_T 8
#define AVT_SLOTS  (AVT_FAST_T + AVT_SLOW_T)

int avt_abi_version(void);
const char* avt_last_error(void);
int avt_device_check(char* name, size_t name_len);


int avt_clip_sample_table(int win_len, int32_t* fast_idx, int32_t* slow_idx);

int avt_clip_pack_plan(const int32_t* win_start, int n_win, int win_len,
                       int n_frames, int32_t* dst_off, int32_t* dst_slot);

int avt_clip_pack_u8(const uint8_t* frames, int n_frames, int height, int width,
                     const int32_t* dst_off, const int32_t* dst_slot, int n_win,
                     int out_hw, float mean, float std, int bgr,
                     void* slow, void* fast, int out_dtype, void* stream);

int avt_clip_pack_u8_ndhwc4(const uint8_t* frames, int n_frames, int height,
                            int width, const int32_t* dst_off,
                            const int32_t* dst_slot, int n_win, int out_hw,
                            float mean, float std, int bgr, void* slow,
                            void* fast, void* stream);

int avt_l2norm_rows(const float* x0, int d0, const float* x1, int d1, int64_t n,
                    float eps, float* y_f32, void* y_hi, void* y_lo,
                    void* stream);

int avt_sim_gemm_nt(const void* q, const void* q_lo, const void* t,
                    const void* t_lo, int64_t nq, int64_t nt, int d, float temp,
                    int precision, float* out, int64_t ldo, void* stream);
int avt_gemm_nt_x3_f32out(const void* a_hi, const void* a_lo, int lda, const void* b_hi, const void* b_lo, float* out, int64_t ldo,
                          int m, int n, int k, float divisor, const int32_t* ktab, int plane_dtype, void* stream);

int avt_row_transition(const float* sim, int64_t nq, int64_t nt, int64_t ld,
                       const int64_t* q_ids, int64_t n_seg, const float* sim_a,
                       int64_t ld_a, float alpha, float threshold, int cap,
                       int32_t* surv_idx, int32_t* surv_seg, float* surv_p,
                       int32_t* surv_cnt, float* stats, void* stream);

int avt_row_topk(const float* sim, int64_t nq, int64_t nt, int64_t ld,
                 const int64_t* self_col, int k, int32_t* top_idx,
                 float* top_val, void* stream);

int avt_softmax_ce_fwd(const float* logits, int64_t b, int64_t c,
                       const int64_t* label, float* loss, float* prob,
                       void* stream);
int avt_softmax_ce_bwd(const float* prob, const int64_t* label, int64_t b,
                       int64_t c, float scale, float* dlogits, void* stream);

int avt_infonce_fwd(const float* q, const float* t, int64_t b, int n, int d,
                    float temp, float eps, float* logits, float* inv_q,
                    float* inv_t, void* stream);
int avt_infonce_bwd(const float* q, const float* t, const float* logits,
                    const float* dlogits, const float* inv_q, const float* inv_t,
                    int64_t b, int n, int d, float temp, float* dq, float* dt,
                    void* stream);

int avt_conv3d_ktab(int cin, int kt, int kh, int kw, int h, int w, int ldi,
                    int32_t* ktab, int n_entries);
int avt_conv3d_igemm_bf16(const void* in, const void* wt, const float* bias,
                          const void* res, void* out, const int32_t* ktab,
                          int batch, int t, int h, int w, int cin, int cout,
                          int kt, int kh, int kw, int st, int sh, int sw,
                          int pt, int ph, int pw, int to, int ho, int wo,
                          int ldi, int ldo, int ldr, int relu, void* stream);
int avt_conv3d_igemm_rows_bf16(const void* in, const void* wt, const float* bias,
                               const void* res, void* out, const int32_t* ktab,
                               int batch, int t, int h, int w, int cin, int cout,
                               int kt, int kh, int kw, int st, int sh, int sw,
                               int pt, int ph, int pw, int to, int ho, int wo,
                               int ldi, int ldo, int ldr, int relu,
                               int out_row_stride, int out_h, int out_w, void* stream);

int avt_conv3d_igemm_wfrag_supported(int cin, int cout, int kt, int kh, int kw);
int avt_conv3d_igemm_wfrag_bf16(const void* in, const void* wt, const float* bias,
                                const void* res, void* out, const int32_t* ktab,
                                int batch, int t, int h, int w, int cin, int cout,
                                int kt, int kh, int kw, int st, int sh, int sw,
                                int pt, int ph, int pw, int to, int ho, int wo,
                                int ldi, int ldo, int ldr, int relu,
                                int out_row_stride, int out_h, int out_w,
                                const void* wfrag, int nup, void* stream);

int avt_maxpool_hw3s2_ndhwc_bf16(const void* in, void* out, int bt, int h, int w,
                                 int c, int ldi, int ldo, int tgroup, void* stream);

int avt_mean_positions_bf16(const void* in, int batch, int p, int c, int ldi,
                            float* out, int ldo, void* stream);

int avt_maxpool_hw2s2_ndhwc_bf16(const void* in, void* out, int bt, int h, int w,
                                 int c, int ldi, int ldo, void* stream);

int avt_stem_conv_supported(int h, int pw, int cout);
int avt_stem_conv_bf16(const void* in, const void* wt, const float* bias, void* out,
                       int batch, int t, int h, int pw, int cout, int kt, int st, int pt,
                       int relu, void* stream);
int avt_stem_conv_pool_bf16(const void* in, const void* wt, const float* bias, void* out,
                            int batch, int t, int h, int pw, int cout, int kt, int st, int pt,
                            int tgroup, int ldo, void* stream);

int avt_bottleneck_fused_supported(int c, int w);
int avt_bottleneck_first_supported(int cin, int c, int w);
int avt_bottleneck_first_bf16(const void* x, void* out, const void* wa, const float* ba,
                              const void* wb, const float* bb, const void* wc, const void* wsc,
                              const float* bc, int batch, int t, int h, int w, int cin, int c,
                              int tchunk, void* stream);
int avt_bottleneck_fused_bf16(const void* x, void* out, const void* wa, const float* ba,
                              const void* wb, const float* bb, const void* wc, const float* bc,
                              int batch, int t, int h, int w, int c, int tchunk, void* stream);

#define AVT_X3_BF16 0
#define AVT_X3_F16  1
int avt_conv3d_igemm_x3(const void* in_hi, const void* in_lo, const void* wt_hi, const void* wt_lo,
                        const float* bias, const void* res_hi, const void* res_lo, void* out_hi, void* out_lo,
                        const int32_t* ktab, int batch, int t, int h, int w, int cin, int cout,
                        int kt, int kh, int kw, int st, int sh, int sw, int pt, int ph, int pw,
                        int to, int ho, int wo, int ldi, int ldo, int ldr, int relu,
                        int out_row_stride, int out_h, int out_w, int plane_dtype, const float* wscale,
                        void* stream);
int avt_conv3d_igemm_x3_xl_picked(int cout, int k, int m);
int avt_conv3d_igemm_x3_wblk(const void* in_hi, const void* in_lo, const void* wt_hi, const void* wt_lo,
                             const float* bias, const void* res_hi, const void* res_lo, void* out_hi, void* out_lo,
                             const int32_t* ktab, int batch, int t, int h, int w, int cin, int cout, int kt, int kh,
                             int kw, int st, int sh, int sw, int pt, int ph, int pw, int to, int ho, int wo, int ldi,
                             int ldo, int ldr, int relu, int out_row_stride, int out_h, int out_w, int plane_dtype,
                             const float* wscale, void* stream);
int avt_conv33_x3_supported(int cin, int cout);
int avt_conv33_x3(const void* x_hi, const void* x_lo, const void* wfrag, const float* coef, void* out_hi, void* out_lo,
                  int batch, int t, int h, int w, int ldi, int ldo, int relu, int plane_dtype, void* stream);

int avt_bneck_x3_supported(int cin, int c, int w);
int avt_bneck_x3(const void* x_hi, const void* x_lo, void* out_hi, void* out_lo, const void* wfrag, const float* coef,
                 int batch, int t, int h, int w, int cin, int c, int tchunk, int plane_dtype, void* stream);

int avt_res2_x3_supported(int c, int cm, int w);
int avt_res2_x3_wfrag_bytes(void);
int avt_res2_x3(const void* x_hi, const void* x_lo, void* out_hi, void* out_lo, const void* wfrag, const float* coef, int batch,
                int t, int h, int w, int ldi, int ldo, int plane_dtype, void* stream);

int avt_pw_x3_supported(int k, int n);
int avt_pw_x3(const void* x_hi, const void* x_lo, int ldx, int k, const void* w_hi, const void* w_lo,
              const float* bias, const float* wscale, const void* res_hi, const void* res_lo, int ldr,
              void* y_hi, void* y_lo, int ldy, int n, int64_t m, int relu, int plane_dtype, void* stream);
int avt_pw_x3_f32_supported(int k, int n);
int avt_pw_x3_f32(const float* x, int ldx, int k, const void* w_hi, const void* w_lo, const float* wscale, const float* add, int lda,
                  float* y, int ldy, int n, int64_t m, int plane_dtype, void* stream);
int avt_pw_chain_x3_supported(int k1, int n1, int n2);
int avt_pw_chain_x3(const void* x_hi, const void* x_lo, int ldx, int k1, const void* w1_hi, const void* w1_lo, const float* bias1,
                    const float* wscale1, const void* res_hi, const void* res_lo, int ldr, void* y_hi, void* y_lo, int ldy,
                    int n1, int relu1, const void* w2_hi, const void* w2_lo, const float* bias2, const float* wscale2,
                    void* z_hi, void* z_lo, int ldz, int n2, int64_t m, int plane_dtype, void* stream);
int avt_lateral_x3_supported(int cin, int cout, int kt);
int avt_lateral_x3(const void* x_hi, const void* x_lo, int ldx, int cin, const void* w_hi, const void* w_lo, const float* bias,
                   const float* wscale, void* y_hi, void* y_lo, int ldy, int cout, int batch, int t, int hw, int kt, int st,
                   int pt, int relu, int plane_dtype, void* stream);
int avt_stem_conv_x3(const void* in_hi, const void* in_lo, const void* wt_hi, const void* wt_lo, const float* bias,
                     const float* wscale, void* out_hi, void* out_lo, int batch, int t, int h, int pw, int cout,
                     int kt, int st, int pt, int relu, int plane_dtype, int frames_per_tile, const int32_t* frame_idx,
                     int n_table_frames, void* stream);
int avt_stem_conv_x3_merged(const void* in_hi, const void* in_lo, const void* wt_hi, const void* wt_lo, const float* bias,
                            const float* wscale, void* out_hi, void* out_lo, int batch, int t, int h, int pw, int cout,
                            int kt, int st, int pt, int relu, int plane_dtype, const int32_t* tap_frames,
                            const int32_t* tap_tiles, int ktm, int n_table_frames, void* stream);
int avt_clip_pack_u8_ndhwc4_x3(const uint8_t* frames, int n_frames, int height, int width,
                               const int32_t* dst_off, const int32_t* dst_slot, int n_win, int out_hw,
                               float mean, float std, int bgr, void* slow_hi, void* slow_lo,
                               void* fast_hi, void* fast_lo, int plane_dtype, void* stream);
int avt_maxpool_hw2s2_ndhwc_x3(const void* in_hi, const void* in_lo, void* out_hi, void* out_lo, int bt, int h, int w, int c,
                               int ldi, int ldo, int plane_dtype, void* stream);
int avt_maxpool_hw3s2_ndhwc_x3(const void* in_hi, const void* in_lo, void* out_hi, void* out_lo, int bt, int h,
                               int w, int c, int ldi, int ldo, int tgroup, int plane_dtype, const int32_t* frame_idx,
                               void* stream);
int avt_maxpool3d_k3s2_ndhwc_x3(const void* in_hi, const void* in_lo, void* out_hi, void* out_lo, int batch, int t, int h,
                                int w, int c, int ldi, int ldo, int plane_dtype, void* stream);
int avt_mean_positions_x3(const void* in_hi, const void* in_lo, int batch, int p, int c, int ldi,
                          float* out, int ldo, int plane_dtype, void* stream);

int avt_negative_sample_mt19937(uint32_t* mt_state, const int64_t* idx, int batch, int n_len, int n_negs,
                                int32_t* neg_out, void* stream);
int avt_clip_pack_gather_u8(const uint8_t* frames, int n_frames, int height, int width,
                            const int32_t* win_start, int n_win, int win_len, int out_hw, float mean,
                            float std, int bgr, void* slow, void* fast, int out_dtype, void* stream);
int avt_frames_resize_aa_norm_u8(const uint8_t* frames, int n_frames, int height, int width, int out_hw, const float* mean,
                                 const float* std, float* out, void* stream);
int avt_clip_gather_frames_f32(const float* table, int n_frames, int out_hw, const int32_t* win_start, int n_win, int win_len,
                               float* out, void* stream);

int64_t avt_bn_train_ws_bytes(int64_t m, int c, int groups);
int avt_bn_train_fwd(const float* x, const float* res, float* y, int64_t m, int c, const float* gamma,
                     const float* beta, float eps, float momentum, int relu, int groups, void* ws, int64_t ws_size,
                     float* save_mean, float* save_invstd, float* running_mean, float* running_var,
                     int64_t* num_batches_tracked , void* relu_mask, int64_t ldy,
                     void* stream);
int avt_bn_train_bwd(const float* dy, const float* y, const float* x, int64_t m, int c, const float* gamma,
                     const float* beta, const float* save_mean, const float* save_invstd, int relu, int groups,
                     const void* relu_mask, void* ws, int64_t ws_size, float* dx, float* dres, float* dgamma, float* dbeta,
                     int64_t ld_dy, void* stream);

int avt_conv3d_igemm_x3_f32(const float* in, const void* wt_hi, const void* wt_lo, const float* wscale, const float* add,
                            float* out, const int32_t* ktab, int batch, int t, int h, int w, int cin, int cout, int kt,
                            int kh, int kw, int st, int sh, int sw, int pt, int ph, int pw, int ldi, int ldo, int lda,
                            int plane_dtype, void* stream);
int avt_conv_x3_set_small_tile(int on);
int avt_conv3d_igemm_x3_f32_stat_rows(int cout, int k, int64_t m, int groups);
int avt_conv3d_igemm_x3_f32_stats(const float* in, const void* wt_hi, const void* wt_lo, const float* wscale, float* out,
                                  const int32_t* ktab, int batch, int t, int h, int w, int cin, int cout, int kt, int kh, int kw,
                                  int st, int sh, int sw, int pt, int ph, int pw, int ldi, int ldo, int plane_dtype,
                                  void* stat_part, int groups, int stat_c, void* stream);
int avt_conv3d_igemm_x3_f32_bwdstats_rows(int cout, int k, int64_t m, int groups);
int avt_conv3d_igemm_x3_f32_bwdstats(const float* in, const void* wt_hi, const void* wt_lo, const float* wscale, const float* add,
                                     float* out, const int32_t* ktab, int batch, int t, int h, int w, int cin, int cout, int kt,
                                     int kh, int kw, int pt, int ph, int pw, int ldi, int ldo, int lda, int plane_dtype,
                                     const float* bn_x, const float* bn_mean, const float* bn_invstd, const float* bn_gamma,
                                     const float* bn_beta, const void* bn_mask, int relu, void* stat_part, int groups, int stat_c,
                                     void* stream);
int avt_pw_x3_f32_bwdstats_rows(int k, int n, int64_t m, int groups);
int avt_pw_x3_f32_bwdstats(const float* x, int ldx, int k, const void* w_hi, const void* w_lo, const float* add, int lda, float* y,
                           int ldy, int n, int64_t m, int plane_dtype, const float* bn_x, const float* bn_mean,
                           const float* bn_invstd, const float* bn_gamma, const float* bn_beta, const void* bn_mask, int relu,
                           void* stat_part, int groups, void* stream);
int avt_bn_train_bwd_pre(const float* g, const float* x, int64_t m, int c, const float* gamma, const float* save_mean,
                         const float* save_invstd, int groups, void* ws, int64_t ws_size, int pre_rows, float* dx, float* dgamma,
                         float* dbeta, void* stream);
int avt_pw_x3_f32_stat_rows(int k, int n, int64_t m, int groups);
int avt_pw_x3_f32_stats(const float* x, int ldx, int k, const void* w_hi, const void* w_lo, const float* wscale, float* y, int ldy,
                        int n, int64_t m, int plane_dtype, void* stat_part, int groups, void* stream);
int64_t avt_bn_train_ws_bytes_pre(int c, int groups, int pre_rows);
int avt_bn_train_fwd_pre(const float* x, const float* res, float* y, int64_t m, int c, const float* gamma, const float* beta,
                         float eps, float momentum, int relu, int groups, void* ws, int64_t ws_size, float* save_mean,
                         float* save_invstd, float* running_mean, float* running_var, int64_t* num_batches_tracked,
                         void* relu_mask, int64_t ldy, int pre_rows, void* stream);
int avt_conv3d_igemm_x3_f32_ex(const float* in, const void* wt_hi, const void* wt_lo, const float* wscale, float* out,
                               const int32_t* ktab, int batch, int t, int h, int w, int cin, int cout, int kt, int kh, int kw,
                               int pt, int ph, int pw, int to, int ho, int wo, int ldi, int ldo, int out_row_stride, int out_h,
                               int out_w, int plane_dtype, void* stream);

int avt_conv3d_wgrad_x3_f32(const float* dy, const float* x, float* dw, int batch, int t, int h, int w, int cin, int cout,
                            int kt, int kh, int kw, int st, int sh, int sw, int pt, int ph, int pw, int ldx, int ldy,
                            void* stream);
int avt_wgrad_x3_set_xl(int on);
int avt_conv3d_wgrad_x3_sub_f32(const float* dy, const float* x, float* dw, int batch, int t, int h, int w, int cin, int cout,
                                int kt, int kh, int kw, int st, int sh, int sw, int pt, int ph, int pw, int to, int ho, int wo,
                                int ldx, int ldy, int ldw, int zero_dw, void* stream);

int avt_clip_planes_f32(const float* in, int batch, int t, int h, int w, int64_t sb, int64_t sc, int64_t st, int64_t sh,
                        int64_t sw, void* out_hi, void* out_lo, int plane_dtype, void* stream);
int avt_stem_conv_x3_f32(const void* in_hi, const void* in_lo, const void* wt_hi, const void* wt_lo, const float* wscale,
                         float* out, int batch, int t, int h, int pw, int cout, int kt, int st, int pt, int tgroup,
                         int plane_dtype, int frames_per_tile , void* stream);
int avt_stem_wgrad_x3_supported(int h, int pw, int cout, int kt);
int avt_stem_wgrad_x3(const void* x_hi, const void* x_lo, const float* dy, float* dw, int batch, int t, int h, int pw,
                      int cout, int kt, int pt, void* stream);

int avt_weight_planes_f32(const float* w, int cout, int k, void* hi, void* lo, float* wscale, int plane_dtype, void* stream);
int avt_weight_planes_gather_f32(const float* w, const int32_t* map, int rows, int k, void* hi, void* lo, float* wscale,
                                 int plane_dtype, void* stream);
int avt_weight_planes_t_f32(const float* w, int cout, int taps, int cin, const int32_t* sel, int nsel, void* hi, void* lo,
                            void* stream);
typedef struct AvtPlaneJob {
  const float* w;
  void* hi;
  void* lo;
  float* wscale;
  const int32_t* map;
  int32_t kind;
  int32_t f16;
  int32_t rows, k;
  int32_t cout, taps, cin, nsel;
  int32_t gx, gy;
  int32_t blk0;
  int32_t pad_;
  int32_t sel[32];
} AvtPlaneJob;
int avt_weight_planes_job_bytes(void);
int avt_weight_planes_multi(const void* jobs, const int32_t* blk2job, int nblocks, void* stream);

typedef struct AvtSgdJob {
  float* p;
  const float* g;
  float* buf;
  int64_t numel;
  int32_t group;
  int32_t blk0;
} AvtSgdJob;
int avt_sgd_job_bytes(void);
int avt_sgd_multi(const void* jobs, const int32_t* blk2job, int nblocks, const float* hyper, void* stream);
int avt_sgd_upload(void* dst, const void* src_host, int64_t nbytes, void* stream);

typedef struct AvtPackJob {
  const float* src;
  float* dst;
  int64_t numel;
  int32_t blk0;
  int32_t pad;
} AvtPackJob;
int avt_pack_job_bytes(void);
int avt_grad_pack_multi(const void* jobs, const int32_t* blk2job, int nblocks, const float* scale, void* stream);

int avt_maxpool_train_fwd(const float* x, float* y, void* tap, int bt, int h, int w, int c, int64_t ldy, void* stream);
int avt_maxpool_train_bwd(const float* dy, const void* tap, float* dx, int bt, int h, int w, int c, int64_t ld_dy, void* stream);
int avt_maxpool3d_train_fwd(const float* x, float* y, void* tap, int batch, int t, int h, int w, int c, int64_t ldy, void* stream);
int avt_maxpool3d_train_bwd(const float* dy, const void* tap, float* dx, int batch, int t, int h, int w, int c, int64_t ld_dy, void* stream);

int avt_interp_pack_pair_u8(const uint8_t* frame0, const uint8_t* frame1, int height, int width, const float* mean3,
                            float* img, void* x_hi, void* x_lo, int plane_dtype, void* stream);
int avt_avgpool2_x3(const void* in_hi, const void* in_lo, int batch, int h, int w, int c, int ldi, void* out_hi,
                    void* out_lo, int ldo, int plane_dtype, void* stream);
int avt_upsample2_bilinear_x3(const void* in_hi, const void* in_lo, int batch, int h, int w, int c, int ldi,
                              void* out_hi, void* out_lo, int ldo, int plane_dtype, void* stream);
int avt_interp_mid_input(const float* img, const void* flow_hi, const void* flow_lo, int height, int width, int sf,
                         void* x_hi, void* x_lo, float* ft, int plane_dtype, void* stream);
int avt_interp_final_u8(const float* img, const float* ft, const void* o_hi, const void* o_lo, int height, int width,
                        int sf, const float* mean3, uint8_t* out, int plane_dtype, void* stream);

int avt_pairwise_l2_f32(const float* x, int n, int64_t d, float* out, void* stream);
int avt_diag_filter_f32(const float* d1, int n, const float* w, int fs, float* out, void* stream);
int avt_q_learning_supported(int n);
int avt_q_learning_f32(const float* d3, int n, float alpha, float tol, int max_iter, float* out, int* iters,
                       void* stream);

int avt_conv33_c64_supported(int cin, int cout, int w);
int avt_conv33_c64_bf16(const void* in, const void* wb, const float* bias, void* out, int batch, int t,
                        int h, int w, int ldo, int relu, void* stream);

int avt_pw_chain_supported(int k1, int n1, int n2, int has_res, int k2x);
int avt_pw_chain_bf16(const void* x1, int ldx, int k1, const void* w1, const float* b1, const void* res, int ldr,
                      void* y, int ldy, int n1, const void* x2, int ldx2, int k2x, const void* w2, const float* b2,
                      void* z, int ldz, int n2, int64_t m, void* stream);

int avt_logmel_f64(const void* wave, int wave_is_f64, int64_t n_samples,
                   const double* window, int win, int hop, int fft_len,
                   const double* melmat, int n_mel, double log_offset,
                   double* logmel, void* stream);

int avt_logmel_examples_f32(const double* logmel, int64_t n_frames, int n_mel,
                            int ex_len, int ex_hop, float* out, void* stream);

#ifdef __cplusplus
}
#endif
#endif
```

Measured before the change: 1451.

## Load x3 conv weights in MFMA fragment order directly from global into registers

Adds a fragment-order weight layout for the 256x256 x3 implicit-GEMM conv kernel. Each wave now loads its hi/lo weight fragments straight from global memory into registers, prefetched two k-steps ahead inside the MFMA loop. This removes the weight tiles from LDS staging, halving the stage size and the LDS read traffic. It costs extra vector registers and relaxed vmcnt waits, and it is enabled by default for supported layer shapes apart from a skip list.

```diff
diff --git a/audio-video-textures_amd/_lib.py b/audio-video-textures_amd/_lib.py
--- a/audio-video-textures_amd/_lib.py
+++ b/audio-video-textures_amd/_lib.py
@@ -116,6 +116,8 @@
                         _vp, _vp, _vp, _vp, _vp, _vp, C.c_int, C.c_int, C.c_int64, C.c_int, _vp],
     "avt_conv3d_igemm_x3": [_vp] * 10 + [C.c_int] * 26 + [_vp, _vp],
     "avt_conv3d_igemm_x3_wblk": [_vp] * 10 + [C.c_int] * 26 + [_vp, _vp],
+    "avt_conv3d_igemm_x3_wfrag_supported": [C.c_int] * 5,
+    "avt_conv3d_igemm_x3_wfrag": [_vp] * 9 + [C.c_int] * 26 + [_vp, _vp],
     "avt_clip_pack_u8_ndhwc4_x3": [_vp, C.c_int, C.c_int, C.c_int, _vp, _vp, C.c_int, C.c_int, C.c_float, C.c_float,
                                    C.c_int, _vp, _vp, _vp, _vp, C.c_int, _vp],
     "avt_maxpool_hw3s2_ndhwc_x3": [_vp] * 4 + [C.c_int] * 8 + [_vp, _vp],
diff --git a/audio-video-textures_amd/csrc/conv_x3.hip b/audio-video-textures_amd/csrc/conv_x3.hip
--- a/audio-video-textures_amd/csrc/conv_x3.hip
+++ b/audio-video-textures_amd/csrc/conv_x3.hip
@@ -420,13 +420,15 @@
   STAMP_END();
 }
 
-template <bool F16, bool IO32 = false, bool OUT32 = IO32>
+template <bool F16, bool IO32 = false, bool OUT32 = IO32, bool WF = false>
 __global__ __launch_bounds__(512, 2) void conv_x3_xl_kernel(ConvArgs a) {
+  static_assert(!WF || (!IO32 && !OUT32), "fragment-order weights: the inference form only");
   constexpr int BM = 256, BN = 256, NTHR = 512, KB = 32;
   constexpr int MT = 4, NT = 2;
   constexpr int AU = BM / 128, BU = BN / 128;
   constexpr int PL = BM * 64;
-  constexpr int STG = 4 * PL;
+  constexpr int STG = (WF ? 2 : 4) * PL;
+  constexpr int TAB = 2 * 4 * PL;
   constexpr int ESTR = BN * 4 + 16;
   extern __shared__ __attribute__((aligned(16))) char lds[];
 
@@ -485,7 +487,7 @@
   const __amdgpu_buffer_rsrc_t ril = avt::buffer_rsrc(a.in_lo, a.in_bytes);
   const __amdgpu_buffer_rsrc_t rwh = avt::buffer_rsrc(a.wt, a.wt_bytes);
   const __amdgpu_buffer_rsrc_t rwl = avt::buffer_rsrc(a.wt_lo, a.wt_bytes);
-  int2* ltab = reinterpret_cast<int2*>(lds + 2 * STG);
+  int2* ltab = reinterpret_cast<int2*>(lds + TAB);
   for (int i = tid; i < a.nk * 8; i += NTHR) ltab[i] = a.ktab[i];
   const int nk32 = (a.K + KB - 1) / KB;
 
@@ -498,17 +500,19 @@
       const unsigned sel = ((rowmask[u] & ebits) == ebits) ? 0xFFFFFFFFu : 0u;
       aoffs[u] = (((unsigned)(rowoff[u] + e.x) * (IO32 ? 4u : 2u)) & sel) | (kOob & ~sel);
     }
-    const unsigned ksel = ~(unsigned)(e.y >> 31);
-    const unsigned kc2 = (unsigned)((kt * 4 + c4) * 16);
-#pragma unroll
-    for (int u = 0; u < BU; ++u) {
-      const unsigned sel = ksel & wsel[u];
-      boffs[u] = (((unsigned)wrow[u] * 2u + kc2) & sel) | (kOob & ~sel);
-      if (a.wblk) boffs[u] = (((unsigned)(kt * a.Cout + n0 + r0 + 128 * u) * 64u + (unsigned)c4 * 16u) & sel) | (kOob & ~sel);
+    if constexpr (!WF) {
+      const unsigned ksel = ~(unsigned)(e.y >> 31);
+      const unsigned kc2 = (unsigned)((kt * 4 + c4) * 16);
+#pragma unroll
+      for (int u = 0; u < BU; ++u) {
+        const unsigned sel = ksel & wsel[u];
+        boffs[u] = (((unsigned)wrow[u] * 2u + kc2) & sel) | (kOob & ~sel);
+        if (a.wblk) boffs[u] = (((unsigned)(kt * a.Cout + n0 + r0 + 128 * u) * 64u + (unsigned)c4 * 16u) & sel) | (kOob & ~sel);
+      }
     }
   };
   auto gprep = [&](int kt) { gcalc(kt, gtab(kt)); };
-  constexpr int NPIECE = 2 * (AU + BU);
+  constexpr int NPIECE = WF ? 2 * AU : 2 * (AU + BU);
   typedef __attribute__((address_space(3))) void* lds_ptr;
   const int wrow0 = wid * 16 * 64;
   auto gpiece = [&](int p, char* st) {
@@ -552,12 +556,20 @@
   struct Frags {
     i32x4 ah[MT], al[MT], wh[NT], wl[NT];
   };
+  const __amdgpu_buffer_rsrc_t rwf = avt::buffer_rsrc(a.wfrag, a.wf_bytes);
+  const int wfb = WF ? __builtin_amdgcn_readfirstlane((tn * 4 + wn) * nk32 * 8192) : 0;
+  auto wload = [&](Frags& f, int i, int s) {
+    f.wh[i] = __builtin_amdgcn_raw_buffer_load_b128(rwf, lane * 16 + i * 2048, wfb + s * 4096, 0);
+    f.wl[i] = __builtin_amdgcn_raw_buffer_load_b128(rwf, lane * 16 + i * 2048 + 1024, wfb + s * 4096, 0);
+  };
   auto fload = [&](Frags& f, const char* st, int ks) {
     const int slot = ((ks * 2 + lh) ^ fsw) * 16;
     auto rd_w = [&](int i) {
-      const int o = (wn * 64 + i * 32 + lr) * 64 + slot;
-      f.wh[i] = *reinterpret_cast<const i32x4*>(st + 2 * PL + o);
-      f.wl[i] = *reinterpret_cast<const i32x4*>(st + 3 * PL + o);
+      if constexpr (!WF) {
+        const int o = (wn * 64 + i * 32 + lr) * 64 + slot;
+        f.wh[i] = *reinterpret_cast<const i32x4*>(st + 2 * PL + o);
+        f.wl[i] = *reinterpret_cast<const i32x4*>(st + 3 * PL + o);
+      }
     };
     rd_w(0);
 #pragma unroll
@@ -569,9 +581,9 @@
 #pragma unroll
     for (int i = 1; i < NT; ++i) rd_w(i);
   };
-  auto fmul = [&](const Frags& f, int g0, bool more, char* nst) {
-#pragma unroll
-    for (int i = 0; i < NT; ++i)
+  auto fmul = [&](Frags& f, int g0, bool more, char* nst, bool refill = false, int wnext = 0) {
+#pragma unroll
+    for (int i = 0; i < NT; ++i) {
 #pragma unroll
       for (int j = 0; j < MT; ++j) {
         acc[i][j] = mfma32<F16>(f.wl[i], f.ah[j], acc[i][j]);
@@ -581,6 +593,13 @@
         if (more && pc < NPIECE) gpiece(pc, nst);
         __builtin_amdgcn_sched_barrier(0);
       }
+      if constexpr (WF) {
+        if (refill) {
+          wload(f, i, wnext);
+          __builtin_amdgcn_sched_barrier(0);
+        }
+      }
+    }
   };
 
   float* cfl = reinterpret_cast<float*>(lds + a.cf_ofs);
@@ -605,6 +624,14 @@
 #pragma unroll
     for (int p = 0; p < NPIECE; ++p) gpiece(p, lds);
     asm volatile("s_waitcnt vmcnt(0)" ::: "memory");
+  }
+  Frags f0, f1;
+  if constexpr (WF) {
+#pragma unroll
+    for (int i = 0; i < NT; ++i) wload(f0, i, 0);
+#pragma unroll
+    for (int i = 0; i < NT; ++i) wload(f1, i, 1);
+    __builtin_amdgcn_sched_barrier(0);
   }
   __syncthreads();
   STAMP(0);
@@ -631,42 +658,47 @@
       __syncthreads();
     }
   } else {
-    Frags f0, f1;
+    const int slast = 2 * nk32 - 1;
+    const int2 enone = make_int2(0, -1);
     fload(f0, lds, 0);
-    if (nk32 > 1) gprep(1);
+    if constexpr (WF) gcalc(1, nk32 > 1 ? gtab(1) : enone);
+    else if (nk32 > 1) gprep(1);
     fload(f1, lds, 1);
     __builtin_amdgcn_sched_barrier(0);
-    fmul(f0, 0, nk32 > 1, lds + STG);
-    asm volatile("s_waitcnt vmcnt(0) lgkmcnt(0)" ::: "memory");
+    fmul(f0, 0, WF || nk32 > 1, lds + STG, WF, 2 < slast ? 2 : slast);
+    if constexpr (WF) asm volatile("s_waitcnt vmcnt(4) lgkmcnt(0)" ::: "memory");
+    else asm volatile("s_waitcnt vmcnt(0) lgkmcnt(0)" ::: "memory");
     __syncthreads();
     for (int kt = 1; kt < nk32; ++kt) {
       const bool more = kt + 1 < nk32;
       char* cur = lds + (kt & 1) * STG;
       char* nst = lds + ((kt + 1) & 1) * STG;
-      int2 e = make_int2(0, 0);
+      int2 e = WF ? enone : make_int2(0, 0);
       if (more) e = gtab(kt + 1);
       fload(f0, cur, 0);
-      if (more) gcalc(kt + 1, e);
+      if (WF || more) gcalc(kt + 1, e);
       __builtin_amdgcn_sched_barrier(0);
-      fmul(f1, 0, more, nst);
+      fmul(f1, 0, WF || more, nst, WF, 2 * kt + 1);
       KSTAMP(1);
       fload(f1, cur, 1);
       __builtin_amdgcn_sched_barrier(0);
-      fmul(f0, NPIECE, false, nst);
+      fmul(f0, NPIECE, false, nst, WF, more ? 2 * kt + 2 : slast);
       KSTAMP(2);
-      asm volatile("s_waitcnt vmcnt(0) lgkmcnt(0)" ::: "memory");
+      if constexpr (WF) asm volatile("s_waitcnt vmcnt(8) lgkmcnt(0)" ::: "memory");
+      else asm volatile("s_waitcnt vmcnt(0) lgkmcnt(0)" ::: "memory");
       KSTAMP(3);
       __syncthreads();
       KSTAMP(4);
     }
     fmul(f1, NPIECE, false, lds);
+    if constexpr (WF) asm volatile("" ::"v"(f0.wh[0]), "v"(f0.wl[0]), "v"(f0.wh[1]), "v"(f0.wl[1]));
   }
 
   constexpr int SR = 64;
   constexpr int CPR = BN / 8;
   constexpr int EU = (SR * CPR) / NTHR;
   constexpr int EBUF = SR * ESTR;
-  static_assert(2 * EBUF <= 2 * STG + kMaxTabSteps * 64, "two staging buffers fit the operand stages + the table area");
+  static_assert(2 * EBUF <= TAB + kMaxTabSteps * 64, "two staging buffers fit the operand stages + the table area");
   const bool has_res = !OUT32 && a.res != nullptr;
   auto stage_slab = [&](auto half, int pass) {
     constexpr int H = decltype(half)::value;
@@ -809,7 +841,7 @@
   STAMP_END();
 }
 
-template <bool F16, bool IO32 = false, bool OUT32 = IO32>
+template <bool F16, bool IO32 = false, bool OUT32 = IO32, bool WF = false>
 int launch_x3_xl(ConvArgs& a, hipStream_t st) {
   if (a.stat_part) a.stat_tpg = (a.stat_mg + 255) / 256;
   const int tiles_m = a.stat_part ? a.stat_groups * a.stat_tpg : (a.M + 255) / 256;
@@ -817,8 +849,8 @@
   a.nblk = tiles_m * a.tiles_n;
   constexpr int lds_bytes = 2 * 4 * 256 * 64 + kMaxTabSteps * 64 + 2 * 256 * 4;
   a.cf_ofs = lds_bytes - 2 * 256 * 4;
-  return avt::launch<conv_x3_xl_kernel<F16, IO32, OUT32>>("avt_conv3d_igemm_x3", dim3((unsigned)a.nblk), dim3(512), lds_bytes, lds_bytes,
-                                                          st, a);
+  return avt::launch<conv_x3_xl_kernel<F16, IO32, OUT32, WF>>("avt_conv3d_igemm_x3", dim3((unsigned)a.nblk), dim3(512), lds_bytes,
+                                                              lds_bytes, st, a);
 }
 
 template <int BM, int BN, int WTM, bool F16, bool IO32 = false, bool BST = false>
@@ -862,8 +894,16 @@
   return (cout % 256 == 0 && k >= 256 && k <= kMaxTabSteps * 64 && m >= 256 * 64) ? 1 : 0;
 }
 
+enum { kWRows = 0, kWBlk = 1, kWFrag = 2 };
+
+extern "C" int avt_conv3d_igemm_x3_wfrag_supported(int cin, int cout, int kt, int kh, int kw) {
+  if (cin <= 0 || cin % 8 || cout <= 0 || kt < 1 || kh < 1 || kw < 1 || kt > 8 || kh > 8 || kw > 8) return 0;
+  const int64_t k = (int64_t)cin * kt * kh * kw;
+  return (k % 32 == 0 && k * cout * 4 < (1ll << 31) && avt_conv3d_igemm_x3_xl_picked(cout, (int)k, 256 * 64)) ? 1 : 0;
+}
+
 static int igemm_x3_one(const X3Planes& p, const int32_t* ktab, const ConvGeom& g, int plane_dtype, const float* wscale, void* stream,
-                        int wblk, int xl) {
+                        int worder, int xl) {
   AVT_REQUIRE(plane_dtype == AVT_X3_BF16 || plane_dtype == AVT_X3_F16, "avt_conv3d_igemm_x3: plane_dtype must be 0 (bf16) or 1 (fp16)");
   AVT_REQUIRE(!wscale || avt::aligned16(wscale), "avt_conv3d_igemm_x3: wscale must be 16-byte aligned");
   AVT_REQUIRE(p.in_lo && p.wt_lo && p.out_lo && (!p.res_hi == !p.res_lo), "avt_conv3d_igemm_x3: every tensor needs both planes");
@@ -879,16 +919,24 @@
   a.wscale = wscale;
   a.wfrag = nullptr;
   a.nup = 0;
-  a.wblk = wblk;
+  a.wblk = worder == kWBlk;
   hipStream_t s = static_cast<hipStream_t>(stream);
-  AVT_REQUIRE(!wblk || (xl && a.K % 32 == 0),
+  AVT_REQUIRE(worder != kWBlk || (xl && a.K % 32 == 0),
               "avt_conv3d_igemm_x3_wblk: K-blocked weights are the 256 x 256 tile's (avt_conv3d_igemm_x3_xl_picked, K %% 32 == 0)");
+  if (worder == kWFrag) {
+    AVT_REQUIRE(xl && avt_conv3d_igemm_x3_wfrag_supported(g.cin, g.cout, g.kt, g.kh, g.kw),
+                "avt_conv3d_igemm_x3_wfrag: fragment-order weights are the 256 x 256 tile's (avt_conv3d_igemm_x3_wfrag_supported, "
+                "avt_conv3d_igemm_x3_xl_picked)");
+    a.wfrag = a.wt;
+    a.wf_bytes = (unsigned)((int64_t)a.Cout * a.K * 4);
+    return plane_dtype == AVT_X3_F16 ? launch_x3_xl<true, false, false, true>(a, s) : launch_x3_xl<false, false, false, true>(a, s);
+  }
   if (xl) return plane_dtype == AVT_X3_F16 ? launch_x3_xl<true>(a, s) : launch_x3_xl<false>(a, s);
   return plane_dtype == AVT_X3_F16 ? launch_x3_by_cout<true>(a, s) : launch_x3_by_cout<false>(a, s);
 }
 
 static int igemm_x3_impl(const X3Planes& p, const int32_t* ktab, const ConvGeom& g, int plane_dtype, const float* wscale, void* stream,
-                         int wblk) {
+                         int worder) {
   constexpr int64_t kMaxPlane = (1ll << 31) - 64;
   const bool sane = g.batch > 0 && g.t > 0 && g.h > 0 && g.w > 0 && g.ldi > 0 && g.ldo > 0 && g.cin > 0 && g.cout > 0 && g.kt >= 1 &&
                     g.kh >= 1 && g.kw >= 1 && g.st >= 1 && g.sh >= 1 && g.sw >= 1 && g.ph >= 0 && g.pw >= 0 && g.ho >= 0 && g.wo >= 0 &&
@@ -903,7 +951,7 @@
       const int64_t m = (int64_t)g.batch * fto * fho * fwo;
       xl = (m > 0 && m < (1ll << 31)) ? avt_conv3d_igemm_x3_xl_picked(g.cout, (int)k_all, (int)m) : 0;
     }
-    return igemm_x3_one(p, ktab, g, plane_dtype, wscale, stream, wblk, xl);
+    return igemm_x3_one(p, ktab, g, plane_dtype, wscale, stream, worder, xl);
   }
   AVT_REQUIRE(frame < kMaxPlane, "avt_conv3d_igemm_x3: one frame's input plane (%d x %d x %d elements) is too large for 32-bit offsets", g.h,
               g.w, g.ldi);
@@ -930,7 +978,7 @@
     pr.in_hi = adv(p.in_hi, io), pr.in_lo = adv(p.in_lo, io);
     pr.res_hi = adv(p.res_hi, ro), pr.res_lo = adv(p.res_lo, ro);
     pr.out_hi = const_cast<void*>(adv(p.out_hi, oo)), pr.out_lo = const_cast<void*>(adv(p.out_lo, oo));
-    const int rc = igemm_x3_one(pr, ktab, gr, plane_dtype, wscale, stream, wblk, xl);
+    const int rc = igemm_x3_one(pr, ktab, gr, plane_dtype, wscale, stream, worder, xl);
     if (rc != AVT_OK) return rc;
   }
   return AVT_OK;
@@ -947,7 +995,7 @@
                       .ldi = ldi, .ldo = ldo, .ldr = ldr, .relu = relu, .out_row_stride = out_row_stride, .out_h = out_h, .out_w = out_w};
   const X3Planes p = {.in_hi = in_hi, .in_lo = in_lo, .wt_hi = wt_hi, .wt_lo = wt_lo, .bias = bias,
                       .res_hi = res_hi, .res_lo = res_lo, .out_hi = out_hi, .out_lo = out_lo};
-  return igemm_x3_impl(p, ktab, g, plane_dtype, wscale, stream, 0);
+  return igemm_x3_impl(p, ktab, g, plane_dtype, wscale, stream, kWRows);
 }
 
 extern "C" int avt_conv3d_igemm_x3_wblk(const void* in_hi, const void* in_lo, const void* wt_hi, const void* wt_lo,
@@ -961,7 +1009,20 @@
                       .ldi = ldi, .ldo = ldo, .ldr = ldr, .relu = relu, .out_row_stride = out_row_stride, .out_h = out_h, .out_w = out_w};
   const X3Planes p = {.in_hi = in_hi, .in_lo = in_lo, .wt_hi = wt_hi, .wt_lo = wt_lo, .bias = bias,
                       .res_hi = res_hi, .res_lo = res_lo, .out_hi = out_hi, .out_lo = out_lo};
-  return igemm_x3_impl(p, ktab, g, plane_dtype, wscale, stream, 1);
+  return igemm_x3_impl(p, ktab, g, plane_dtype, wscale, stream, kWBlk);
+}
+
+extern "C" int avt_conv3d_igemm_x3_wfrag(const void* in_hi, const void* in_lo, const void* wfrag, const float* bias, const void* res_hi,
+                                         const void* res_lo, void* out_hi, void* out_lo, const int32_t* ktab, int batch, int t, int h,
+                                         int w, int cin, int cout, int kt, int kh, int kw, int st, int sh, int sw, int pt, int ph, int pw,
+                                         int to, int ho, int wo, int ldi, int ldo, int ldr, int relu, int out_row_stride, int out_h,
+                                         int out_w, int plane_dtype, const float* wscale, void* stream) {
+  const ConvGeom g = {.batch = batch, .t = t, .h = h, .w = w, .cin = cin, .cout = cout, .kt = kt, .kh = kh, .kw = kw,
+                      .st = st, .sh = sh, .sw = sw, .pt = pt, .ph = ph, .pw = pw, .to = to, .ho = ho, .wo = wo,
+                      .ldi = ldi, .ldo = ldo, .ldr = ldr, .relu = relu, .out_row_stride = out_row_stride, .out_h = out_h, .out_w = out_w};
+  const X3Planes p = {.in_hi = in_hi, .in_lo = in_lo, .wt_hi = wfrag, .wt_lo = wfrag, .bias = bias,
+                      .res_hi = res_hi, .res_lo = res_lo, .out_hi = out_hi, .out_lo = out_lo};
+  return igemm_x3_impl(p, ktab, g, plane_dtype, wscale, stream, kWFrag);
 }
 
 extern "C" int avt_gemm_nt_x3_f32out(const void* a_hi, const void* a_lo, int lda, const void* b_hi, const void* b_lo, float* out, int64_t ldo,
diff --git a/audio-video-textures_amd/fused_slowfast.py b/audio-video-textures_amd/fused_slowfast.py
--- a/audio-video-textures_amd/fused_slowfast.py
+++ b/audio-video-textures_amd/fused_slowfast.py
@@ -19,6 +19,9 @@
 _FUSE_TCHUNK_X3 = 0
 _CHAIN_X3 = 1
 _WBLK_X3 = 1
+_WFRAG_X3 = 1
+_WFRAG_X3_SKIP = {(256, 1920), (2048, 1792), (256, 896)}
+_WFRAG_X3_SKIP |= {(256, 3456), (256, 6912), (512, 6912), (512, 256), (256, 8192)}
 _STEM_FM_X3 = 1
 _C33_X3 = 1
 _RES2_X3 = 1
@@ -132,6 +135,14 @@
     kidx = torch.where((cch < cin) & (i < nu), tap * cin + cch, torch.full_like(cch, k)).expand(nup, 2, 64, 8)
     rows = (torch.arange(tiles).view(-1, 1, 1, 1, 1) * 32 + (lane & 31).view(1, 1, 1, 64, 1)).expand(tiles, nup, 2, 64, 8)
     return wp[rows, kidx.unsqueeze(0).expand(tiles, nup, 2, 64, 8)].to(torch.bfloat16).contiguous()
+
+
+def pack_wfrag_x3(hi, lo):
+    cout, k = hi.shape
+    if cout % 256 or k % 32 or lo.shape != hi.shape:
+        raise AvtError("pack_wfrag_x3: planes must be two [Cout, K] with Cout %% 256 == 0 and K %% 32 == 0 (got %s, %s)" % (tuple(hi.shape), tuple(lo.shape)))
+    p = torch.stack([hi, lo]).view(2, cout // 256, 4, 2, 32, k // 32, 2, 2, 8)
+    return p.permute(1, 2, 5, 6, 3, 0, 7, 4, 8).reshape(cout // 256, 4, k // 32, 2, 2, 2, 64, 8).contiguous()
 
 
 class FusedConv:
@@ -160,7 +171,7 @@
             raise AvtError("FusedConv: input channels must be a multiple of 8 (got %d)" % self.cin)
         if cout % 8:
             raise AvtError("FusedConv: output channels must be a multiple of 8 (got %d)" % cout)
-        self.wfrag = self.wt_lo = self.wscale = self.wblk = self.pw = self.lat = None
+        self.wfrag = self.wt_lo = self.wscale = self.wblk = self.wfrag3 = self.pw = self.lat = None
         taps = self.kernel[0] * self.kernel[1] * self.kernel[2]
         if x3 is not None:
             wf = wt.detach().float()
@@ -176,6 +187,8 @@
             if _WBLK_X3 and cout % 256 == 0 and k_all % 32 == 0 and ops.conv3d_igemm_x3_xl_picked(cout, k_all, 1 << 20):
                 blk = lambda p: p.view(cout, k_all // 32, 32).permute(1, 0, 2).contiguous().to(device)
                 self.wblk = (blk(hi), blk(lo))
+            if _WFRAG_X3 and (cout, k_all) not in _WFRAG_X3_SKIP and ops.conv3d_igemm_x3_wfrag_supported(self.cin, cout, self.kernel):
+                self.wfrag3 = pack_wfrag_x3(hi, lo).to(device)
             if (_PW_X3 and relu != 2 and self.kernel == (1, 1, 1) and self.stride == (1, 1, 1) and self.pad == (0, 0, 0) and
                     not any(self.crop) and cout % 32 == 0 and ops.pw_x3_supported(self.cin, cout) and
                     (self.cin, cout) not in _PW_X3_SKIP):
@@ -205,7 +218,7 @@
             if self.pw is not None or self.lat is not None:
                 return "pw_x3_kernel<%s>" % ("f16" if self.x3 == ops.X3_F16 else "bf16")
             if ops.conv3d_igemm_x3_xl_picked(self.cout, self.wt.shape[1], m_out):
-                return "conv_x3_xl_kernel<%s>" % ("f16" if self.x3 == ops.X3_F16 else "bf16")
+                return "conv_x3_xl_kernel<%s%s>" % ("f16" if self.x3 == ops.X3_F16 else "bf16", ",wfrag" if self.wfrag3 is not None else "")
             tile = "128,32,32" if self.cout <= 32 else ("128,64,64" if self.cout <= 64 else "128,128,64")
             return "conv_x3_kernel<%s,%s>" % (tile, "f16" if self.x3 == ops.X3_F16 else "bf16")
         if self.wfrag is not None:
@@ -267,13 +280,15 @@
             out = new_act(m_out, self.cout, od, self.dev, self.x3 is not None)
 
         def launch_x3():
-            blocked = self.wblk is not None and ops.conv3d_igemm_x3_xl_picked(self.cout, self.wt.shape[1], m_out)
+            xl = ops.conv3d_igemm_x3_xl_picked(self.cout, self.wt.shape[1], m_out)
+            frag = self.wfrag3 if xl else None
+            blocked = frag is None and self.wblk is not None and xl
             wh, wl = self.wblk if blocked else (self.wt, self.wt_lo)
             ops.conv3d_igemm_x3(x.ptrs, wh, wl, self.bias, res.ptrs if res is not None else None, out.ptrs, tab,
                                 x.dims, self.cin, self.cout, self.kernel, self.stride, self.pad, x.ld, out.ld,
                                 res.ld if res is not None else 0, self.relu if relu is None else relu, self.x3,
                                 wscale=self.wscale, out_dims=od[1:] if any(self.crop) else (0, 0, 0), out_rows=out_rows,
-                                wblk=blocked)
+                                wblk=blocked, wfrag=frag)
 
         def launch_pw():
             ops.pw_x3(x.ptrs, x.ld, self.cin, self.pw[0], self.pw[1], self.bias, self.wscale,
diff --git a/audio-video-textures_amd/ops.py b/audio-video-textures_amd/ops.py
--- a/audio-video-textures_amd/ops.py
+++ b/audio-video-textures_amd/ops.py
@@ -406,19 +406,24 @@
 
 
 def conv3d_igemm_x3(x_ptrs, wt_hi, wt_lo, bias, res_ptrs, out_ptrs, ktab, dims, cin, cout, kernel, stride, pad, ldi, ldo,
-                    ldr, relu, plane_dtype, wscale=None, out_dims=(0, 0, 0), out_rows=None, wblk=False):
+                    ldr, relu, plane_dtype, wscale=None, out_dims=(0, 0, 0), out_rows=None, wblk=False, wfrag=None):
     b, t, h, w = dims
-    _dev(wt_hi, "wt_hi", torch.bfloat16)
-    _dev(wt_lo, "wt_lo", torch.bfloat16)
     orr = out_rows if out_rows is not None else (1, 0, 0)
     rh, rl = res_ptrs if res_ptrs is not None else (0, 0)
-    fn = _lib.lib().avt_conv3d_igemm_x3_wblk if wblk else _lib.lib().avt_conv3d_igemm_x3
-    _lib.check(fn(C.c_void_p(x_ptrs[0]), C.c_void_p(x_ptrs[1]), _p(wt_hi), _p(wt_lo), _p(bias),
+    if wfrag is not None:
+        _dev(wfrag, "wfrag", torch.bfloat16)
+        fn, who, wts = _lib.lib().avt_conv3d_igemm_x3_wfrag, "avt_conv3d_igemm_x3_wfrag", (_p(wfrag),)
+    else:
+        _dev(wt_hi, "wt_hi", torch.bfloat16)
+        _dev(wt_lo, "wt_lo", torch.bfloat16)
+        fn, who = (_lib.lib().avt_conv3d_igemm_x3_wblk, "avt_conv3d_igemm_x3_wblk") if wblk else (_lib.lib().avt_conv3d_igemm_x3, "avt_conv3d_igemm_x3")
+        wts = (_p(wt_hi), _p(wt_lo))
+    _lib.check(fn(C.c_void_p(x_ptrs[0]), C.c_void_p(x_ptrs[1]), *wts, _p(bias),
                                               C.c_void_p(rh) if rh else None, C.c_void_p(rl) if rl else None,
                                               C.c_void_p(out_ptrs[0]), C.c_void_p(out_ptrs[1]), _p(ktab), b, t, h, w,
                                               int(cin), int(cout), *kernel, *stride, *pad, *out_dims, int(ldi), int(ldo),
                                               int(ldr), int(relu), int(orr[0]), int(orr[1]), int(orr[2]),
-                                              int(plane_dtype), _p(wscale), _stream()), "avt_conv3d_igemm_x3_wblk" if wblk else "avt_conv3d_igemm_x3")
+                                              int(plane_dtype), _p(wscale), _stream()), who)
 
 
 def conv3d_igemm_x3_f32(x, wt_hi, wt_lo, wscale, out, ktab, dims, cin, cout, kernel, stride, pad, ldi, ldo, plane_dtype, add=None):
@@ -803,6 +808,10 @@
     return bool(_lib.lib().avt_conv3d_igemm_x3_xl_picked(int(cout), int(k), int(m)))
 
 
+def conv3d_igemm_x3_wfrag_supported(cin, cout, kernel):
+    return bool(_lib.lib().avt_conv3d_igemm_x3_wfrag_supported(int(cin), int(cout), *[int(v) for v in kernel]))
+
+
 def conv33_x3_supported(cin, cout):
     return bool(_lib.lib().avt_conv33_x3_supported(int(cin), int(cout)))
 
diff --git a/include/avt.h b/include/avt.h
--- a/include/avt.h
+++ b/include/avt.h
@@ -153,6 +153,13 @@
                              int kw, int st, int sh, int sw, int pt, int ph, int pw, int to, int ho, int wo, int ldi,
                              int ldo, int ldr, int relu, int out_row_stride, int out_h, int out_w, int plane_dtype,
                              const float* wscale, void* stream);
+int avt_conv3d_igemm_x3_wfrag_supported(int cin, int cout, int kt, int kh, int kw);
+int avt_conv3d_igemm_x3_wfrag(const void* in_hi, const void* in_lo, const void* wfrag, const float* bias,
+                              const void* res_hi, const void* res_lo, void* out_hi, void* out_lo,
+                              const int32_t* ktab, int batch, int t, int h, int w, int cin, int cout, int kt, int kh,
+                              int kw, int st, int sh, int sw, int pt, int ph, int pw, int to, int ho, int wo, int ldi,
+                              int ldo, int ldr, int relu, int out_row_stride, int out_h, int out_w, int plane_dtype,
+                              const float* wscale, void* stream);
 int avt_conv33_x3_supported(int cin, int cout);
 int avt_conv33_x3(const void* x_hi, const void* x_lo, const void* wfrag, const float* coef, void* out_hi, void* out_lo,
                   int batch, int t, int h, int w, int ldi, int ldo, int relu, int plane_dtype, void* stream);
```

After: 1449. Within noise of the previous version (-0.1%).
